# yuxiaoxiangyong/Multilateral-Temporal-view-Pyramid-Transformer-for-Video-Inpainting-Detection

Hardware: AMD Instinct MI355X
Metric: clips/sec fwd (B=8,T=5,224x224) (higher is better)
Workload: dtype f32; 1 GPU; full Mumpy forward (3 temporal views, pyramid decoder), B=8 clips/GPU, T=5, 224x224, fp32, tubelets (5,4,1); global_batch=8, launch=hipGraph replay, fork/join over HIP streams (independent branches co-scheduled), parallelism=batch-sharded x1, one metric all-reduce

## Files before the change

### multilateral-temporal-view-pyramid-transformer-for-video-inpainting-detection_amd/csrc/abi.cpp

```cpp
#include <stdarg.h>
#include <stdio.h>
#include <string.h>
#include "common.h"
#include "../../include/mumpy_hip_ext.h"
#include "../../include/mumpy_hip_ext2.h"
#include "../../include/mumpy_hip_ext3.h"
#include "../../include/mumpy_hip_ext4.h"
#include "../../include/mumpy_hip_ext5.h"
#include "../../include/mumpy_hip_ext6.h"
#include "../../include/mumpy_hip_ext7.h"
#include "../../include/mumpy_hip_ext8.h"
#include "../../include/mumpy_hip_ext9.h"
#include "../../include/mumpy_hip_ext10.h"
#include "../../include/mumpy_perturb.h"

namespace mumpy {
static thread_local char g_err[512] = "";
void set_error(const char* fmt, ...) {
    va_list ap;
    va_start(ap, fmt);
    vsnprintf(g_err, sizeof(g_err), fmt, ap);
    va_end(ap);
}
thread_local Route g_route;
static thread_local char g_route_text[160] = "";
static const char* format_route() {
    static const char* const addr[] = {"dense", "rows", "kseg", "conv"};
    static const char* const ln[] = {"none", "producer", "consumer"};
    static const char* const red[] = {"none", "one", "two-in-one", "taps"};
    const Route& r = g_route;
    char* t = g_route_text;
    const size_t n = sizeof(g_route_text);
    switch (r.family) {
    case Route::TILED: snprintf(t, n, "tiled tile=%d ks=%d np=%d addr=%s", r.tile, r.ks, r.np, addr[r.addr & 3]); break;
    case Route::TILED16: snprintf(t, n, "tiled16 tile=%d ks=%d np=%d addr=%s", r.tile, r.ks, r.np, addr[r.addr & 3]); break;
    case Route::WS:
        snprintf(t, n, "ws sched=%s P=%d ln=%s addr=%s", r.split ? "split" : "whole", r.passes, ln[r.ln < 3 ? r.ln : 0], addr[r.addr & 3]);
        break;
    case Route::WS64: snprintf(t, n, "ws64 P=%d addr=dense", r.passes); break;
    case Route::WS16: snprintf(t, n, "ws16 P=%d addr=dense", r.passes); break;
    case Route::XGEMM: {
        char dx[24] = "-", dw[24] = "-";
        if (r.prod[0].wt) snprintf(dx, sizeof(dx), "%dx%d", r.prod[0].wt, r.prod[0].ks);
        if (r.prod[1].wt) snprintf(dw, sizeof(dw), "%dx%d", r.prod[1].wt, r.prod[1].ks);
        snprintf(t, n, "xgemm np=%d addr=%s dx=%s dw=%s reduce=%s", r.np, addr[r.addr & 3], dx, dw, red[r.reduce & 3]);
        break;
    }
    default: snprintf(t, n, "none");
    }
    if (r.dual && r.family != Route::NONE) {
        const size_t len = strlen(t);
        snprintf(t + len, n - len, r.family == Route::XGEMM ? " gate=gelu" : " dual=z");
    }
    return t;
}
#ifdef MUMPY_TUNING
#include <stdlib.h>
int tune_int(const char* name, int dflt) {
    const char* v = getenv(name);
    return v ? atoi(v) : dflt;
}
const char* tune_str(const char* name) { return getenv(name); }
#endif
}

extern "C" int mumpy_tuning_build(void) {
#ifdef MUMPY_TUNING
    return 1;
#else
    return 0;
#endif
}

extern "C" int mumpy_abi_version(void) { return MUMPY_ABI_VERSION; }
extern "C" int mumpy_ext_version(void) { return MUMPY_EXT_VERSION; }
extern "C" int mumpy_ext2_version(void) { return MUMPY_EXT2_VERSION; }
extern "C" int mumpy_ext3_version(void) { return MUMPY_EXT3_VERSION; }
extern "C" int mumpy_ext4_version(void) { return MUMPY_EXT4_VERSION; }
extern "C" int mumpy_ext5_version(void) { return MUMPY_EXT5_VERSION; }
extern "C" int mumpy_ext6_version(void) { return MUMPY_EXT6_VERSION; }
extern "C" int mumpy_ext7_version(void) { return MUMPY_EXT7_VERSION; }
extern "C" int mumpy_ext8_version(void) { return MUMPY_EXT8_VERSION; }
extern "C" int mumpy_ext9_version(void) { return MUMPY_EXT9_VERSION; }
extern "C" int mumpy_ext10_version(void) { return MUMPY_EXT10_VERSION; }
extern "C" int mumpy_perturb_version(void) { return MUMPY_PERTURB_VERSION; }
extern "C" const char* mumpy_last_error(void) { return mumpy::g_err; }
extern "C" const char* mumpy_last_route(void) { return mumpy::format_route(); }
```

### multilateral-temporal-view-pyramid-transformer-for-video-inpainting-detection_amd/csrc/common.h

```cpp
#pragma once
#include <hip/hip_runtime.h>
#include <stdint.h>
#include <stdio.h>
#include "../../include/mumpy_hip.h"

namespace mumpy {

typedef float f32x4 __attribute__((ext_vector_type(4)));
typedef float f32x16 __attribute__((ext_vector_type(16)));

constexpr int WAVE = 64;
constexpr int WS = 7;
constexpr int WT = 49;
constexpr int HD = 32;

void set_error(const char* fmt, ...);

#ifdef MUMPY_TUNING
int tune_int(const char* name, int dflt);
const char* tune_str(const char* name);
#else
inline int tune_int(const char*, int dflt) { return dflt; }
inline const char* tune_str(const char*) { return nullptr; }
#endif

struct Route {
    enum Family : uint8_t { NONE, TILED, TILED16, WS, WS64, WS16, XGEMM };
    enum Addr : uint8_t { DENSE, ROWS, KSEG, CONV };
    enum Reduce : uint8_t { R_NONE, R_ONE, R_TWO_IN_ONE, R_TAPS };
    uint8_t family = NONE;
    uint8_t tile = 0;
    uint8_t np = 0;
    uint8_t addr = DENSE;
    uint8_t split = 0;
    uint8_t passes = 0;
    uint8_t ln = 0;
    uint8_t reduce = R_NONE;
    uint8_t dual = 0;
    int ks = 1;
    struct { int wt, ks; } prod[2] = {{0, 0}, {0, 0}};
};
extern thread_local Route g_route;

inline hipStream_t as_stream(void* s) { return reinterpret_cast<hipStream_t>(s); }
inline bool aligned16(const void* p) { return (reinterpret_cast<uintptr_t>(p) & 15u) == 0; }

#define MUMPY_CHECK_LAUNCH(name)                                                     \
    do {                                                                             \
        hipError_t e_ = hipGetLastError();                                           \
        if (e_ != hipSuccess) {                                                      \
            mumpy::set_error("%s: launch failed: %s", name, hipGetErrorString(e_));  \
            return (int)e_;                                                          \
        }                                                                            \
    } while (0)

#define MUMPY_REQUIRE(cond, code, ...)                                               \
    do {                                                                             \
        if (!(cond)) {                                                               \
            mumpy::set_error(__VA_ARGS__);                                           \
            return code;                                                             \
        }                                                                            \
    } while (0)

__device__ __forceinline__ unsigned xcd_major_id(unsigned orig, unsigned nwg) {
    const unsigned xcd = orig & 7, q8 = nwg >> 3, r8 = nwg & 7;
    return (xcd < r8 ? xcd * (q8 + 1) : r8 * (q8 + 1) + (xcd - r8) * q8) + (orig >> 3);
}

template <int CTRL>
__device__ __forceinline__ float dpp_f(float v) {
    return __builtin_bit_cast(float, __builtin_amdgcn_update_dpp(0, __builtin_bit_cast(int, v), CTRL, 0xF, 0xF, true));
}
__device__ __forceinline__ float swz_xor16(float v) {
    return __builtin_bit_cast(float, __builtin_amdgcn_ds_swizzle(__builtin_bit_cast(int, v), (16 << 10) | 0x1f));
}

__device__ __forceinline__ float wave_sum(float v, int width) {
    if (width > 1) v += dpp_f<0xB1>(v);
    if (width > 2) v += dpp_f<0x4E>(v);
    if (width > 4) v += dpp_f<0x141>(v);
    if (width > 8) v += dpp_f<0x140>(v);
    if (width > 16) v += swz_xor16(v);
    if (width > 32) v += __shfl_xor(v, 32);
    return v;
}

template <typename T>
__device__ __forceinline__ T ordered_sum(T first, const T* __restrict__ p, int64_t stride, int n_more) {
    T s = first;
    int z = 0;
    for (; z + 8 <= n_more; z += 8) {
        T v[8];
#pragma unroll
        for (int u = 0; u < 8; ++u) v[u] = p[(int64_t)(z + u) * stride];
#pragma unroll
        for (int u = 0; u < 8; ++u) s += v[u];
    }
    for (; z < n_more; ++z) s += p[(int64_t)z * stride];
    return s;
}

__device__ __forceinline__ void gn_block_stats(const float* __restrict__ stats, int nsplit, int G, int b, int64_t HW, int cg, float eps,
                                               float* gm, float* gr, double (*red)[2]) {
    const int tid = threadIdx.x, nslice = 256 / G, g = tid % G, k = tid / G;
    const int64_t per = (HW + nsplit - 1) / nsplit;
    const float* base = stats + (int64_t)b * nsplit * G * 2 + g * 2;
    const double piv = (double)base[0] / (double)((per < HW ? per : HW) * cg);
    double s = 0.0, q = 0.0;
    if (k < nslice)
        for (int sp = k; sp < nsplit; sp += nslice) {
            const int64_t p0 = sp * per, cnt = ((p0 + per < HW) ? p0 + per : HW) - p0;
            if (cnt <= 0) continue;
            const float* o = base + (int64_t)sp * G * 2;
            const double ni = (double)(cnt * cg), dm = (double)o[0] / ni - piv;
            s += ni * dm; q += (double)o[1] + ni * dm * dm;
        }
    red[tid][0] = s; red[tid][1] = q;
    __syncthreads();
    if (tid < G) {
        double ss = 0.0, qq = 0.0;
        for (int j = 0; j < nslice; ++j) { ss += red[j * G + tid][0]; qq += red[j * G + tid][1]; }
        const double n = (double)HW * (double)cg, dm = ss / n;
        double var = qq / n - dm * dm;
        if (var < 0.0) var = 0.0;
        gm[tid] = (float)(piv + dm);
        gr[tid] = (float)(1.0 / sqrt(var + (double)eps));
    }
    __syncthreads();
}

__device__ __forceinline__ float erf_fast(float x) {
    const float ax = fabsf(x);
    const float t = __builtin_amdgcn_rcpf(fmaf(0.3275911f, ax, 1.0f));
    float p = fmaf(1.061405429f, t, -1.453152027f);
    p = fmaf(p, t, 1.421413741f);
    p = fmaf(p, t, -0.284496736f);
    p = fmaf(p, t, 0.254829592f);
    const float y = 1.0f - p * t * __expf(-ax * ax);
    return copysignf(y, x);
}

__device__ __forceinline__ float gelu_erf(float x) { return 0.5f * x * (1.0f + erf_fast(x * 0.70710678118654752440f)); }

__device__ __forceinline__ float gelu_grad(float x) {
    const float cdf = 0.5f * (1.0f + erf_fast(x * 0.70710678118654752440f));
    const float pdf = 0.3989422804014327f * __expf(-0.5f * x * x);
    return cdf + x * pdf;
}

__device__ __forceinline__ int window_token(int wy, int wx, int p, int Hs, int W, int shift) {
    int py = p / WS, px = p - py * WS;
    int y = wy * WS + py + shift;
    int x = wx * WS + px + shift;
    if (y >= Hs) y -= Hs;
    if (x >= W) x -= W;
    return y * W + x;
}

}
```

### multilateral-temporal-view-pyramid-transformer-for-video-inpainting-detection_amd/csrc/gemm.hip

```cpp
#include <stdlib.h>
#include <type_traits>
#include "common.h"
#include "../../include/mumpy_hip_ext2.h"
#include "gemm_ws.h"
#include "gemm_ws64.h"
using namespace mumpy;

namespace {

constexpr int BK = 32;
constexpr int LDR = 36;

struct ConvGeom {
    int H, W, Cin, kh, kw, ph, pw;
    int kseg, kstride;
};

__device__ __attribute__((aligned(128))) float g_zero_page[32];

template <int BM, int BN>
__device__ __forceinline__ void tile_of_block(int64_t M, unsigned gn, int ksplit, unsigned& tm, unsigned& tn, int& ks) {
    constexpr unsigned NG = (BN >= 128) ? 4 : 8;
    unsigned wgid = xcd_major_id(blockIdx.x, gridDim.x);
    ks = (int)(wgid % (unsigned)ksplit);
    wgid /= (unsigned)ksplit;
    const unsigned gm = (unsigned)((M + BM - 1) / BM);
    const unsigned full = (gn / NG) * NG;
    if (wgid < gm * full) {
        const unsigned grp = wgid / (gm * NG), rem = wgid - grp * gm * NG;
        tm = rem / NG;
        tn = grp * NG + rem % NG;
    } else {
        const unsigned wdt = gn - full, rem = wgid - gm * full;
        tm = rem / wdt;
        tn = full + rem % wdt;
    }
}

struct ConvTap {
    int dy, dx, off;
    __device__ __forceinline__ bool inside(const ConvGeom& cg, int yx) const {
        const int yy = (yx >> 16) + dy, xx = (yx & 0xffff) + dx;
        return (unsigned)yy < (unsigned)cg.H && (unsigned)xx < (unsigned)cg.W;
    }
};
__device__ __forceinline__ ConvTap conv_tap(const ConvGeom& cg, int k0) {
    const int tap = k0 / cg.Cin, c0 = k0 - tap * cg.Cin;
    const int dy = tap / cg.kw - cg.ph, dx = tap % cg.kw - cg.pw;
    return {dy, dx, (dy * cg.W + dx) * cg.Cin + c0};
}

template <int TM, int TN, int WM, int WN, bool OUT16 = false, bool DUAL = false>
__device__ __forceinline__ void store_tile(const f32x16 (&acc)[TM][TN], int64_t m0, int n0, int wm, int wn, int c, int h,
                                           int64_t M, int N, const float* __restrict__ bias, const float* residual,
                                           float* Y, int act, int ksplit, int ks, float* slab) {
    const int wm_u = __builtin_amdgcn_readfirstlane(wm), wn_u = __builtin_amdgcn_readfirstlane(wn);
    const int64_t mw = m0 + wm_u * WM;
    const int64_t wbase = mw * N + n0 + wn_u * WN;
    const int rows_left = (int)((M - mw) < (int64_t)WM ? (M - mw) : (int64_t)WM);
    const uint32_t nb = 4u * (uint32_t)N;
    const uint32_t lane_off = 4u * h * nb + 4u * c;
    if (ksplit > 1) {
        char* S = reinterpret_cast<char*>(slab + (int64_t)ks * M * N + wbase);
#pragma unroll
        for (int j = 0; j < TN; ++j) {
            if (n0 + wn_u * WN + 32 * j + c >= N) continue;
#pragma unroll
            for (int i = 0; i < TM; ++i)
#pragma unroll
                for (int r = 0; r < 16; ++r) {
                    const int row = 32 * i + (r & 3) + 8 * (r >> 2);
                    if (row + 4 * h < rows_left) *reinterpret_cast<float*>(S + ((uint32_t)row * nb + lane_off + 128u * j)) = acc[i][j][r];
                }
        }
        return;
    }
    char* Yw = OUT16 ? reinterpret_cast<char*>(reinterpret_cast<__bf16*>(Y) + wbase) : reinterpret_cast<char*>(Y + wbase);
    const char* Rw = residual ? reinterpret_cast<const char*>(residual + wbase) : nullptr;
#pragma unroll
    for (int j = 0; j < TN; ++j) {
        const int n = n0 + wn_u * WN + 32 * j + c;
        if (n >= N) continue;
        const float bv = bias ? bias[n] : 0.f;
#pragma unroll
        for (int i = 0; i < TM; ++i)
#pragma unroll
            for (int r = 0; r < 16; ++r) {
                const int row = 32 * i + (r & 3) + 8 * (r >> 2);
                if (row + 4 * h >= rows_left) continue;
                const uint32_t off = (uint32_t)row * nb + lane_off + 128u * j;
                float v = acc[i][j][r] + bv;
                if (DUAL) *reinterpret_cast<float*>(const_cast<char*>(Rw) + off) = v;
                if (act == MUMPY_ACT_GELU) v = gelu_erf(v);
                if (!DUAL && Rw) v += *reinterpret_cast<const float*>(Rw + off);
                if (OUT16) *reinterpret_cast<__bf16*>(Yw + (off >> 1)) = (__bf16)v;
                else *reinterpret_cast<float*>(Yw + off) = v;
            }
    }
}

template <int BM, int BN, int WM, int WN, bool CONV, bool GLDS, bool PIPE = true, bool DUAL = false>
__global__ __launch_bounds__(64 * (BM / WM) * (BN / WN), (BM * BN > 64 * 64) ? 2 : (CONV ? 3 : 4)) void linear_kernel(const float* __restrict__ X, const float* __restrict__ Wt,
                                                     const float* __restrict__ bias, const float* residual,
                                                     float* Y, int64_t M, int N, int K, int act, unsigned gn,
                                                     int ksplit, float* slab, int64_t rpb, int64_t bstride, ConvGeom cg) {
    constexpr int TM = WM / 32, TN = WN / 32;
    constexpr int WAVES_N = BN / WN;
    constexpr int NT = 64 * (BM / WM) * (BN / WN);
    constexpr int RPI = NT / 8;
    constexpr int A_LD = BM / RPI;
    constexpr int B_LD = BN / RPI;
    static_assert(BM % RPI == 0 && BN % RPI == 0, "tile rows must divide over the staging passes");
    constexpr int LD = GLDS ? 32 : LDR;
    __shared__ __attribute__((aligned(1024))) float lds[2][(BM + BN) * LD];

    const int tid = threadIdx.x, lane = tid & 63, wave = tid >> 6;
    const int c = lane & 31, h = lane >> 5;
    const int wm = wave / WAVES_N, wn = wave % WAVES_N;
    unsigned tm, tn;
    int ks;
    tile_of_block<BM, BN>(M, gn, ksplit, tm, tn, ks);
    const int64_t m0 = (int64_t)tm * BM;
    const int n0 = (int)tn * BN;
    const int kbeg = ks * (K / ksplit);

    const int ld_row = tid >> 3, ld_c4 = tid & 7;
    f32x4 areg[A_LD], breg[B_LD];

    const float* arow[A_LD];
    const float* brow[B_LD];
    int ayx[A_LD];
#pragma unroll
    for (int i = 0; i < A_LD; ++i) {
        int64_t m = m0 + ld_row + RPI * i;
        if (m > M - 1) m = M - 1;
        if (CONV) {
            const unsigned mu = (unsigned)m, qx = mu / (unsigned)cg.W;
            const int x = (int)(mu - qx * (unsigned)cg.W);
            const int y = (int)(qx % (unsigned)cg.H);
            ayx[i] = (y << 16) | x;
            arow[i] = X + m * cg.Cin + 4 * ld_c4;
        } else {
            ayx[i] = 0;
            if (rpb >= M && !cg.kseg) arow[i] = X + m * K + 4 * ld_c4;
            else {
                const unsigned mu = (unsigned)m, blk = mu / (unsigned)rpb;
                arow[i] = X + (int64_t)blk * bstride + (int64_t)(mu - blk * (unsigned)rpb) * (cg.kseg ? cg.kseg : K) + 4 * ld_c4;
            }
        }
    }
#pragma unroll
    for (int i = 0; i < B_LD; ++i) {
        int n = n0 + ld_row + RPI * i;
        if (n > N - 1) n = N - 1;
        brow[i] = Wt + (int64_t)n * K + 4 * ld_c4;
    }
    int asw[A_LD], bsw[B_LD];
#pragma unroll
    for (int i = 0; i < A_LD; ++i) asw[i] = 4 * ((ld_c4 ^ (((ld_row + RPI * i) >> 1) & 7)) - ld_c4);
#pragma unroll
    for (int i = 0; i < B_LD; ++i) bsw[i] = 4 * ((ld_c4 ^ (((ld_row + RPI * i) >> 1) & 7)) - ld_c4);
    typedef __attribute__((address_space(1))) const void* gptr_t;
    typedef __attribute__((address_space(3))) void* lptr_t;
    auto gdma = [&](int k0, int buf) {
        const int wave_row = (tid >> 6) * 8;
        if (CONV) {
            const int tap = k0 / cg.Cin, c0 = k0 - tap * cg.Cin;
            const int dy = tap / cg.kw - cg.ph, dx = tap % cg.kw - cg.pw;
            const int off = (dy * cg.W + dx) * cg.Cin + c0;
#pragma unroll
            for (int i = 0; i < A_LD; ++i) {
                const int yy = (ayx[i] >> 16) + dy, xx = (ayx[i] & 0xffff) + dx;
                const bool ok = (unsigned)yy < (unsigned)cg.H && (unsigned)xx < (unsigned)cg.W;
                const float* src = ok ? arow[i] + off + asw[i] : g_zero_page + 4 * ld_c4;
                __builtin_amdgcn_global_load_lds((gptr_t)src, (lptr_t)&lds[buf][(wave_row + RPI * i) * LD], 16, 0, 0);
            }
        } else {
            const int ka = cg.kseg ? (k0 / cg.kseg) * cg.kstride + k0 % cg.kseg : k0;
#pragma unroll
            for (int i = 0; i < A_LD; ++i)
                __builtin_amdgcn_global_load_lds((gptr_t)(arow[i] + ka + asw[i]), (lptr_t)&lds[buf][(wave_row + RPI * i) * LD], 16, 0, 0);
        }
#pragma unroll
        for (int i = 0; i < B_LD; ++i)
            __builtin_amdgcn_global_load_lds((gptr_t)(brow[i] + k0 + bsw[i]), (lptr_t)&lds[buf][(BM + wave_row + RPI * i) * LD], 16, 0, 0);
    };
    auto gload = [&](int k0) {
        if (CONV) {
            const ConvTap t = conv_tap(cg, k0);
#pragma unroll
            for (int i = 0; i < A_LD; ++i) {
                const bool ok = t.inside(cg, ayx[i]);
                const f32x4 v = *reinterpret_cast<const f32x4*>(arow[i] + (ok ? t.off : 0));
                areg[i] = ok ? v : f32x4{0, 0, 0, 0};
            }
        } else {
            const int ka = cg.kseg ? (k0 / cg.kseg) * cg.kstride + k0 % cg.kseg : k0;
#pragma unroll
            for (int i = 0; i < A_LD; ++i) areg[i] = *reinterpret_cast<const f32x4*>(arow[i] + ka);
        }
#pragma unroll
        for (int i = 0; i < B_LD; ++i) breg[i] = *reinterpret_cast<const f32x4*>(brow[i] + k0);
    };
    auto lstore = [&](int buf) {
#pragma unroll
        for (int i = 0; i < A_LD; ++i)
            *reinterpret_cast<f32x4*>(&lds[buf][(ld_row + RPI * i) * LD + 4 * ld_c4]) = areg[i];
#pragma unroll
        for (int i = 0; i < B_LD; ++i)
            *reinterpret_cast<f32x4*>(&lds[buf][(BM + ld_row + RPI * i) * LD + 4 * ld_c4]) = breg[i];
    };
    auto fread = [&](int buf, f32x4 (&af)[TM][4], f32x4 (&bf)[TN][4]) {
#pragma unroll
        for (int i = 0; i < TM; ++i) {
            const int R = wm * WM + 32 * i + c;
#pragma unroll
            for (int q = 0; q < 4; ++q) {
                const int col = GLDS ? 4 * ((4 * h + q) ^ ((R >> 1) & 7)) : 16 * h + 4 * q;
                af[i][q] = *reinterpret_cast<const f32x4*>(&lds[buf][R * LD + col]);
            }
        }
#pragma unroll
        for (int j = 0; j < TN; ++j) {
            const int R = wn * WN + 32 * j + c;
#pragma unroll
            for (int q = 0; q < 4; ++q) {
                const int col = GLDS ? 4 * ((4 * h + q) ^ ((R >> 1) & 7)) : 16 * h + 4 * q;
                bf[j][q] = *reinterpret_cast<const f32x4*>(&lds[buf][(BM + R) * LD + col]);
            }
        }
    };

    f32x16 acc[TM][TN];
#pragma unroll
    for (int i = 0; i < TM; ++i)
#pragma unroll
        for (int j = 0; j < TN; ++j)
#pragma unroll
            for (int r = 0; r < 16; ++r) acc[i][j][r] = 0.f;
    auto mma = [&](const f32x4 (&af)[TM][4], const f32x4 (&bf)[TN][4]) {
#pragma unroll
        for (int s = 0; s < 16; ++s)
#pragma unroll
            for (int i = 0; i < TM; ++i)
#pragma unroll
                for (int j = 0; j < TN; ++j)
                    acc[i][j] = __builtin_amdgcn_mfma_f32_32x32x2f32(af[i][s >> 2][s & 3], bf[j][s >> 2][s & 3], acc[i][j], 0, 0, 0);
    };

    const int nk = K / ksplit / BK;
    f32x4 afA[TM][4], bfA[TN][4];
    if (GLDS && !PIPE) {
        gdma(kbeg, 0);
        if (nk > 1) gdma(kbeg + BK, 1);
        for (int kc = 0; kc < nk; ++kc) {
            __syncthreads();
            fread(kc & 1, afA, bfA);
            __syncthreads();
            if (kc + 2 < nk) gdma(kbeg + (kc + 2) * BK, kc & 1);
            mma(afA, bfA);
        }
    } else if (GLDS) {
        f32x4 afB[TM][4], bfB[TN][4];
        gdma(kbeg, 0);
        if (nk > 1) gdma(kbeg + BK, 1);
        __syncthreads();
        fread(0, afA, bfA);
        __syncthreads();
        if (nk > 2) gdma(kbeg + 2 * BK, 0);
        int kc = 0;
        for (; kc + 1 < nk; kc += 2) {
            fread(1, afB, bfB);
            mma(afA, bfA);
            __syncthreads();
            if (kc + 3 < nk) gdma(kbeg + (kc + 3) * BK, 1);
            if (kc + 2 < nk) fread(0, afA, bfA);
            mma(afB, bfB);
            __syncthreads();
            if (kc + 4 < nk) gdma(kbeg + (kc + 4) * BK, 0);
        }
        if (kc < nk) mma(afA, bfA);
    } else {
    f32x4 afB[TM][4], bfB[TN][4];
    gload(kbeg);
    lstore(0);
    if (nk > 1) gload(kbeg + BK);
    __syncthreads();
    fread(0, afA, bfA);
    if (nk > 1) lstore(1);
    if (nk > 2) gload(kbeg + 2 * BK);
    __syncthreads();
    int kc = 0;
    for (; kc + 1 < nk; kc += 2) {
        fread(1, afB, bfB);
        mma(afA, bfA);
        if (kc + 2 < nk) lstore(0);
        if (kc + 3 < nk) gload(kbeg + (kc + 3) * BK);
        __syncthreads();
        if (kc + 2 < nk) fread(0, afA, bfA);
        mma(afB, bfB);
        if (kc + 3 < nk) lstore(1);
        if (kc + 4 < nk) gload(kbeg + (kc + 4) * BK);
        __syncthreads();
    }
    if (kc < nk) mma(afA, bfA);
    }
    store_tile<TM, TN, WM, WN, false, DUAL>(acc, m0, n0, wm, wn, c, h, M, N, bias, residual, Y, act, ksplit, ks, slab);
}

typedef __bf16 bf16x8 __attribute__((ext_vector_type(8)));
typedef __bf16 bf16x2 __attribute__((ext_vector_type(2)));
typedef float f32x2 __attribute__((ext_vector_type(2)));
constexpr int LDH = 20;

template <int BM, int BN, int WM, int WN, bool CONV, int NP = 1, int NBUF = 2, bool IN16 = false, bool OUT16 = false, bool DUAL = false>
__global__ __launch_bounds__(256, 2) void linear_bf16_kernel(const float* __restrict__ X, const float* __restrict__ Wt,
                                                            const float* __restrict__ bias, const float* residual,
                                                            float* Y, int64_t M, int N, int K, int act, unsigned gn,
                                                            int ksplit, float* slab, int64_t rpb, int64_t bstride,
                                                            ConvGeom cg) {
    constexpr int TM = WM / 32, TN = WN / 32;
    constexpr int WAVES_N = BN / WN;
    static_assert((BM / WM) * (BN / WN) == 4, "4 waves per block");
    constexpr int RPI = 32, A_LD = BM / RPI, B_LD = BN / RPI;
    constexpr int PL = (BM + BN) * LDH;
    static_assert(NBUF * NP * PL * 4 <= 65536, "LDS tile exceeds the static limit");
    __shared__ __attribute__((aligned(16))) uint32_t lds[NBUF][NP * PL];
    const int tid = threadIdx.x, lane = tid & 63, wave = tid >> 6;
    const int c = lane & 31, h = lane >> 5;
    const int wm = wave / WAVES_N, wn = wave % WAVES_N;
    unsigned tm, tn;
    int ks;
    tile_of_block<BM, BN>(M, gn, ksplit, tm, tn, ks);
    const int64_t m0 = (int64_t)tm * BM;
    const int n0 = (int)tn * BN;
    const int kbeg = ks * (K / ksplit);
    const int ld_row = tid >> 3, ld_c4 = tid & 7;
    static_assert(!(IN16 || OUT16) || (NP == 1 && !CONV), "bf16 storage: plain bf16 products on dense operands only");
    f32x4 areg[A_LD], breg[B_LD];
    uint2 areg16[IN16 ? A_LD : 1], breg16[IN16 ? B_LD : 1];
    const float* arow[A_LD];
    const float* brow[B_LD];
    int ayx[A_LD];
#pragma unroll
    for (int i = 0; i < A_LD; ++i) {
        int64_t m = m0 + ld_row + RPI * i;
        if (m > M - 1) m = M - 1;
        if (IN16) {
            ayx[i] = 0;
            arow[i] = reinterpret_cast<const float*>(reinterpret_cast<const __bf16*>(X) + m * K + 4 * ld_c4);
            continue;
        }
        if (CONV) {
            const unsigned mu = (unsigned)m, qx = mu / (unsigned)cg.W;
            ayx[i] = ((int)(qx % (unsigned)cg.H) << 16) | (int)(mu - qx * (unsigned)cg.W);
            arow[i] = X + m * cg.Cin + 4 * ld_c4;
        } else {
            ayx[i] = 0;
            if (rpb >= M && !cg.kseg) arow[i] = X + m * K + 4 * ld_c4;
            else {
                const unsigned mu = (unsigned)m, blk = mu / (unsigned)rpb;
                arow[i] = X + (int64_t)blk * bstride + (int64_t)(mu - blk * (unsigned)rpb) * (cg.kseg ? cg.kseg : K) + 4 * ld_c4;
            }
        }
    }
#pragma unroll
    for (int i = 0; i < B_LD; ++i) {
        int n = n0 + ld_row + RPI * i;
        if (n > N - 1) n = N - 1;
        if (IN16) brow[i] = reinterpret_cast<const float*>(reinterpret_cast<const __bf16*>(Wt) + (int64_t)n * K + 4 * ld_c4);
        else brow[i] = Wt + (int64_t)n * K + 4 * ld_c4;
    }
    auto gload = [&](int k0) {
        if (IN16) {
#pragma unroll
            for (int i = 0; i < A_LD; ++i) areg16[i] = *reinterpret_cast<const uint2*>(reinterpret_cast<const __bf16*>(arow[i]) + k0);
#pragma unroll
            for (int i = 0; i < B_LD; ++i) breg16[i] = *reinterpret_cast<const uint2*>(reinterpret_cast<const __bf16*>(brow[i]) + k0);
            return;
        }
        if (CONV) {
            const ConvTap t = conv_tap(cg, k0);
#pragma unroll
            for (int i = 0; i < A_LD; ++i) {
                const bool ok = t.inside(cg, ayx[i]);
                const f32x4 v = *reinterpret_cast<const f32x4*>(arow[i] + (ok ? t.off : 0));
                areg[i] = ok ? v : f32x4{0, 0, 0, 0};
            }
        } else {
            const int ka = cg.kseg ? (k0 / cg.kseg) * cg.kstride + k0 % cg.kseg : k0;
#pragma unroll
            for (int i = 0; i < A_LD; ++i) areg[i] = *reinterpret_cast<const f32x4*>(arow[i] + ka);
        }
#pragma unroll
        for (int i = 0; i < B_LD; ++i) breg[i] = *reinterpret_cast<const f32x4*>(brow[i] + k0);
    };
    auto lstore_row = [&](uint32_t* dst, f32x4 r) {
#pragma unroll
        for (int p = 0; p < NP; ++p) {
            const bf16x2 lo = __builtin_convertvector(f32x2{r.x, r.y}, bf16x2), hi = __builtin_convertvector(f32x2{r.z, r.w}, bf16x2);
            const uint2 u = {*reinterpret_cast<const uint32_t*>(&lo), *reinterpret_cast<const uint32_t*>(&hi)};
            *reinterpret_cast<uint2*>(dst + p * PL) = u;
            if (p + 1 < NP)
                r -= f32x4{__uint_as_float(u.x << 16), __uint_as_float(u.x & 0xffff0000u), __uint_as_float(u.y << 16),
                           __uint_as_float(u.y & 0xffff0000u)};
        }
    };
    auto lstore = [&](int buf) {
        if (IN16) {
#pragma unroll
            for (int i = 0; i < A_LD; ++i) *reinterpret_cast<uint2*>(&lds[buf][(ld_row + RPI * i) * LDH + 2 * ld_c4]) = areg16[i];
#pragma unroll
            for (int i = 0; i < B_LD; ++i) *reinterpret_cast<uint2*>(&lds[buf][(BM + ld_row + RPI * i) * LDH + 2 * ld_c4]) = breg16[i];
            return;
        }
#pragma unroll
        for (int i = 0; i < A_LD; ++i) lstore_row(&lds[buf][(ld_row + RPI * i) * LDH + 2 * ld_c4], areg[i]);
#pragma unroll
        for (int i = 0; i < B_LD; ++i) lstore_row(&lds[buf][(BM + ld_row + RPI * i) * LDH + 2 * ld_c4], breg[i]);
    };
    f32x16 acc[TM][TN];
#pragma unroll
    for (int i = 0; i < TM; ++i)
#pragma unroll
        for (int j = 0; j < TN; ++j)
#pragma unroll
            for (int r = 0; r < 16; ++r) acc[i][j][r] = 0.f;
    constexpr int NPROD = (NP == 3) ? 6 : (NP == 2) ? 3 : 1;
    constexpr int PA[6] = {NP == 3 ? 2 : 1, 0, NP == 3 ? 1 : 0, 1, 0, 0}, PB[6] = {0, NP == 3 ? 2 : 1, NP == 3 ? 1 : 0, 0, 1, 0};
    const int nk = K / ksplit / BK;
    bf16x8 af[TM][2][NP], bf[TN][2][NP];
    auto fread = [&](int buf) {
#pragma unroll
        for (int i = 0; i < TM; ++i)
#pragma unroll
            for (int st = 0; st < 2; ++st)
#pragma unroll
                for (int p = 0; p < NP; ++p)
                    af[i][st][p] = *reinterpret_cast<const bf16x8*>(&lds[buf][p * PL + (wm * WM + 32 * i + c) * LDH + 8 * st + 4 * h]);
#pragma unroll
        for (int j = 0; j < TN; ++j)
#pragma unroll
            for (int st = 0; st < 2; ++st)
#pragma unroll
                for (int p = 0; p < NP; ++p)
                    bf[j][st][p] = *reinterpret_cast<const bf16x8*>(&lds[buf][p * PL + (BM + wn * WN + 32 * j + c) * LDH + 8 * st + 4 * h]);
    };
    auto mma = [&]() {
#pragma unroll
        for (int st = 0; st < 2; ++st)
#pragma unroll
            for (int q = 0; q < NPROD; ++q)
#pragma unroll
                for (int i = 0; i < TM; ++i)
#pragma unroll
                    for (int j = 0; j < TN; ++j)
                        acc[i][j] = __builtin_amdgcn_mfma_f32_32x32x16_bf16(af[i][st][NP > 1 ? PA[q] : 0],
                                                                            bf[j][st][NP > 1 ? PB[q] : 0], acc[i][j], 0, 0, 0);
    };
    const int klast = kbeg + (nk - 1) * BK;
    if (NBUF == 2) {
        gload(kbeg);
        lstore(0);
        __syncthreads();
        for (int kc = 0; kc + 1 < nk; ++kc) {
            gload(kbeg + (kc + 1) * BK);
            __builtin_amdgcn_sched_barrier(0);
            fread(kc & 1);
            mma();
            lstore((kc & 1) ^ 1);
            __syncthreads();
        }
        fread((nk - 1) & 1);
        mma();
    } else {
        gload(kbeg);
        lstore(0);
        gload(nk > 1 ? kbeg + BK : kbeg);
        __syncthreads();
        for (int kc = 0; kc + 1 < nk; ++kc) {
            fread(0);
            __syncthreads();
            lstore(0);
            const int knext = kbeg + (kc + 2) * BK;
            gload(knext < klast ? knext : klast);
            mma();
            __syncthreads();
        }
        fread(0);
        mma();
    }
    store_tile<TM, TN, WM, WN, OUT16, DUAL>(acc, m0, n0, wm, wn, c, h, M, N, bias, residual, Y, act, ksplit, ks, slab);
}

template <bool DUAL = false>
__global__ __launch_bounds__(256) void splitk_reduce_kernel(const float* __restrict__ slab, const float* __restrict__ bias,
                                                            const float* residual, float* Y, int64_t MN4, int N,
                                                            int ksplit, int act) {
    for (int64_t i = (int64_t)blockIdx.x * 256 + threadIdx.x; i < MN4; i += (int64_t)gridDim.x * 256) {
        f32x4 v = ordered_sum(reinterpret_cast<const f32x4*>(slab)[i], reinterpret_cast<const f32x4*>(slab) + MN4 + i, MN4, ksplit - 1);
        const int n = (int)((i * 4) % N);
        if (bias) v += *reinterpret_cast<const f32x4*>(bias + n);
        if (DUAL) reinterpret_cast<f32x4*>(const_cast<float*>(residual))[i] = v;
        if (act == MUMPY_ACT_GELU) {
#pragma unroll
            for (int e = 0; e < 4; ++e) v[e] = gelu_erf(v[e]);
        }
        if (!DUAL && residual) v += reinterpret_cast<const f32x4*>(residual)[i];
        reinterpret_cast<f32x4*>(Y)[i] = v;
    }
}

struct Plan {
    int tile;
    int ksplit;
    unsigned gn;
    int64_t gm;
};

constexpr int NUM_CU = 256;

int fit_ksplit(int K, int want, int min_slice, int max_ks) {
    int ks = want;
    if (ks > K / min_slice) ks = K / min_slice;
    if (ks > max_ks) ks = max_ks;
    while (ks > 1 && (K % (32 * ks)) != 0) --ks;
    return ks < 1 ? 1 : ks;
}

Plan make_plan_x3(int64_t M, int N, int K, bool allow_split) {
    Plan p;
    const int64_t gm128 = (M + 127) / 128, gm64 = (M + 63) / 64;
    const unsigned gn128 = (N + 127) / 128, gn64 = (N + 63) / 64;
    const int64_t b128 = gm128 * gn128, b64 = gm64 * gn64;
    auto fit = [&](int want) { return allow_split ? fit_ksplit(K, want, 384, 16) : 1; };
    const int ksw = fit((int)((448 + b128 / 2) / b128));
    if (b128 * ksw >= 240) {
        p.tile = 0; p.ksplit = ksw; p.gm = gm128; p.gn = gn128;
    } else {
        p.tile = 2; p.ksplit = (b64 < 2 * 256 && K >= 768) ? fit((int)((3 * 256 + b64 - 1) / b64)) : 1;
        p.gm = gm64; p.gn = gn64;
    }
    return p;
}

Plan make_plan(int64_t M, int N, int K, bool allow_split, bool x3 = false) {
    static const char* force = tune_str("MUMPY_GEMM_FORCE");
    if (x3 && !force) return make_plan_x3(M, N, K, allow_split);
    Plan p;
    const int64_t gm128 = (M + 127) / 128, gm64 = (M + 63) / 64;
    const unsigned gn128 = (N + 127) / 128, gn64 = (N + 63) / 64;
    const int64_t b128 = gm128 * gn128, b64 = gm64 * gn64;
    const double nk = (double)K / BK;
    const double t128 = (double)((b128 + NUM_CU - 1) / NUM_CU) * (nk + 2.0) / nk;
    double t64 = (double)((b64 + NUM_CU - 1) / NUM_CU) * 0.272;
    if (t64 < 0.357) t64 = 0.357;
    t64 *= (nk + 0.5) / nk;
    int tile = (t128 <= t64) ? 0 : 2;
    if (tile == 0 && b128 > NUM_CU && K >= 512) tile = 3;
    int ks = 1;
    static const int min_slice = tune_int("MUMPY_GEMM_MINSLICE", 384), max_ks = tune_int("MUMPY_GEMM_MAXKS", 16),
                     min_k = tune_int("MUMPY_GEMM_SPLIT_MINK", 768);
    if (tile == 2 && allow_split && b64 < 2 * NUM_CU && K >= min_k) ks = fit_ksplit(K, (int)((3 * NUM_CU + b64 - 1) / b64), min_slice, max_ks);
    if (force) {
        int ft = -1, fk = -1;
        if (sscanf(force, "%d,%d", &ft, &fk) >= 1 && ft >= 0 && ft <= 3) {
            tile = ft;
            if (fk >= 1 && allow_split && K % (32 * fk) == 0) ks = fk; else if (fk >= 1) ks = 1;
        }
    }
    p.tile = tile; p.ksplit = ks;
    p.gm = (tile == 0 || tile == 3) ? gm128 : gm64;
    p.gn = (tile == 2) ? gn64 : gn128;
    return p;
}

int device_cus() {
    static int num_cu = 0;
    if (!num_cu) {
        int dev = 0;
        hipDeviceProp_t prop;
        if (hipGetDevice(&dev) == hipSuccess && hipGetDeviceProperties(&prop, dev) == hipSuccess) num_cu = prop.multiProcessorCount;
        else num_cu = NUM_CU;
    }
    return num_cu;
}

int ws_plan(int64_t M, int N, int K, bool have_ws, bool conv) {
    static const int ws_mode = tune_int("MUMPY_GEMM_WS", 2);
    const int num_cu = device_cus();
    const int64_t tiles = ((M + 127) / 128) * ((N + 127) / 128);
    const int nk = K / 32;
    const double rounds = (double)tiles / num_cu, eff = rounds / (double)((tiles + num_cu - 1) / num_cu);
    const double per_cu = (double)tiles * nk / num_cu;
    int how = 0;
    if (ws_mode == 1) how = 1;
    else if (ws_mode == 3) how = have_ws ? 2 : 1;
    else if (ws_mode == 2 && conv) {
        if (have_ws && eff < 0.86 && per_cu >= 24.0 && (double)nk / per_cu <= 3.0) how = 2;
        else if (tiles >= (int64_t)(0.75 * num_cu) && eff >= 0.75 && K >= 128) how = 1;
    } else if (ws_mode == 2) {
        if (tiles >= (int64_t)(0.75 * num_cu) && eff >= 0.86 && K >= 128 && !(K >= 1024 && rounds >= 1.8)) how = 1;
        else if (have_ws && eff < 0.86 && per_cu >= 24.0 && (double)nk / per_cu <= 3.0 && !(K >= 1024 && rounds >= 1.8)) how = 2;
    }
    return how;
}

struct LinearArgs {
    const float *x, *W, *bias, *residual;
    float* y;
    int64_t M;
    int N, K, act;
    hipStream_t s;
    float* ws = nullptr;
    int64_t ws_bytes = 0;
    bool ws_clean = false;
    int64_t rpb = 0, bstride = 0;
    int kseg = 0, kstride = 0;
    const ConvGeom* conv = nullptr;
    const gemm_ws::LnArgs* ln = nullptr;
    float* z = nullptr;
};

struct TiledArgs {
    const float *x, *W, *bias, *residual;
    float* y;
    int64_t M;
    int N, K, act;
    unsigned gn;
    int ksplit;
    float* slab;
    int64_t rpb, bstride;
    ConvGeom cg;
    int64_t grid;
    hipStream_t s;
};

template <class Kern>
void launch_tiled(Kern kern, unsigned threads, const TiledArgs& t) {
    hipLaunchKernelGGL(kern, dim3((unsigned)t.grid), dim3(threads), 0, t.s, t.x, t.W, t.bias, t.residual, t.y, t.M, t.N, t.K, t.act,
                       t.gn, t.ksplit, t.slab, t.rpb, t.bstride, t.cg);
}

template <class F>
void with_bool(bool b, F&& f) {
    if (b) f(std::true_type{});
    else f(std::false_type{});
}

void launch_tiled_fp32(int tile, bool conv, bool glds, const TiledArgs& t) {
    with_bool(conv, [&](auto cv) {
        constexpr bool CV = decltype(cv)::value;
        if (tile == 3) return launch_tiled(linear_kernel<128, 128, 64, 64, CV, true, false>, 256, t);
        with_bool(glds, [&](auto gl) {
            constexpr bool GL = decltype(gl)::value;
            if (tile == 0) launch_tiled(linear_kernel<128, 128, 64, 32, CV, GL>, 512, t);
            else if (tile == 1) launch_tiled(linear_kernel<64, 128, 32, 64, CV, GL>, 256, t);
            else launch_tiled(linear_kernel<64, 64, 32, 32, CV, GL>, 256, t);
        });
    });
}

void launch_tiled_dual(int tile, bool bf16, const TiledArgs& t) {
    if (bf16) {
        if (tile == 0) launch_tiled(linear_bf16_kernel<128, 128, 64, 64, false, 1, 2, false, false, true>, 256, t);
        else launch_tiled(linear_bf16_kernel<64, 64, 32, 32, false, 1, 2, false, false, true>, 256, t);
    } else if (tile == 3) launch_tiled(linear_kernel<128, 128, 64, 64, false, true, false, true>, 256, t);
    else if (tile == 0) launch_tiled(linear_kernel<128, 128, 64, 32, false, false, true, true>, 512, t);
    else launch_tiled(linear_kernel<64, 64, 32, 32, false, false, true, true>, 256, t);
}

template <int NP, bool IN16 = false>
void launch_tiled_bf16(bool wide, bool flag, const TiledArgs& t) {
    with_bool(wide, [&](auto wd) {
        with_bool(flag, [&](auto fl) {
            constexpr int T = decltype(wd)::value ? 128 : 64, NBUF = (T == 128 && NP > 1) ? 1 : 2;
            constexpr bool FL = decltype(fl)::value;
            launch_tiled(linear_bf16_kernel<T, T, T / 2, T / 2, !IN16 && FL, NP, NBUF, IN16, IN16 && FL>, 256, t);
        });
    });
}

int launch_linear(const LinearArgs& a) {
    const int64_t M = a.M, rpb = a.rpb > 0 ? a.rpb : M, bstride = a.rpb > 0 ? a.bstride : 0;
    const int N = a.N, K = a.K, act = a.act & 0xff;
    const ConvGeom* conv = a.conv;
    ConvGeom cg = conv ? *conv : ConvGeom{0, 0, 0, 0, 0, 0, 0, 0, 0};
    cg.kseg = a.kseg; cg.kstride = a.kstride;
    const bool math_bf16 = (a.act & MUMPY_MATH_BF16) != 0;
    const bool math_x2 = (a.act & MUMPY_MATH_BF16X2) != 0;
    const bool math_x3 = (a.act & MUMPY_MATH_BF16X3) != 0 || math_x2;
    float* ws = a.ws;
    int64_t ws_bytes = a.ws_bytes;
    const gemm_ws::Conv cvd{cg.H, cg.W, cg.Cin, cg.kh, cg.kw};
    if (a.ln && (rpb < M || math_bf16 || math_x3 || conv || !gemm_ws::eligible(M, N, K) ||
                 !ws_plan(M, N, K, ws && ws_bytes >= gemm_ws::workspace_bytes(device_cus()), false))) {
        set_error("linear: LayerNorm folding needs a shape the persistent 128x128 kernel takes (mumpy_linear_ln_tiles) in fp32 mode");
        return MUMPY_EINVAL;
    }
    if (rpb >= M && !a.kseg && !math_bf16 && !math_x3 && (conv ? gemm_ws::conv_eligible(M, N, cvd) : gemm_ws::eligible(M, N, K))) {
        const int num_cu = device_cus();
        const bool have_ws = ws && ws_bytes >= gemm_ws::workspace_bytes(num_cu);
        const int how = ws_plan(M, N, K, have_ws, conv != nullptr);
        const int nk = K / 32;
        static const int ws64_mode = tune_int("MUMPY_GEMM_WS64", 1);
        if (!how && !conv && ws64_mode && !a.z) {
            const int64_t t64 = ((M + 63) / 64) * ((N + 63) / 64);
            const double r64 = (double)t64 / (2.0 * num_cu);
            const bool fits = ws64_mode == 2 || (act != MUMPY_ACT_GELU && nk <= 32 && t64 >= 64 && (r64 <= 1.0 || r64 >= 2.5 || nk <= 12));
            if (fits) {
                if (int rc = gemm_ws64::launch(a.x, a.W, a.bias, a.residual, a.y, M, N, K, act, num_cu, a.s)) return rc;
                MUMPY_CHECK_LAUNCH("linear(ws64)");
                return 0;
            }
        }
        if (how) {
            if (int rc = gemm_ws::launch(a.x, a.W, a.bias, a.residual, a.y, M, N, K, act, num_cu, a.s, ws, ws_bytes, how == 2 ? 1 : 0, nullptr,
                                         a.ws_clean, conv ? &cvd : nullptr, a.ln, a.z)) return rc;
            MUMPY_CHECK_LAUNCH("linear(ws)");
            return 0;
        }
    }
    Plan p = make_plan(M, N, K, ws != nullptr, math_x3);
    if (ws) { ws += 1024; ws_bytes -= 4096; }
    if (p.ksplit > 1 && (int64_t)p.ksplit * M * N * (int64_t)sizeof(float) > ws_bytes) p.ksplit = 1;
    if (math_bf16 || math_x3) {
        if (p.tile == 3) p.tile = 0;
        if (p.tile == 1) { p.tile = 2; p.gn = (unsigned)((N + 63) / 64); }
    }
    if (a.z && p.tile == 1) { p.tile = 2; p.gn = (unsigned)((N + 63) / 64); }
    const int64_t grid = p.gm * p.gn * p.ksplit;
    MUMPY_REQUIRE(grid < (1ll << 31), MUMPY_ERANGE, "linear: too many tiles");
    static const bool use_glds = tune_int("MUMPY_GEMM_GLDS", 0) != 0;
    const bool wide = (p.tile == 0 || p.tile == 3);
    const TiledArgs t{a.x, a.W, a.bias, a.z ? a.z : a.residual, a.y, M, N, K, act, p.gn, p.ksplit, ws, rpb, bstride, cg, grid, a.s};
    g_route = Route{};
    g_route.family = Route::TILED; g_route.tile = (uint8_t)p.tile; g_route.ks = p.ksplit;
    g_route.np = math_x2 ? 2 : math_x3 ? 3 : math_bf16 ? 1 : 0;
    g_route.addr = conv ? Route::CONV : a.kseg ? Route::KSEG : rpb < M ? Route::ROWS : Route::DENSE;
    g_route.dual = a.z ? 1 : 0;
    if (a.z) launch_tiled_dual(p.tile, math_bf16, t);
    else if (math_x2) launch_tiled_bf16<2>(wide, conv != nullptr, t);
    else if (math_x3) launch_tiled_bf16<3>(wide, conv != nullptr, t);
    else if (math_bf16) launch_tiled_bf16<1>(wide, conv != nullptr, t);
    else launch_tiled_fp32(p.tile, conv != nullptr, use_glds, t);
    MUMPY_CHECK_LAUNCH("linear");
    if (p.ksplit > 1) {
        const int64_t mn4 = M * N / 4;
        int64_t g = (mn4 + 255) / 256;
        if (g > 2048) g = 2048;
        if (a.z) hipLaunchKernelGGL(splitk_reduce_kernel<true>, dim3((unsigned)g), dim3(256), 0, a.s, ws, a.bias, a.z, a.y, mn4, N, p.ksplit, act);
        else hipLaunchKernelGGL(splitk_reduce_kernel<false>, dim3((unsigned)g), dim3(256), 0, a.s, ws, a.bias, a.residual, a.y, mn4, N,
                                p.ksplit, act);
        MUMPY_CHECK_LAUNCH("linear(split-K reduce)");
    }
    return 0;
}

}

static int check_linear_args(const char* who, const void* x, const void* W, const float* residual, const void* y, int64_t M, int N,
                             int K, int act) {
    MUMPY_REQUIRE(x && W && y, MUMPY_ENULL, "%s: null pointer", who);
    MUMPY_REQUIRE(aligned16(x) && aligned16(W) && aligned16(y) && aligned16(residual), MUMPY_EALIGN,
                  "%s: pointers must be 16-byte aligned", who);
    MUMPY_REQUIRE(M < (1ll << 31) - 256 && (int64_t)N * 4 * 128 < (1ll << 32), MUMPY_ERANGE,
                  "%s: M=%lld rows / N=%d columns beyond the 32-bit row index / tile byte offsets", who, (long long)M, N);
    MUMPY_REQUIRE(M >= 0 && N > 0 && K > 0 && K % BK == 0 && N % 32 == 0, MUMPY_EINVAL,
                  "%s: need K %% 32 == 0 and N %% 32 == 0 (got M=%lld N=%d K=%d)", who, (long long)M, N, K);
    MUMPY_REQUIRE((act & 0xff) == MUMPY_ACT_NONE || (act & 0xff) == MUMPY_ACT_GELU, MUMPY_EINVAL, "%s: unknown act %d", who, act);
    constexpr int math_bits = MUMPY_MATH_BF16 | MUMPY_MATH_BF16X3 | MUMPY_MATH_BF16X2;
    MUMPY_REQUIRE((act & ~(0xff | math_bits)) == 0, MUMPY_EINVAL, "%s: unknown flag bits in act 0x%x", who, act);
    MUMPY_REQUIRE(((act & math_bits) & ((act & math_bits) - 1)) == 0, MUMPY_EINVAL, "%s: the MUMPY_MATH_* modes are exclusive", who);
    return 0;
}

static LinearArgs linear_args(const float* x, const float* W, const float* bias, const float* residual, float* y, int64_t M, int N,
                              int K, int act, void* workspace, int64_t workspace_bytes, void* stream) {
    LinearArgs a{x, W, bias, residual, y, M, N, K, act, as_stream(stream)};
    a.ws = static_cast<float*>(workspace);
    a.ws_bytes = workspace ? workspace_bytes : 0;
    return a;
}

extern "C" int mumpy_linear_fwd(const float* x, const float* W, const float* bias, const float* residual, float* y,
                                int64_t M, int N, int K, int act, void* stream) {
    if (M == 0) return 0;
    if (int rc = check_linear_args("linear", x, W, residual, y, M, N, K, act)) return rc;
    return launch_linear(linear_args(x, W, bias, residual, y, M, N, K, act, nullptr, 0, stream));
}

extern "C" int64_t mumpy_linear_workspace_bytes(int64_t M, int N, int K) {
    if (M <= 0 || N <= 0 || K <= 0 || K % BK) return 0;
    const Plan p = make_plan(M, N, K, true), q = make_plan(M, N, K, true, true);
    const int ks = p.ksplit > q.ksplit ? p.ksplit : q.ksplit;
    int64_t bytes = ks > 1 ? (int64_t)ks * M * N * (int64_t)sizeof(float) + 4096 : 0;
    if (gemm_ws::eligible(M, N, K)) {
        const int64_t tiles = ((M + 127) / 128) * ((N + 127) / 128);
        const double per_cu = (double)tiles * (K / 32) / NUM_CU;
        const int64_t need = gemm_ws::workspace_bytes(2 * NUM_CU);
        if (per_cu >= 16.0 && bytes < need) bytes = need;
    }
    return bytes;
}

extern "C" int mumpy_linear_ws_fwd(const float* x, const float* W, const float* bias, const float* residual, float* y,
                                   int64_t M, int N, int K, int act, void* workspace, int64_t workspace_bytes,
                                   void* stream) {
    if (M == 0) return 0;
    if (int rc = check_linear_args("linear", x, W, residual, y, M, N, K, act)) return rc;
    MUMPY_REQUIRE(workspace_bytes >= 0, MUMPY_EINVAL, "linear_ws: workspace_bytes must not be negative");
    MUMPY_REQUIRE(aligned16(workspace), MUMPY_EALIGN, "linear: workspace must be 16-byte aligned");
    return launch_linear(linear_args(x, W, bias, residual, y, M, N, K, act, workspace, workspace_bytes, stream));
}

extern "C" int mumpy_linear_bf16s_fwd(const void* x, const void* W, const float* bias, const float* residual, void* y,
                                      int64_t M, int N, int K, int act, int out_bf16, void* stream) {
    if (M == 0) return 0;
    if (int rc = check_linear_args("linear_bf16s", x, W, residual, y, M, N, K, act)) return rc;
    MUMPY_REQUIRE((act & ~0xff) == 0, MUMPY_EINVAL, "linear_bf16s: unknown act %d", act);
    MUMPY_REQUIRE(!(out_bf16 && residual), MUMPY_EINVAL, "linear_bf16s: a bf16 output takes no residual");
    hipStream_t s = as_stream(stream);
    static const int ws16 = tune_int("MUMPY_GEMM_WS16", 2);
    const int64_t gm128 = (M + 127) / 128, gm64 = (M + 63) / 64;
    const unsigned gn128 = (N + 127) / 128, gn64 = (N + 63) / 64;
    if (ws16 && gemm_ws::eligible16(M, N, K)) {
        const int num_cu = device_cus();
        const int64_t tiles = gm128 * gn128;
        const double rounds = (double)tiles / num_cu, eff = rounds / (double)((tiles + num_cu - 1) / num_cu);
        if (ws16 == 2 || (tiles >= (int64_t)(0.75 * num_cu) && eff >= 0.75)) {
            if (int rc = gemm_ws::launch16(x, W, bias, residual, y, M, N, K, act, out_bf16 != 0, num_cu, s)) return rc;
            MUMPY_CHECK_LAUNCH("linear_bf16s(ws)");
            return 0;
        }
    }
    const bool wide = gm128 * gn128 >= 200;
    const unsigned gn = wide ? gn128 : gn64;
    const int64_t grid = (wide ? gm128 : gm64) * gn;
    MUMPY_REQUIRE(grid < (1ll << 31), MUMPY_ERANGE, "linear_bf16s: too many tiles");
    const TiledArgs t{static_cast<const float*>(x), static_cast<const float*>(W), bias, residual, static_cast<float*>(y), M, N, K, act,
                      gn, 1, nullptr, M, 0, ConvGeom{0, 0, 0, 0, 0, 0, 0, 0, 0}, grid, s};
    g_route = Route{};
    g_route.family = Route::TILED16; g_route.tile = wide ? 0 : 2; g_route.np = 1;
    launch_tiled_bf16<1, true>(wide, out_bf16 != 0, t);
    MUMPY_CHECK_LAUNCH("linear_bf16s");
    return 0;
}

extern "C" int mumpy_linear_wsz_fwd(const float* x, const float* W, const float* bias, const float* residual, float* y,
                                    int64_t M, int N, int K, int act, void* workspace, int64_t workspace_bytes,
                                    void* stream) {
    if (M == 0) return 0;
    if (int rc = check_linear_args("linear", x, W, residual, y, M, N, K, act)) return rc;
    MUMPY_REQUIRE(workspace_bytes >= 0, MUMPY_EINVAL, "linear_wsz: workspace_bytes must not be negative");
    MUMPY_REQUIRE(aligned16(workspace), MUMPY_EALIGN, "linear: workspace must be 16-byte aligned");
    LinearArgs a = linear_args(x, W, bias, residual, y, M, N, K, act, workspace, workspace_bytes, stream);
    a.ws_clean = true;
    return launch_linear(a);
}

extern "C" int mumpy_linear_gelu_dual_fwd(const float* x, const float* W, const float* bias, float* z, float* a, int64_t M, int N,
                                          int K, int math, void* workspace, int64_t workspace_bytes, void* stream) {
    if (M == 0) return 0;
    MUMPY_REQUIRE(math == 0 || math == MUMPY_MATH_BF16, MUMPY_EINVAL,
                  "linear_gelu_dual: math is 0 or MUMPY_MATH_BF16 (the split-precision modes have no dual-output form; got 0x%x)", math);
    MUMPY_REQUIRE(z, MUMPY_ENULL, "linear_gelu_dual: null pointer");
    if (int rc = check_linear_args("linear_gelu_dual", x, W, z, a, M, N, K, MUMPY_ACT_GELU | math)) return rc;
    MUMPY_REQUIRE(z != a, MUMPY_EINVAL, "linear_gelu_dual: z and a must be two buffers");
    MUMPY_REQUIRE(workspace_bytes >= 0, MUMPY_EINVAL, "linear_gelu_dual: workspace_bytes must not be negative");
    MUMPY_REQUIRE(aligned16(workspace) && aligned16(bias), MUMPY_EALIGN, "linear_gelu_dual: bias and workspace must be 16-byte aligned");
    MUMPY_REQUIRE(!workspace || workspace_bytes >= mumpy_linear_workspace_bytes(M, N, K), MUMPY_EINVAL,
                  "linear_gelu_dual: workspace too small (mumpy_linear_workspace_bytes)");
    LinearArgs la = linear_args(x, W, bias, nullptr, a, M, N, K, MUMPY_ACT_GELU | math, workspace, workspace_bytes, stream);
    la.ws_clean = true;
    la.z = z;
    return launch_linear(la);
}

extern "C" int mumpy_workspace_status(const void* workspace, int* status) {
    MUMPY_REQUIRE(workspace && status, MUMPY_ENULL, "workspace_status: null pointer");
    unsigned w[2] = {0, 0};
    static_assert(gemm_ws::LN_GUARD_WORD + 1 == gemm_ws::STATUS_WORD, "status words must be adjacent");
    hipError_t e = hipMemcpy(w, static_cast<const unsigned*>(workspace) + gemm_ws::LN_GUARD_WORD, sizeof(w), hipMemcpyDeviceToHost);
    if (e != hipSuccess) { set_error("workspace_status: %s", hipGetErrorString(e)); return (int)e; }
    *status = w[1] ? (int)w[1] : (w[0] ? -1 : 0);
    return 0;
}

extern "C" int mumpy_linear_ln_tiles(int64_t M, int N, int K) {
    if (M <= 0 || N <= 0 || K <= 0 || K % BK || N % 32 || !gemm_ws::eligible(M, N, K)) return 0;
    return ws_plan(M, N, K, true, false) ? (N + 127) / 128 : 0;
}

extern "C" int mumpy_linear_lnx_fwd(const float* x, const float* W, const float* bias, const float* residual, float* y, int64_t M,
                                    int N, int K, int act, void* workspace, int64_t workspace_bytes, float* stats_out,
                                    const float* ln_stats, int ln_gn, const float* ln_colsum, float ln_eps, void* stream) {
    if (M == 0) return 0;
    if (int rc = check_linear_args("linear", x, W, residual, y, M, N, K, act)) return rc;
    MUMPY_REQUIRE((act & ~0xff) == 0, MUMPY_EINVAL, "linear_lnx: fp32 matrix math only");
    MUMPY_REQUIRE(aligned16(workspace) && workspace, MUMPY_EALIGN, "linear_lnx: needs the kept (zeroed) workspace of mumpy_linear_wsz_fwd");
    MUMPY_REQUIRE(ln_gn >= 0, MUMPY_EINVAL, "linear_lnx: ln_gn must not be negative");
    MUMPY_REQUIRE(workspace_bytes >= 4096, MUMPY_EINVAL, "linear_lnx: the kept workspace holds at least its 4096-byte flag page (got %lld B)",
                  (long long)workspace_bytes);
    MUMPY_REQUIRE((stats_out != nullptr) != (ln_stats != nullptr), MUMPY_EINVAL, "linear_lnx: exactly one of stats_out (producer) / ln_stats (consumer)");
    MUMPY_REQUIRE(!ln_stats || (ln_colsum && bias && !residual && ln_gn == (K + 127) / 128 && ln_gn <= 16 && ln_eps > 0.f), MUMPY_EINVAL,
                  "linear_lnx: the consumer takes W gamma, colsum, bias = W beta + b, no residual, and ln_gn = ceil(K / 128) tiles (got %d)", ln_gn);
    MUMPY_REQUIRE(aligned16(stats_out) && aligned16(ln_stats) && aligned16(ln_colsum), MUMPY_EALIGN, "linear_lnx: pointers must be 16-byte aligned");
    MUMPY_REQUIRE(M * (int64_t)((N + 127) / 128) * 8 < (1ll << 31) && M * (int64_t)(ln_gn > 0 ? ln_gn : 1) * 8 < (1ll << 31), MUMPY_ERANGE,
                  "linear_lnx: statistics buffer beyond 2 GiB");
    const gemm_ws::LnArgs ln{stats_out, ln_stats, ln_colsum, ln_gn, K, ln_eps};
    LinearArgs a = linear_args(x, W, bias, residual, y, M, N, K, act, workspace, workspace_bytes, stream);
    a.ws_clean = true;
    a.ln = &ln;
    return launch_linear(a);
}

extern "C" int mumpy_linear_rows_fwd(const float* x, int64_t rows_per_block, int64_t block_stride, const float* W,
                                     const float* bias, const float* residual, float* y, int64_t M, int N, int K, int act,
                                     void* workspace, int64_t workspace_bytes, void* stream) {
    if (M == 0) return 0;
    if (int rc = check_linear_args("linear", x, W, residual, y, M, N, K, act)) return rc;
    MUMPY_REQUIRE(workspace_bytes >= 0, MUMPY_EINVAL, "linear_rows: workspace_bytes must not be negative");
    MUMPY_REQUIRE(rows_per_block > 0 && M % rows_per_block == 0 && block_stride >= 0 && block_stride % 4 == 0, MUMPY_EINVAL,
                  "linear_rows: M=%lld must be a multiple of rows_per_block=%lld and block_stride >= 0, %% 4 == 0",
                  (long long)M, (long long)rows_per_block);
    LinearArgs a = linear_args(x, W, bias, residual, y, M, N, K, act, workspace, workspace_bytes, stream);
    a.rpb = rows_per_block; a.bstride = block_stride;
    return launch_linear(a);
}

extern "C" int mumpy_linear_rows_kseg_fwd(const float* x, int64_t rows_per_block, int64_t block_stride, int kseg, int kstride,
                                          const float* W, const float* bias, const float* residual, float* y, int64_t M, int N, int K,
                                          int act, void* workspace, int64_t workspace_bytes, void* stream) {
    if (M == 0) return 0;
    if (int rc = check_linear_args("linear", x, W, residual, y, M, N, K, act)) return rc;
    MUMPY_REQUIRE(workspace_bytes >= 0, MUMPY_EINVAL, "linear_rows_kseg: workspace_bytes must not be negative");
    MUMPY_REQUIRE(rows_per_block > 0 && M % rows_per_block == 0 && block_stride >= 0 && block_stride % 4 == 0, MUMPY_EINVAL,
                  "linear_rows_kseg: M=%lld must be a multiple of rows_per_block=%lld and block_stride >= 0, %% 4 == 0",
                  (long long)M, (long long)rows_per_block);
    MUMPY_REQUIRE(kseg > 0 && kseg % 32 == 0 && K % kseg == 0 && kstride % 4 == 0 && kstride >= 0, MUMPY_EINVAL,
                  "linear_rows_kseg: need kseg %% 32 == 0, K %% kseg == 0, kstride %% 4 == 0 (got kseg=%d K=%d kstride=%d)", kseg, K, kstride);
    LinearArgs a = linear_args(x, W, bias, residual, y, M, N, K, act, workspace, workspace_bytes, stream);
    a.rpb = rows_per_block; a.bstride = block_stride;
    a.kseg = kseg; a.kstride = kstride;
    return launch_linear(a);
}

extern "C" int64_t mumpy_conv2d_workspace_bytes(int B, int H, int W, int Cin, int Cout, int kh, int kw) {
    return mumpy_linear_workspace_bytes((int64_t)B * H * W, Cout, kh * kw * Cin);
}

extern "C" int mumpy_conv2d_nhwc_fwd(const float* x, const float* w_krsc, const float* bias, const float* residual,
                                     float* y, int B, int H, int W, int Cin, int Cout, int kh, int kw, int act,
                                     void* workspace, int64_t workspace_bytes, void* stream) {
    MUMPY_REQUIRE(B > 0 && H > 0 && W > 0 && H < 32768 && W < 32768, MUMPY_EINVAL, "conv2d: bad image size %dx%d", H, W);
    MUMPY_REQUIRE(kh > 0 && kw > 0 && (kh & 1) && (kw & 1), MUMPY_EINVAL, "conv2d: kernel %dx%d must be odd (same padding)", kh, kw);
    MUMPY_REQUIRE(Cin % 32 == 0 && Cout % 32 == 0, MUMPY_EINVAL, "conv2d: Cin=%d and Cout=%d must be multiples of 32", Cin, Cout);
    const int64_t M = (int64_t)B * H * W;
    const int K = kh * kw * Cin;
    if (int rc = check_linear_args("linear", x, w_krsc, residual, y, M, Cout, K, act)) return rc;
    MUMPY_REQUIRE(workspace_bytes >= 0, MUMPY_EINVAL, "conv2d: workspace_bytes must not be negative");
    MUMPY_REQUIRE(aligned16(workspace), MUMPY_EALIGN, "conv2d: workspace must be 16-byte aligned");
    const ConvGeom cg{H, W, Cin, kh, kw, kh / 2, kw / 2, 0, 0};
    LinearArgs a = linear_args(x, w_krsc, bias, residual, y, M, Cout, K, act, workspace, workspace_bytes, stream);
    a.conv = &cg;
    return launch_linear(a);
}
```

### multilateral-temporal-view-pyramid-transformer-for-video-inpainting-detection_amd/csrc/gemm_ws.h

```cpp
#pragma once
#include <type_traits>
#include "common.h"

namespace mumpy {
namespace gemm_ws {

constexpr int BM = 128, BN = 128, BK = 32;
constexpr int STAGE_DW = (BM + BN) * BK;
constexpr int NSTAGE = 3;
constexpr int E_DW = BM * BN;
constexpr int E_OFF_DW = NSTAGE * STAGE_DW;
constexpr int LDS_BYTES = (E_OFF_DW + E_DW) * 4;
constexpr int PASSES = BM / 8;
#ifndef MUMPY_WS_DBG
#define MUMPY_WS_DBG 0
#endif
constexpr int DBG = MUMPY_WS_DBG;
#ifndef MUMPY_WS_STORE_AUX
#define MUMPY_WS_STORE_AUX 0
#endif
constexpr uint32_t OOB = 0x80000000u;
constexpr int LN_GUARD_WORD = 1022;
constexpr float LN_GUARD_RATIO = 256.f;
constexpr int STATUS_WORD = 1023;

typedef uint32_t u32x4 __attribute__((ext_vector_type(4)));

struct Params {
    const float* X;
    const float* W;
    const float* bias;
    const float* residual;
    float* Y;
    int M, N, K, act;
    int nk;
    unsigned gm, gn;
    unsigned tiles;
    unsigned rr_cnt, rr_G;
    unsigned st_w;
    unsigned walk = 0;
    unsigned units;
    int lmin = 0;
    int cv_H = 0, cv_W = 0, cv_C = 0, cv_kh = 0, cv_kw = 0, cv_cpc = 0;
    unsigned cv_mhw = 0, cv_shw = 0, cv_mw = 0, cv_sw = 0;
    unsigned* flags = nullptr;
    float* slabs = nullptr;
    float* stats_out = nullptr;
    const float* ln_stats = nullptr;
    const float* ln_colsum = nullptr;
    int ln_gn = 0, ln_C = 0;
    float ln_eps = 0.f;
    unsigned* ln_guard = nullptr;
#ifdef MUMPY_WS_STAMP
    unsigned long long* stamps = nullptr;
#endif
};

__device__ __forceinline__ void ws_barrier() { asm volatile("s_waitcnt lgkmcnt(0)\n\ts_barrier" ::: "memory"); }

__device__ __forceinline__ void tile_coords(const Params& p, unsigned v, unsigned& tm, unsigned& tn) {
    unsigned q = v;
    if (p.rr_cnt) {
        const unsigned bq = v / p.rr_cnt, rnd = v - bq * p.rr_cnt;
        q = bq + rnd * p.rr_G;
    }
    const unsigned SW = p.st_w, SH = 32u / SW, SN = p.gn / SW, row_tiles = SN * 32u;
    const unsigned full_rows = p.gm / SH, full = full_rows * row_tiles;
    if (p.walk && q < (full_rows >> 3) * 8u * row_tiles) {
        const unsigned grp = 8u * row_tiles, g = q / grp, l = q - g * grp, s = l >> 5, j = l & 31u;
        tm = (g * 8u + (s & 7u)) * SH + j / SW;
        tn = (s >> 3) * SW + j % SW;
    } else if (q < full) {
        const unsigned sm = q / row_tiles, r = q - sm * row_tiles, sn = r >> 5, j = r & 31u;
        tm = sm * SH + j / SW;
        tn = sn * SW + j % SW;
    } else {
        const unsigned per = (p.gm - full_rows * SH) * SW, r = q - full, sn = r / per, j = r - sn * per;
        tm = full_rows * SH + j / SW;
        tn = sn * SW + j % SW;
    }
}

__device__ __host__ __forceinline__ unsigned first_chunk(unsigned b, unsigned G, unsigned units, int nk, int lmin) {
    unsigned u = (unsigned)(((uint64_t)b * units) / G);
    const unsigned r = u % (unsigned)nk;
    if (r != 0 && r < (unsigned)lmin) u -= r;
    else if (r != 0 && (unsigned)nk - r < 3u) u += (unsigned)nk - r;
    return u;
}

__device__ __forceinline__ void matrix_role(const Params& p, float* lds, int kc0, int n_chunks, int wave, int lane) {
    const int c = lane & 31, h = lane >> 5, wm = wave >> 1, wn = wave & 1;
    const int sw = (c >> 1) & 7;
    int a_off[4], b_off[4];
#pragma unroll
    for (int q = 0; q < 4; ++q) {
        a_off[q] = (64 * wm + c) * BK + 4 * ((4 * h + q) ^ sw);
        b_off[q] = (BM + 64 * wn + c) * BK + 4 * ((4 * h + q) ^ sw);
    }
    float* const E = lds + E_OFF_DW + (64 * wm + 4 * h) * BN + 64 * wn + c;
    f32x16 acc[2][2];
    f32x4 fa0[2], fb0[2], fa1[2], fb1[2];
    auto rd = [&](const float* st, int q, f32x4 (&fa)[2], f32x4 (&fb)[2]) {
#pragma unroll
        for (int i = 0; i < 2; ++i) fa[i] = *reinterpret_cast<const f32x4*>(st + a_off[q] + 32 * i * BK);
#pragma unroll
        for (int j = 0; j < 2; ++j) fb[j] = *reinterpret_cast<const f32x4*>(st + b_off[q] + 32 * j * BK);
    };
    auto mm = [&](const f32x4 (&fa)[2], const f32x4 (&fb)[2], int e) {
#pragma unroll
        for (int i = 0; i < 2; ++i)
#pragma unroll
            for (int j = 0; j < 2; ++j)
                acc[i][j] = __builtin_amdgcn_mfma_f32_32x32x2f32(fa[i][e], fb[j][e], acc[i][j], 0, 0, 0);
    };
    auto mm4 = [&](const f32x4 (&fa)[2], const f32x4 (&fb)[2]) {
#pragma unroll
        for (int e = 0; e < 4; ++e) mm(fa, fb, e);
    };
    auto dump = [&]() {
#pragma unroll
        for (int i = 0; i < 2; ++i)
#pragma unroll
            for (int j = 0; j < 2; ++j)
#pragma unroll
                for (int r = 0; r < 16; ++r) E[(32 * i + (r & 3) + 8 * (r >> 2)) * BN + 32 * j] = acc[i][j][r];
    };
    auto zero = [&]() {
#pragma unroll
        for (int i = 0; i < 2; ++i)
#pragma unroll
            for (int j = 0; j < 2; ++j)
#pragma unroll
                for (int r = 0; r < 16; ++r) acc[i][j][r] = 0.f;
    };
    zero();
#ifdef MUMPY_WS_STAMP
    unsigned long long t_bar = 0;
    const unsigned long long t_begin = __builtin_amdgcn_s_memtime();
#endif
    ws_barrier();
#ifdef MUMPY_WS_STAMP
    const unsigned long long t_loop = __builtin_amdgcn_s_memtime();
#endif
    rd(lds, 0, fa0, fb0);
    int kc = kc0, stage = 0;
#define WS_INTERLEAVE()                                            \
    do {                                                           \
        _Pragma("unroll") for (int g_ = 0; g_ < 4; ++g_) {         \
            __builtin_amdgcn_sched_group_barrier(0x008, 1, 0);     \
            __builtin_amdgcn_sched_group_barrier(0x100, 1, 0);     \
        }                                                          \
        __builtin_amdgcn_sched_group_barrier(0x008, 12, 0);        \
    } while (0)
    for (int i = 0; i < n_chunks; ++i) {
        const float* st = lds + stage * STAGE_DW;
        stage = stage == NSTAGE - 1 ? 0 : stage + 1;
        if (kc == 0 && i > 0) { dump(); zero(); }
        __builtin_amdgcn_sched_barrier(0);
        rd(st, 1, fa1, fb1);
        mm4(fa0, fb0);
        WS_INTERLEAVE();
        rd(st, 2, fa0, fb0);
        mm4(fa1, fb1);
        WS_INTERLEAVE();
        rd(st, 3, fa1, fb1);
        mm4(fa0, fb0);
        WS_INTERLEAVE();
        mm(fa1, fb1, 0);
        mm(fa1, fb1, 1);
        __builtin_amdgcn_sched_barrier(0);
#ifdef MUMPY_WS_STAMP
        const unsigned long long tb0 = __builtin_amdgcn_s_memtime();
#endif
        ws_barrier();
#ifdef MUMPY_WS_STAMP
        t_bar += __builtin_amdgcn_s_memtime() - tb0;
#endif
        __builtin_amdgcn_sched_barrier(0);
        rd(lds + stage * STAGE_DW, 0, fa0, fb0);
        mm(fa1, fb1, 2);
        mm(fa1, fb1, 3);
        __builtin_amdgcn_sched_group_barrier(0x100, 4, 0);
        __builtin_amdgcn_sched_group_barrier(0x008, 8, 0);
        __builtin_amdgcn_sched_barrier(0);
        if (++kc == p.nk) kc = 0;
    }
#undef WS_INTERLEAVE
#ifdef MUMPY_WS_STAMP
    const unsigned long long t_end = __builtin_amdgcn_s_memtime();
    if (wave == 0 && lane == 0) {
        unsigned long long* o = p.stamps + 8 * blockIdx.x;
        o[0] = t_loop - t_begin; o[1] = t_end - t_loop; o[2] = t_bar; o[3] = (unsigned long long)n_chunks;
    }
#endif
    dump();
    ws_barrier();
}

typedef __bf16 bf16x8 __attribute__((ext_vector_type(8)));
__device__ __forceinline__ void matrix_role16(const Params& p, float* lds, int kc0, int n_chunks, int wave, int lane) {
    const int c = lane & 31, h = lane >> 5, wm = wave >> 1, wn = wave & 1;
    const int sw = (c >> 1) & 7;
    int a_off[4], b_off[4];
#pragma unroll
// ... 18 lines not shown
#pragma unroll
        for (int i = 0; i < 2; ++i)
#pragma unroll
            for (int j = 0; j < 2; ++j)
#pragma unroll
                for (int r = 0; r < 16; ++r) E[(32 * i + (r & 3) + 8 * (r >> 2)) * BN + 32 * j] = acc[i][j][r];
    };
    auto zero = [&]() {
#pragma unroll
        for (int i = 0; i < 2; ++i)
#pragma unroll
            for (int j = 0; j < 2; ++j)
#pragma unroll
                for (int r = 0; r < 16; ++r) acc[i][j][r] = 0.f;
    };
    zero();
    ws_barrier();
    rd(lds, 0, fa0, fb0);
    int kc = kc0, stage = 0;
    for (int i = 0; i < n_chunks; ++i) {
        const float* st = lds + stage * STAGE_DW;
        stage = stage == NSTAGE - 1 ? 0 : stage + 1;
        if (kc == 0 && i > 0) { dump(); zero(); }
        rd(st, 1, fa1, fb1);
        mm_row(fa0, fb0, 0); mm_row(fa0, fb0, 1);
        rd(st, 2, fa0, fb0);
        mm_row(fa1, fb1, 0); mm_row(fa1, fb1, 1);
        rd(st, 3, fa1, fb1);
        mm_row(fa0, fb0, 0); mm_row(fa0, fb0, 1);
        mm_row(fa1, fb1, 0);
        ws_barrier();
        rd(lds + stage * STAGE_DW, 0, fa0, fb0);
        mm_row(fa1, fb1, 1);
        if (++kc == p.nk) kc = 0;
    }
    dump();
    ws_barrier();
}

template <bool CONV, bool IN16 = false>
__device__ __forceinline__ void loader_role(const Params& p, float* lds, unsigned tile0, int kc0, int n_chunks, int hl) {
    constexpr uint32_t ESZ = IN16 ? 2u : 4u;
    const int lane = hl & 63, lw = __builtin_amdgcn_readfirstlane(hl >> 6);
    const int prow = lane >> 3;
    uint32_t aoff[4], boff[4];
    uint32_t amask[4];
    auto set_tile = [&](unsigned t) {
        unsigned tm, tn;
        tile_coords(p, t, tm, tn);
#pragma unroll
        for (int q = 0; q < 4; ++q) {
            const int r = 32 * q + 8 * lw + prow;
            const uint32_t ch = (uint32_t)((lane & 7) ^ ((r >> 1) & 7));
            int m = (int)tm * BM + r;
            if (m > p.M - 1) m = p.M - 1;
            if (CONV) {
                const uint32_t img = __umulhi((uint32_t)m, p.cv_mhw) >> p.cv_shw;
                const uint32_t rem = (uint32_t)m - img * (uint32_t)(p.cv_H * p.cv_W);
                const uint32_t yy = __umulhi(rem, p.cv_mw) >> p.cv_sw, xx = rem - yy * (uint32_t)p.cv_W;
                uint32_t colbits = 0, mask = 0;
                for (int sx = 0; sx < p.cv_kw; ++sx)
                    colbits |= (uint32_t)((uint32_t)((int)xx + sx - (p.cv_kw >> 1)) < (uint32_t)p.cv_W) << sx;
                for (int ry = 0; ry < p.cv_kh; ++ry)
                    if ((uint32_t)((int)yy + ry - (p.cv_kh >> 1)) < (uint32_t)p.cv_H) mask |= colbits << (ry * p.cv_kw);
                amask[q] = mask;
                aoff[q] = ((uint32_t)m * (uint32_t)p.cv_C + 4u * ch) * 4u;
            } else {
                aoff[q] = (uint32_t)m * (uint32_t)p.K * ESZ + 16u * ch;
            }
            int n = (int)tn * BN + r;
            if (n > p.N - 1) n = p.N - 1;
            boff[q] = (uint32_t)n * (uint32_t)p.K * ESZ + 16u * ch;
        }
    };
    const auto rs_x = __builtin_amdgcn_make_buffer_rsrc(const_cast<float*>(p.X), 0, (int)0x7fffffff, 0x00020000);
    const auto rs_w = __builtin_amdgcn_make_buffer_rsrc(const_cast<float*>(p.W), 0, (int)0x7fffffff, 0x00020000);
    typedef __attribute__((address_space(3))) void* lptr_t;
    int cv_r = 0, cv_s = 0, cv_c = 0;
    if (CONV) {
        const int tap0 = kc0 / p.cv_cpc;
        cv_c = kc0 - tap0 * p.cv_cpc;
        cv_r = tap0 / p.cv_kw;
        cv_s = tap0 - cv_r * p.cv_kw;
    }
    auto dma = [&](int kc, int stage) {
        if (DBG & 1) return;
        const int so = kc * 128;
        float* st = lds + stage * STAGE_DW + 8 * lw * BK;
        if (CONV) {
            const int tap = cv_r * p.cv_kw + cv_s;
            const int delta = (((cv_r - (p.cv_kh >> 1)) * p.cv_W + (cv_s - (p.cv_kw >> 1))) * p.cv_C + 32 * cv_c) * 4;
#pragma unroll
            for (int q = 0; q < 4; ++q) {
                const uint32_t off = ((amask[q] >> tap) & 1u) ? aoff[q] + (uint32_t)delta : OOB;
                __builtin_amdgcn_raw_ptr_buffer_load_lds(rs_x, (lptr_t)(st + 32 * q * BK), 16, off, 0, 0, 0);
            }
        } else {
#pragma unroll
            for (int q = 0; q < 4; ++q)
                __builtin_amdgcn_raw_ptr_buffer_load_lds(rs_x, (lptr_t)(st + 32 * q * BK), 16, aoff[q], so, 0, 0);
        }
#pragma unroll
        for (int q = 0; q < 4; ++q)
            __builtin_amdgcn_raw_ptr_buffer_load_lds(rs_w, (lptr_t)(st + (BM + 32 * q) * BK), 16, boff[q], so, 0, 0);
    };
    unsigned ld_tile = tile0;
    int ld_kc = kc0, ld_idx = 0;
    auto advance = [&]() {
        if (ld_idx + 1 < n_chunks) {
            ++ld_idx;
            if (++ld_kc == p.nk) {
                ld_kc = 0; ++ld_tile; set_tile(ld_tile);
                if (CONV) { cv_r = 0; cv_s = 0; cv_c = 0; }
            } else if (CONV && ++cv_c == p.cv_cpc) {
                cv_c = 0;
                if (++cv_s == p.cv_kw) { cv_s = 0; ++cv_r; }
            }
        }
    };
    set_tile(ld_tile);
    dma(ld_kc, 0);
    advance();
    dma(ld_kc, 1);
    advance();
    asm volatile("s_waitcnt vmcnt(8)" ::: "memory");
    ws_barrier();
    int stage = 2;
#ifdef MUMPY_WS_STAMP
    unsigned long long t_work = 0, t_wait = 0, t_prev = __builtin_amdgcn_s_memtime();
#endif
    for (int i = 0; i < n_chunks; ++i) {
        dma(ld_kc, stage);
        advance();
        stage = stage == NSTAGE - 1 ? 0 : stage + 1;
        asm volatile("s_waitcnt vmcnt(8)" ::: "memory");
#ifdef MUMPY_WS_STAMP
        const unsigned long long t1 = __builtin_amdgcn_s_memtime();
#endif
        ws_barrier();
#ifdef MUMPY_WS_STAMP
        const unsigned long long t2 = __builtin_amdgcn_s_memtime();
        t_work += t1 - t_prev; t_wait += t2 - t1; t_prev = t2;
#endif
    }
#ifdef MUMPY_WS_STAMP
    if (hl == 0) { p.stamps[8 * blockIdx.x + 4] = t_work; p.stamps[8 * blockIdx.x + 5] = t_wait; }
#endif
    asm volatile("s_waitcnt vmcnt(0)" ::: "memory");
    ws_barrier();
}

__device__ __forceinline__ float half_sum32(float x) { return wave_sum(x, 32); }

template <int P, bool OUT16 = false, int LN = 0, bool DUAL = false>
__device__ __forceinline__ void epilogue_role(const Params& p, float* lds, unsigned b, unsigned G, unsigned u0, unsigned u1, int hl) {
    constexpr uint32_t OSZ = OUT16 ? 2u : 4u;
    const float* const E = lds + E_OFF_DW;
    const int e_row = hl >> 5, e_c4 = hl & 31;
    const unsigned nk = (unsigned)p.nk;
    const bool split = p.flags != nullptr;
    const auto rs_y = __builtin_amdgcn_make_buffer_rsrc(p.Y, 0, (int)((int64_t)p.M * p.N * OSZ), 0x00020000);
    const auto rs_r = __builtin_amdgcn_make_buffer_rsrc(const_cast<float*>(p.residual ? p.residual : p.Y), 0,
                                                        p.residual ? (int)((int64_t)p.M * p.N * 4) : 0, 0x00020000);
    const auto rs_b = __builtin_amdgcn_make_buffer_rsrc(const_cast<float*>(p.bias ? p.bias : p.Y), 0, p.bias ? p.N * 4 : 0, 0x00020000);
    const auto rs_s = __builtin_amdgcn_make_buffer_rsrc(split ? p.slabs + (size_t)b * E_DW : p.Y, 0, split ? E_DW * 4 : 0, 0x00020000);
    constexpr int STEPS = PASSES / P;
    f32x4 rv[PASSES], bias4;
    uint32_t yo[PASSES];
    const uint32_t row8 = 8u * (uint32_t)p.N * OSZ;
    const auto rs_st = __builtin_amdgcn_make_buffer_rsrc(LN == 1 ? p.stats_out : p.Y, 0, LN == 1 ? (int)((int64_t)p.M * p.gn * 8) : 0, 0x00020000);
    const auto rs_ln = __builtin_amdgcn_make_buffer_rsrc(const_cast<float*>(LN == 2 ? p.ln_stats : p.Y), 0,
                                                         LN == 2 ? (int)((int64_t)p.M * p.ln_gn * 8) : 0, 0x00020000);
    const auto rs_cs = __builtin_amdgcn_make_buffer_rsrc(const_cast<float*>(LN == 2 ? p.ln_colsum : p.Y), 0, LN == 2 ? p.N * 4 : 0, 0x00020000);
    uint32_t st_off = 0;
    float st_inv = 0.f;
    bool st_valid = false;
    float ln_mean = 0.f, ln_rstd = 0.f;
    f32x4 cs4 = {0.f, 0.f, 0.f, 0.f};
    const int ln_lane4 = ((hl & 32)) * 4;
    auto begin_tile = [&](unsigned t) {
        unsigned tm, tn;
        tile_coords(p, t, tm, tn);
        const int n = (int)tn * BN + 4 * e_c4;
        const uint32_t ybase = n < p.N ? (((uint32_t)tm * BM + e_row) * (uint32_t)p.N + (uint32_t)n) * OSZ : OOB;
#pragma unroll
        for (int e = 0; e < PASSES; ++e) {
            yo[e] = ybase + (uint32_t)e * row8;
            if (!DUAL) rv[e] = __builtin_bit_cast(f32x4, __builtin_amdgcn_raw_buffer_load_b128(rs_r, yo[e], 0, 0));
        }
        bias4 = __builtin_bit_cast(f32x4, __builtin_amdgcn_raw_buffer_load_b128(rs_b, n < p.N ? (uint32_t)n * 4u : OOB, 0, 0));
        if (LN == 1) {
            const int nt = p.N - (int)tn * BN < BN ? p.N - (int)tn * BN : BN;
            st_inv = 1.0f / (float)nt;
            st_valid = n < p.N;
            st_off = ((((uint32_t)tm * BM + e_row) * p.gn) + tn) * 8u;
        }
        if (LN == 2) {
            cs4 = __builtin_bit_cast(f32x4, __builtin_amdgcn_raw_buffer_load_b128(rs_cs, n < p.N ? (uint32_t)n * 4u : OOB, 0, 0));
            const uint32_t row = (uint32_t)tm * BM + 8u * (uint32_t)(e_c4 & 15) + (uint32_t)e_row;
            const uint32_t base = row * (uint32_t)p.ln_gn * 8u;
            float msum = 0.f;
            for (int t = 0; t < p.ln_gn; ++t) {
                const float nt = (float)(p.ln_C - t * BN < BN ? p.ln_C - t * BN : BN);
                msum += nt * __builtin_bit_cast(float, __builtin_amdgcn_raw_buffer_load_b32(rs_ln, base + 8u * t, 0, 0));
            }
            const float mean = msum / (float)p.ln_C;
            float m2 = 0.f;
            for (int t = 0; t < p.ln_gn; ++t) {
                const float nt = (float)(p.ln_C - t * BN < BN ? p.ln_C - t * BN : BN);
                const float mt = __builtin_bit_cast(float, __builtin_amdgcn_raw_buffer_load_b32(rs_ln, base + 8u * t, 0, 0));
                const float qt = __builtin_bit_cast(float, __builtin_amdgcn_raw_buffer_load_b32(rs_ln, base + 8u * t + 4u, 0, 0));
                const float d = mt - mean;
                m2 += qt + nt * d * d;
            }
            ln_mean = mean;
            ln_rstd = rsqrtf(m2 / (float)p.ln_C + p.ln_eps);
            if (fabsf(mean) * ln_rstd > LN_GUARD_RATIO && row < (uint32_t)p.M && p.ln_guard)
                __hip_atomic_store(p.ln_guard, 1u, __ATOMIC_RELAXED, __HIP_MEMORY_SCOPE_AGENT);
        }
    };
    auto pass = [&](int e) {
        f32x4 v = *reinterpret_cast<const f32x4*>(E + (8 * e + e_row) * BN + 4 * e_c4);
        if (LN == 2) {
            const float mean = __builtin_bit_cast(float, __builtin_amdgcn_ds_bpermute(ln_lane4 + 4 * e, __builtin_bit_cast(int, ln_mean)));
            const float rstd = __builtin_bit_cast(float, __builtin_amdgcn_ds_bpermute(ln_lane4 + 4 * e, __builtin_bit_cast(int, ln_rstd)));
            v = rstd * (v - mean * cs4);
        }
        v += bias4;
        if (DUAL) __builtin_amdgcn_raw_buffer_store_b128(__builtin_bit_cast(u32x4, v), rs_r, yo[e], 0, MUMPY_WS_STORE_AUX);
        if (p.act == MUMPY_ACT_GELU) {
#pragma unroll
            for (int x = 0; x < 4; ++x) v[x] = gelu_erf(v[x]);
        }
        if (!DUAL) v += rv[e];
        if (LN == 1) {
            const float mean_t = half_sum32(st_valid ? (v[0] + v[1]) + (v[2] + v[3]) : 0.f) * st_inv;
            const f32x4 d = v - mean_t;
            const float m2 = half_sum32(st_valid ? (d[0] * d[0] + d[1] * d[1]) + (d[2] * d[2] + d[3] * d[3]) : 0.f);
            if (e_c4 == 0) {
                typedef uint32_t u32x2 __attribute__((ext_vector_type(2)));
                const u32x2 st = {__builtin_bit_cast(uint32_t, mean_t), __builtin_bit_cast(uint32_t, m2)};
                __builtin_amdgcn_raw_buffer_store_b64(st, rs_st, st_off + (uint32_t)e * (8u * p.gn * 8u), 0, 0);
            }
        }
        if (OUT16) {
            typedef __bf16 bf16x4 __attribute__((ext_vector_type(4)));
            typedef uint32_t u32x2 __attribute__((ext_vector_type(2)));
            const bf16x4 o = {(__bf16)v[0], (__bf16)v[1], (__bf16)v[2], (__bf16)v[3]};
            __builtin_amdgcn_raw_buffer_store_b64(__builtin_bit_cast(u32x2, o), rs_y, yo[e], 0, MUMPY_WS_STORE_AUX);
        } else {
            __builtin_amdgcn_raw_buffer_store_b128(__builtin_bit_cast(u32x4, v), rs_y, yo[e], 0, MUMPY_WS_STORE_AUX);
        }
    };
    const uint32_t soff = ((uint32_t)e_row * BN + 4u * e_c4) * 4u;
    auto pass_part = [&](int e) {
        const f32x4 v = *reinterpret_cast<const f32x4*>(E + (8 * e + e_row) * BN + 4 * e_c4);
        __builtin_amdgcn_raw_buffer_store_b128(__builtin_bit_cast(u32x4, v), rs_s, soff, e * (8 * BN * 4), 0);
    };
    auto publish = [&]() {
        if (hl == 0) {
            __builtin_amdgcn_fence(__ATOMIC_RELEASE, "agent");
            asm volatile("s_waitcnt vmcnt(0)" ::: "memory");
            __hip_atomic_store(p.flags + b, 1u, __ATOMIC_RELAXED, __HIP_MEMORY_SCOPE_AGENT);
        }
    };

    ws_barrier();
    unsigned prev_t = u0 / nk;
    bool prev_part = (u0 % nk) != 0;
    unsigned u = (prev_t + 1) * nk < u1 ? (prev_t + 1) * nk : u1;
    for (unsigned c = u0; c < u; ++c) ws_barrier();
    if (DBG & 2) {
        for (; u < u1; ++u) ws_barrier();
        ws_barrier();
        return;
    }
    if (u < u1 && prev_part) {
        const unsigned end = u + nk < u1 ? u + nk : u1;
        ws_barrier();
#pragma unroll
        for (int st = 0; st < STEPS; ++st) {
#pragma unroll
            for (int k = 0; k < P; ++k) pass_part(st * P + k);
            if (st == STEPS - 1) asm volatile("s_waitcnt vmcnt(0)" ::: "memory");
            ws_barrier();
        }
        publish();
        for (unsigned c = u + 1 + STEPS; c < end; ++c) ws_barrier();
        prev_t = u / nk;
        prev_part = false;
        u = end;
    }
    while (u < u1) {
        const unsigned end = u + nk < u1 ? u + nk : u1;
        begin_tile(prev_t);
        ws_barrier();
#pragma unroll
        for (int st = 0; st < STEPS; ++st) {
#pragma unroll
            for (int k = 0; k < P; ++k) pass(st * P + k);
            ws_barrier();
        }
        for (unsigned c = u + 1 + STEPS; c < end; ++c) ws_barrier();
        prev_t = u / nk;
        u = end;
    }
    const bool head = split && !prev_part && (u1 % nk) != 0;
    if (!prev_part) begin_tile(prev_t);
    ws_barrier();
    if (prev_part) {
#pragma unroll
        for (int e = 0; e < PASSES; ++e) {
            pass_part(e);
            if (e % 4 == 3) __builtin_amdgcn_sched_barrier(0);
        }
        asm volatile("s_waitcnt vmcnt(0)\n\ts_barrier" ::: "memory");
        publish();
        return;
    }
    if (head) {
        const unsigned tile_end = (prev_t + 1) * nk;
        if (hl == 0) {
            for (unsigned b2 = b + 1; b2 < G; ++b2) {
                const unsigned f0 = first_chunk(b2, G, p.units, p.nk, p.lmin);
                if (f0 >= tile_end) break;
                if (first_chunk(b2 + 1, G, p.units, p.nk, p.lmin) == f0) continue;
                unsigned spins = 0;
                while (__hip_atomic_load(p.flags + b2, __ATOMIC_RELAXED, __HIP_MEMORY_SCOPE_AGENT) == 0u && ++spins < (1u << 24))
                    __builtin_amdgcn_s_sleep(8);
                if (spins >= (1u << 24)) {
                    __hip_atomic_store(p.flags + STATUS_WORD, 1u + b2, __ATOMIC_RELAXED, __HIP_MEMORY_SCOPE_AGENT);
                    continue;
                }
                __hip_atomic_store(p.flags + b2, 0u, __ATOMIC_RELAXED, __HIP_MEMORY_SCOPE_AGENT);
            }
            __builtin_amdgcn_fence(__ATOMIC_ACQUIRE, "agent");
            asm volatile("s_waitcnt vmcnt(0)" ::: "memory");
        }
        asm volatile("s_waitcnt vmcnt(0) lgkmcnt(0)\n\ts_barrier" ::: "memory");
        float* const Ew = lds + E_OFF_DW;
        for (unsigned b2 = b + 1; b2 < G; ++b2) {
            const unsigned f0 = first_chunk(b2, G, p.units, p.nk, p.lmin);
            if (f0 >= tile_end) break;
            if (first_chunk(b2 + 1, G, p.units, p.nk, p.lmin) == f0) continue;
            const float* sl = p.slabs + (size_t)b2 * E_DW + e_row * BN + 4 * e_c4;
#pragma unroll 4
            for (int e = 0; e < PASSES; ++e) {
                f32x4* d = reinterpret_cast<f32x4*>(Ew + (8 * e + e_row) * BN + 4 * e_c4);
                *d += *reinterpret_cast<const f32x4*>(sl + 8 * e * BN);
            }
        }
        asm volatile("s_waitcnt lgkmcnt(0)" ::: "memory");
    }
#pragma unroll
    for (int e = 0; e < PASSES; ++e) {
        pass(e);
        if (e % 4 == 3) __builtin_amdgcn_sched_barrier(0);
    }
}

template <int P, bool CONV = false, int IO = 0, int LN = 0, bool DUAL = false>
__global__ __launch_bounds__(768, 3) void gemm_ws_kernel(Params p) {
    extern __shared__ __attribute__((aligned(1024))) float lds[];
    const int tid = threadIdx.x, lane = tid & 63;
    const int wave = __builtin_amdgcn_readfirstlane(tid >> 6);
    const unsigned G = gridDim.x, b = xcd_major_id(blockIdx.x, G);
    const bool split = p.flags != nullptr;
    unsigned u0, u1;
    if (split) {
        u0 = first_chunk(b, G, p.units, p.nk, p.lmin);
        u1 = first_chunk(b + 1, G, p.units, p.nk, p.lmin);
    } else {
        const unsigned cnt = b < p.tiles ? (p.tiles - b + G - 1) / G : 0;
        u0 = b * p.rr_cnt * (unsigned)p.nk;
        u1 = u0 + cnt * (unsigned)p.nk;
    }
    const int n_chunks = (int)(u1 - u0);
    if (n_chunks == 0) return;
    const unsigned t0 = u0 / (unsigned)p.nk;
    const int kc0 = (int)(u0 - t0 * (unsigned)p.nk);
    if (wave < 4) {
        if (IO == 0) matrix_role(p, lds, kc0, n_chunks, wave, lane);
        else matrix_role16(p, lds, kc0, n_chunks, wave, lane);
    } else {
        if (!(DBG & 8)) __builtin_amdgcn_s_setprio(3);
        if (wave < 8) loader_role<CONV, IO != 0>(p, lds, t0, kc0, n_chunks, tid - 256);
        else epilogue_role<P, IO == 1, LN, DUAL>(p, lds, b, G, u0, u1, tid - 512);
    }
}

inline bool eligible(int64_t M, int N, int K) {
    return K % BK == 0 && K >= 3 * BK && N % 4 == 0 && M >= 1 && M * (int64_t)K * 4 < (1ll << 31) &&
           (int64_t)N * K * 4 < (1ll << 31) && M * (int64_t)N * 4 < (1ll << 31);
}

struct Conv { int H, W, C, kh, kw; };
inline bool conv_eligible(int64_t M, int N, const Conv& c) {
    const int64_t K = (int64_t)c.kh * c.kw * c.C;
    return c.C % BK == 0 && c.kh * c.kw <= 32 && K >= 3 * BK && K < (1 << 24) && N % 4 == 0 && M >= 1 && c.W >= 2 && c.H * (int64_t)c.W < (1 << 30) &&
           M * (int64_t)c.C * 4 < (1ll << 31) && (int64_t)N * K * 4 < (1ll << 31) && M * (int64_t)N * 4 < (1ll << 31);
}
inline void magic_div(unsigned d, unsigned& magic, unsigned& shift) {
    unsigned s = 0;
    while ((1ull << s) < d) ++s;
    magic = (unsigned)(((1ull << (31 + s)) + d - 1) / d);
    shift = s - 1;
}

inline int64_t workspace_bytes(int num_cu) { return 4096 + (int64_t)num_cu * E_DW * 4; }

struct LnArgs {
    float* stats_out;
    const float* ln_stats;
    const float* ln_colsum;
    int ln_gn, ln_C;
    float ln_eps;
};

inline unsigned base_params(Params& p, const void* x, const void* W, const float* bias, const float* residual, void* y, int64_t M,
                            int N, int K, int act, int tile, int chunk, unsigned slots) {
    p.X = static_cast<const float*>(x); p.W = static_cast<const float*>(W); p.bias = bias; p.residual = residual;
    p.Y = static_cast<float*>(y);
    p.M = (int)M; p.N = N; p.K = K; p.act = act; p.nk = K / chunk;
    p.gm = (unsigned)((M + tile - 1) / tile); p.gn = (unsigned)((N + tile - 1) / tile);
    p.tiles = p.gm * p.gn;
    p.units = p.tiles * (unsigned)p.nk;
    p.st_w = (p.gn % 4 == 0) ? 4u : (p.gn % 2 == 0) ? 2u : 1u;
    const unsigned grid = p.tiles < slots ? p.tiles : slots;
    p.rr_G = grid;
    p.rr_cnt = (p.tiles + grid - 1) / grid;
    return grid;
}

inline int passes_per_chunk(int passes, int nk) {
    const int need = (passes + nk - 2) / (nk - 1);
    return need <= 1 ? 1 : need <= 2 ? 2 : need <= 4 ? 4 : 8;
}

template <int PMAX = 8, class F>
inline int with_passes(int P, F&& f) {
    if (P == 1) return f(std::integral_constant<int, 1>{});
    if (P == 2) return f(std::integral_constant<int, 2>{});
    if (PMAX == 4 || P == 4) return f(std::integral_constant<int, 4>{});
    return f(std::integral_constant<int, PMAX>{});
}

template <auto Kernel>
inline int launch_ws(unsigned grid, int lds_bytes, int max_lds, hipStream_t s, const Params& p, const char* who = "gemm_ws") {
    static bool attr_set = false;
    if (!attr_set) {
        hipError_t e = hipFuncSetAttribute(reinterpret_cast<const void*>(Kernel), hipFuncAttributeMaxDynamicSharedMemorySize, max_lds);
        if (e != hipSuccess) { set_error("%s: cannot reserve %d B of LDS: %s", who, max_lds, hipGetErrorString(e)); return (int)e; }
        attr_set = true;
    }
    hipLaunchKernelGGL(Kernel, dim3(grid), dim3(768), lds_bytes, s, p);
    return 0;
}

inline int launch(const float* x, const float* W, const float* bias, const float* residual, float* y, int64_t M, int N,
                  int K, int act, int num_cu, hipStream_t s, void* ws = nullptr, int64_t ws_bytes = 0, int force_split = -1,
                  void* stamps = nullptr, bool ws_clean = false, const Conv* cv = nullptr, const LnArgs* ln = nullptr,
                  float* dual_z = nullptr) {
    Params p;
    unsigned grid = base_params(p, x, W, bias, dual_z ? dual_z : residual, y, M, N, K, act, BM, BK, (unsigned)num_cu);
    if (ln) {
        p.stats_out = ln->stats_out; p.ln_stats = ln->ln_stats; p.ln_colsum = ln->ln_colsum;
        p.ln_gn = ln->ln_gn; p.ln_C = ln->ln_C; p.ln_eps = ln->ln_eps;
        if (ln->ln_stats && ws && ws_bytes >= 4096) p.ln_guard = static_cast<unsigned*>(ws) + LN_GUARD_WORD;
    }
    const int ln_mode = !ln ? 0 : (ln->stats_out ? 1 : 2);
    if (cv) {
        p.cv_H = cv->H; p.cv_W = cv->W; p.cv_C = cv->C; p.cv_kh = cv->kh; p.cv_kw = cv->kw; p.cv_cpc = cv->C / BK;
        magic_div((unsigned)(cv->H * cv->W), p.cv_mhw, p.cv_shw);
        magic_div((unsigned)cv->W, p.cv_mw, p.cv_sw);
    }
#ifdef MUMPY_WS_STAMP
    p.stamps = static_cast<unsigned long long*>(stamps);
#endif
    int P = passes_per_chunk(PASSES, p.nk);
    const double rounds = (double)p.tiles / num_cu;
    const double eff = rounds / (double)((p.tiles + num_cu - 1) / num_cu);
    bool split = ws && ws_bytes >= workspace_bytes(num_cu) && eff < 0.93 && p.units >= 16u * (unsigned)num_cu;
    if (force_split >= 0) split = force_split && ws && ws_bytes >= workspace_bytes(num_cu);
    if (split && P < 4) P = 4;
    p.lmin = 1 + PASSES / P;
    p.walk = (grid == 256u && !split && tune_int("MUMPY_WS_WALK", 0)) ? 1u : 0u;
    if (split) {
        p.rr_cnt = 0;
        grid = (unsigned)num_cu;
        p.flags = static_cast<unsigned*>(ws);
        p.slabs = reinterpret_cast<float*>(static_cast<char*>(ws) + 4096);
        if (!ws_clean) {
            hipError_t e = hipMemsetAsync(p.flags, 0, 4096, s);
            if (e != hipSuccess) { set_error("gemm_ws: flag reset failed: %s", hipGetErrorString(e)); return (int)e; }
        }
    }
    g_route = Route{};
    g_route.family = Route::WS; g_route.addr = cv ? Route::CONV : Route::DENSE;
    g_route.split = split; g_route.passes = (uint8_t)P; g_route.ln = (uint8_t)ln_mode; g_route.dual = dual_z ? 1 : 0;
    return with_passes(P, [&](auto pc) {
        constexpr int PC = decltype(pc)::value;
        if (dual_z) return launch_ws<gemm_ws_kernel<PC, false, 0, 0, true>>(grid, LDS_BYTES, LDS_BYTES, s, p);
        if (cv) return launch_ws<gemm_ws_kernel<PC, true>>(grid, LDS_BYTES, LDS_BYTES, s, p);
        if (ln_mode == 1) return launch_ws<gemm_ws_kernel<PC, false, 0, 1>>(grid, LDS_BYTES, LDS_BYTES, s, p);
        if (ln_mode == 2) return launch_ws<gemm_ws_kernel<PC, false, 0, 2>>(grid, LDS_BYTES, LDS_BYTES, s, p);
        return launch_ws<gemm_ws_kernel<PC>>(grid, LDS_BYTES, LDS_BYTES, s, p);
    });
}

inline bool eligible16(int64_t M, int N, int K) {
    return K % 64 == 0 && K >= 192 && N % 4 == 0 && M >= 1 && M * (int64_t)K * 2 < (1ll << 31) && (int64_t)N * K * 2 < (1ll << 31) &&
           M * (int64_t)N * 4 < (1ll << 31);
}

inline int launch16(const void* x16, const void* W16, const float* bias, const float* residual, void* y, int64_t M, int N, int K,
                    int act, bool out_bf16, int num_cu, hipStream_t s) {
    Params p;
    const unsigned grid = base_params(p, x16, W16, bias, residual, y, M, N, K, act, BM, 64, (unsigned)num_cu);
    const int P = passes_per_chunk(PASSES, p.nk);
    p.lmin = 1 + PASSES / P;
    g_route = Route{};
    g_route.family = Route::WS16; g_route.passes = (uint8_t)P;
    return with_passes(P, [&](auto pc) {
        constexpr int PC = decltype(pc)::value;
        if (out_bf16) return launch_ws<gemm_ws_kernel<PC, false, 1>>(grid, LDS_BYTES, LDS_BYTES, s, p);
        return launch_ws<gemm_ws_kernel<PC, false, 2>>(grid, LDS_BYTES, LDS_BYTES, s, p);
    });
}

}
}
```

### multilateral-temporal-view-pyramid-transformer-for-video-inpainting-detection_amd/csrc/gemm_ws64.h

```cpp
#pragma once
#include "gemm_ws.h"

namespace mumpy {
namespace gemm_ws64 {

using gemm_ws::BK;
using gemm_ws::OOB;
using gemm_ws::Params;
using gemm_ws::tile_coords;
using gemm_ws::u32x4;
using gemm_ws::ws_barrier;

constexpr int T = 64;
constexpr int STAGE_DW = 2 * T * BK;
constexpr int NSTAGE = 3;
constexpr int E_DW = T * T;
constexpr int E_OFF_DW = NSTAGE * STAGE_DW;
constexpr int LDS_BYTES = (E_OFF_DW + E_DW) * 4;
constexpr int PASSES = 4;

__device__ __forceinline__ void matrix_role(const Params& p, float* lds, int n_chunks, int wave, int lane) {
    const int c = lane & 31, h = lane >> 5, wm = wave >> 1, wn = wave & 1;
    const int sw = (c >> 1) & 7;
    int a_off[4], b_off[4];
#pragma unroll
    for (int q = 0; q < 4; ++q) {
        a_off[q] = (32 * wm + c) * BK + 4 * ((4 * h + q) ^ sw);
        b_off[q] = (T + 32 * wn + c) * BK + 4 * ((4 * h + q) ^ sw);
    }
    float* const E = lds + E_OFF_DW + (32 * wm + 4 * h) * T + 32 * wn + c;
    f32x16 acc;
    f32x4 fa0, fb0, fa1, fb1;
    auto rd = [&](const float* st, int q, f32x4& fa, f32x4& fb) {
        fa = *reinterpret_cast<const f32x4*>(st + a_off[q]);
        fb = *reinterpret_cast<const f32x4*>(st + b_off[q]);
    };
    auto mm = [&](const f32x4& fa, const f32x4& fb, int e) { acc = __builtin_amdgcn_mfma_f32_32x32x2f32(fa[e], fb[e], acc, 0, 0, 0); };
    auto mm4 = [&](const f32x4& fa, const f32x4& fb) {
#pragma unroll
        for (int e = 0; e < 4; ++e) mm(fa, fb, e);
    };
    auto dump = [&]() {
#pragma unroll
        for (int r = 0; r < 16; ++r) E[((r & 3) + 8 * (r >> 2)) * T] = acc[r];
    };
    auto zero = [&]() {
#pragma unroll
        for (int r = 0; r < 16; ++r) acc[r] = 0.f;
    };
    zero();
    ws_barrier();
    rd(lds, 0, fa0, fb0);
    int kc = 0, stage = 0;
    for (int i = 0; i < n_chunks; ++i) {
        const float* st = lds + stage * STAGE_DW;
        stage = stage == NSTAGE - 1 ? 0 : stage + 1;
        if (kc == 0 && i > 0) { dump(); zero(); }
        __builtin_amdgcn_sched_barrier(0);
        rd(st, 1, fa1, fb1);
        mm4(fa0, fb0);
        __builtin_amdgcn_sched_group_barrier(0x008, 1, 0);
        __builtin_amdgcn_sched_group_barrier(0x100, 2, 0);
        __builtin_amdgcn_sched_group_barrier(0x008, 3, 0);
        rd(st, 2, fa0, fb0);
        mm4(fa1, fb1);
        __builtin_amdgcn_sched_group_barrier(0x008, 1, 0);
        __builtin_amdgcn_sched_group_barrier(0x100, 2, 0);
        __builtin_amdgcn_sched_group_barrier(0x008, 3, 0);
        rd(st, 3, fa1, fb1);
        mm4(fa0, fb0);
        __builtin_amdgcn_sched_group_barrier(0x008, 1, 0);
        __builtin_amdgcn_sched_group_barrier(0x100, 2, 0);
        __builtin_amdgcn_sched_group_barrier(0x008, 3, 0);
        mm(fa1, fb1, 0);
        mm(fa1, fb1, 1);
        __builtin_amdgcn_sched_barrier(0);
        ws_barrier();
        __builtin_amdgcn_sched_barrier(0);
        rd(lds + stage * STAGE_DW, 0, fa0, fb0);
        mm(fa1, fb1, 2);
        mm(fa1, fb1, 3);
        __builtin_amdgcn_sched_barrier(0);
        if (++kc == p.nk) kc = 0;
    }
    dump();
    ws_barrier();
}

__device__ __forceinline__ void loader_role(const Params& p, float* lds, unsigned tile0, int n_chunks, int hl) {
    const int lane = hl & 63, lw = __builtin_amdgcn_readfirstlane(hl >> 6);
    const int prow = lane >> 3;
    uint32_t aoff[2], boff[2];
    auto set_tile = [&](unsigned t) {
        unsigned tm, tn;
        tile_coords(p, t, tm, tn);
#pragma unroll
        for (int q = 0; q < 2; ++q) {
            const int r = 32 * q + 8 * lw + prow;
            const uint32_t ch = (uint32_t)((lane & 7) ^ ((r >> 1) & 7));
            int m = (int)tm * T + r;
            if (m > p.M - 1) m = p.M - 1;
            aoff[q] = (uint32_t)m * (uint32_t)p.K * 4u + 16u * ch;
            int n = (int)tn * T + r;
            if (n > p.N - 1) n = p.N - 1;
            boff[q] = (uint32_t)n * (uint32_t)p.K * 4u + 16u * ch;
        }
    };
    const auto rs_x = __builtin_amdgcn_make_buffer_rsrc(const_cast<float*>(p.X), 0, (int)0x7fffffff, 0x00020000);
    const auto rs_w = __builtin_amdgcn_make_buffer_rsrc(const_cast<float*>(p.W), 0, (int)0x7fffffff, 0x00020000);
    typedef __attribute__((address_space(3))) void* lptr_t;
    auto dma = [&](int kc, int stage) {
        const int so = kc * 128;
        float* st = lds + stage * STAGE_DW + 8 * lw * BK;
#pragma unroll
        for (int q = 0; q < 2; ++q)
            __builtin_amdgcn_raw_ptr_buffer_load_lds(rs_x, (lptr_t)(st + 32 * q * BK), 16, aoff[q], so, 0, 0);
#pragma unroll
        for (int q = 0; q < 2; ++q)
            __builtin_amdgcn_raw_ptr_buffer_load_lds(rs_w, (lptr_t)(st + (T + 32 * q) * BK), 16, boff[q], so, 0, 0);
    };
    unsigned ld_tile = tile0;
    int ld_kc = 0, ld_idx = 0;
    auto advance = [&]() {
        if (ld_idx + 1 < n_chunks) {
            ++ld_idx;
            if (++ld_kc == p.nk) { ld_kc = 0; ++ld_tile; set_tile(ld_tile); }
        }
    };
    set_tile(ld_tile);
    dma(ld_kc, 0);
    advance();
    dma(ld_kc, 1);
    advance();
    asm volatile("s_waitcnt vmcnt(4)" ::: "memory");
    ws_barrier();
    int stage = 2;
    for (int i = 0; i < n_chunks; ++i) {
        dma(ld_kc, stage);
        advance();
        stage = stage == NSTAGE - 1 ? 0 : stage + 1;
        asm volatile("s_waitcnt vmcnt(4)" ::: "memory");
        ws_barrier();
    }
    asm volatile("s_waitcnt vmcnt(0)" ::: "memory");
    ws_barrier();
}

template <int P>
__device__ __forceinline__ void epilogue_role(const Params& p, float* lds, unsigned v0, unsigned n_tiles, int hl) {
    const float* const E = lds + E_OFF_DW;
    const int e_row = hl >> 4, e_c4 = hl & 15;
    const int nk = p.nk;
    const auto rs_y = __builtin_amdgcn_make_buffer_rsrc(p.Y, 0, (int)((int64_t)p.M * p.N * 4), 0x00020000);
    const auto rs_r = __builtin_amdgcn_make_buffer_rsrc(const_cast<float*>(p.residual ? p.residual : p.Y), 0,
                                                        p.residual ? (int)((int64_t)p.M * p.N * 4) : 0, 0x00020000);
    const auto rs_b = __builtin_amdgcn_make_buffer_rsrc(const_cast<float*>(p.bias ? p.bias : p.Y), 0, p.bias ? p.N * 4 : 0, 0x00020000);
    constexpr int STEPS = PASSES / P;
    f32x4 rv[PASSES], bias4;
    uint32_t yo[PASSES];
    const uint32_t row16 = 16u * (uint32_t)p.N * 4u;
    auto begin_tile = [&](unsigned t) {
        unsigned tm, tn;
        tile_coords(p, t, tm, tn);
        const int n = (int)tn * T + 4 * e_c4;
        const uint32_t ybase = n < p.N ? (((uint32_t)tm * T + e_row) * (uint32_t)p.N + (uint32_t)n) * 4u : OOB;
#pragma unroll
        for (int e = 0; e < PASSES; ++e) {
            yo[e] = ybase + (uint32_t)e * row16;
            rv[e] = __builtin_bit_cast(f32x4, __builtin_amdgcn_raw_buffer_load_b128(rs_r, yo[e], 0, 0));
        }
        bias4 = __builtin_bit_cast(f32x4, __builtin_amdgcn_raw_buffer_load_b128(rs_b, n < p.N ? (uint32_t)n * 4u : OOB, 0, 0));
    };
    auto pass = [&](int e) {
        f32x4 v = *reinterpret_cast<const f32x4*>(E + (16 * e + e_row) * T + 4 * e_c4) + bias4;
        if (p.act == MUMPY_ACT_GELU) {
#pragma unroll
            for (int x = 0; x < 4; ++x) v[x] = gelu_erf(v[x]);
        }
        v += rv[e];
        __builtin_amdgcn_raw_buffer_store_b128(__builtin_bit_cast(u32x4, v), rs_y, yo[e], 0, 0);
    };
    ws_barrier();
    for (int c = 0; c < nk; ++c) ws_barrier();
    for (unsigned t = 1; t < n_tiles; ++t) {
        begin_tile(v0 + t - 1);
        ws_barrier();
#pragma unroll
        for (int st = 0; st < STEPS; ++st) {
#pragma unroll
            for (int k = 0; k < P; ++k) pass(st * P + k);
            ws_barrier();
        }
        for (int c = 1 + STEPS; c < nk; ++c) ws_barrier();
    }
    begin_tile(v0 + n_tiles - 1);
    ws_barrier();
#pragma unroll
    for (int e = 0; e < PASSES; ++e) pass(e);
}

template <int P>
__global__ __launch_bounds__(768, 6) void gemm_ws64_kernel(Params p) {
    extern __shared__ __attribute__((aligned(1024))) float lds[];
    const int tid = threadIdx.x, lane = tid & 63;
    const int wave = __builtin_amdgcn_readfirstlane(tid >> 6);
    const unsigned G = gridDim.x, b = xcd_major_id(blockIdx.x, G);
    const unsigned cnt = b < p.tiles ? (p.tiles - b + G - 1) / G : 0;
    if (cnt == 0) return;
    const unsigned v0 = b * p.rr_cnt;
    const int n_chunks = (int)cnt * p.nk;
    if (wave < 4) matrix_role(p, lds, n_chunks, wave, lane);
    else {
        __builtin_amdgcn_s_setprio(3);
        if (wave < 8) loader_role(p, lds, v0, n_chunks, tid - 256);
        else epilogue_role<P>(p, lds, v0, cnt, tid - 512);
    }
}

inline bool eligible(int64_t M, int N, int K) { return gemm_ws::eligible(M, N, K); }

inline int launch(const float* x, const float* W, const float* bias, const float* residual, float* y, int64_t M, int N, int K,
                  int act, int num_cu, hipStream_t s, int per_cu = 2) {
    Params p;
    const unsigned grid = gemm_ws::base_params(p, x, W, bias, residual, y, M, N, K, act, T, BK, (unsigned)per_cu * (unsigned)num_cu);
    const int P = gemm_ws::passes_per_chunk(PASSES, p.nk);
    const int lds_bytes = per_cu == 1 ? 2 * LDS_BYTES + 1024 : LDS_BYTES;
    g_route = Route{};
    g_route.family = Route::WS64; g_route.passes = (uint8_t)(P > 4 ? 4 : P);
    return gemm_ws::with_passes<4>(P, [&](auto pc) {
        return gemm_ws::launch_ws<gemm_ws64_kernel<decltype(pc)::value>>(grid, lds_bytes, 2 * LDS_BYTES + 1024, s, p, "gemm_ws64");
    });
}

}
}
```

### multilateral-temporal-view-pyramid-transformer-for-video-inpainting-detection_amd/models/encoder/multiTemporalViewEncoder.py

```python
import torch
import torch.nn as nn

from models.modules.blocks import Block
from models.modules.dct import FAF
from models.modules.deformableAttention import SwinDAttention
from models.modules.layers import Derived, DropPath, refuse_stochastic_depth, to_2tuple, trunc_normal_
from models.modules.swinTransformer import Mlp, SwinTransformerBlock, ThreeViewPatchMerging, WindowAttention
from mumpy_hip import ops
from mumpy_hip.streams import run_parallel


class CVAModule(nn.Module):
    def __init__(self, dim1, num_heads, window_size=7, temporal_dims=[], qkv_bias=True, qk_scale=None, drop=0.0,
                 attn_drop=0.0, drop_path=0.0, cur_stage=0):
        super().__init__()
        self.crossattn = SwinDAttention(dim1, num_heads, attn_drop, n_groups=3)
        self.drop_path = DropPath(drop_path) if drop_path > 0.0 else nn.Identity()

    def forward(self, x1, x2, mask=None, return_attention=False):
        if return_attention:
            return self.crossattn(x1, x2, return_attention=True)[1]
        y, _ = self.crossattn(x1, x2)
        return ops.add(x1, y), None


class CrossSwinBlock(nn.Module):
    def __init__(self, dim1, dim2, input_resolution, num_heads, window_size=7, shift_size=0, mlp_ratio=4.0, qkv_bias=True,
                 qk_scale=None, drop=0.0, attn_drop=0.0, drop_path=0.0, act_layer=nn.GELU, norm_layer=nn.LayerNorm,
                 fused_window_process=False, last_view=False, temporal_dims=1, cur_stage=0):
        super().__init__()
        if shift_size != 0:
            raise NotImplementedError("cross blocks are always un-shifted (mTVE:310,323,336)")
        self.dim, self.input_resolution, self.num_heads = dim1, tuple(input_resolution), num_heads
        self.window_size = min(window_size, min(self.input_resolution))
        self.shift_size, self.mlp_ratio = 0, mlp_ratio
        self.last_view, self.temporal_dims, self.cur_stage = last_view, temporal_dims, cur_stage
        self.norm1 = norm_layer(dim1)
        self.attn = WindowAttention(dim1, to_2tuple(self.window_size), num_heads, qkv_bias, qk_scale, attn_drop, drop)
        self.drop_path = DropPath(drop_path) if drop_path > 0.0 else nn.Identity()
        self.norm2 = norm_layer(dim1)
        self.mlp = Mlp(dim1, int(dim1 * mlp_ratio), act_layer=act_layer, drop=drop)
        if last_view:
            self.pre, self.cva = nn.Identity(), nn.Identity()
        else:
            self.pre = nn.Linear(dim2, dim1)
            trunc_normal_(self.pre.weight, std=0.02)
            nn.init.zeros_(self.pre.bias)
            self.cva = CVAModule(dim1, num_heads, to_2tuple(self.window_size), temporal_dims, qkv_bias, qk_scale, drop,
                                 attn_drop, drop_path, cur_stage)
        self.register_buffer("attn_mask", None)

    def msa(self, x1, need_out=True):
        h, w = self.input_resolution
        b, l1, c1 = x1.shape
        if self.training:
            refuse_stochastic_depth(self)
        if ops.storage() == "bf16":
            from models.modules.swinTransformer import _w16
            a = self.attn.attend(ops.layernorm_bf16(x1, self.norm1.weight, self.norm1.bias, self.norm1.eps), b, l1 // w, w, 0, None)
            out = ops.linear_bf16s(a, _w16(self.attn, "proj"), self.attn.proj.bias, out_bf16=False)
            return ops.add(x1, out), out
        a = self.attn.attend(ops.layernorm(x1, self.norm1.weight, self.norm1.bias, self.norm1.eps), b, l1 // w, w, 0, None)
        if not need_out:
            return ops.linear(a, self.attn.proj.weight, self.attn.proj.bias, residual=x1), None
        out = ops.linear(a, self.attn.proj.weight, self.attn.proj.bias)
        return ops.add(x1, out), out

    def prep(self, x1):
        if self.last_view:
            return None
        h, w = self.input_resolution
        b, l1, _ = x1.shape
        return self.cva.crossattn._prep(x1, (b, l1 // w, w))

    def tail(self, x1, x2, prep=None):
        h, w = self.input_resolution
        b, l1, c1 = x1.shape
        hs1 = l1 // w
        if not self.last_view:
            hs2 = x2.shape[1] // w
            x2p = ops.linear(x2, self.pre.weight, self.pre.bias)
            x1 = self.cva.crossattn.attend_combine(x1, x2p, b, hs1, w, hs2, prep)
        if ops.storage() == "bf16":
            return self.mlp.forward_bf16(ops.layernorm_bf16(x1, self.norm2.weight, self.norm2.bias, self.norm2.eps), x1)
        m = b * l1
        emit = ops.linear_ln_tiles(m, c1, self.mlp.fc2.in_features) > 0 and ops.linear_ln_tiles(m, 3 * c1, c1) > 0
        return self.mlp(ops.layernorm(x1, self.norm2.weight, self.norm2.bias, self.norm2.eps), residual=x1, emit_stats=emit)

    def forward(self, x1, x2):
        x1, out = self.msa(x1)
        return self.tail(x1, x2), out


class CrossThreeViewSwinBlock(nn.Module):
    def __init__(self, view_configs, input_resolution, cur_stage, mlp_ratio=4.0, qkv_bias=True, qk_scale=None, drop=0.0,
                 attn_drop=0.0, drop_path=0.0, norm_layer=nn.LayerNorm, fused_window_process=False):
        super().__init__()
        kw = dict(shift_size=0, mlp_ratio=mlp_ratio, qkv_bias=qkv_bias, qk_scale=qk_scale, drop=drop, attn_drop=attn_drop,
                  drop_path=drop_path, cur_stage=cur_stage)
        hid = [view_configs[v]["hidden_size"][cur_stage] for v in range(3)]
        heads = [view_configs[v]["num_heads"][cur_stage] for v in range(3)]
        ws = [view_configs[v]["window_size"] for v in range(3)]
        self.block1 = CrossSwinBlock(hid[0], hid[1], input_resolution[0], heads[0], window_size=ws[0],
                                     temporal_dims=view_configs[0]["temporal_ratio"], **kw)
        self.block2 = CrossSwinBlock(hid[1], hid[2], input_resolution[1], heads[1], window_size=ws[1],
                                     temporal_dims=view_configs[0]["temporal_ratio"], **kw)
        self.block3 = CrossSwinBlock(hid[2], hid[2], input_resolution[2], heads[2], window_size=ws[2], last_view=True,
                                     temporal_dims=3, **kw)

    def forward(self, x):
        from mumpy_hip import streams
        if streams.SERIAL:
            x3, out3 = self.block3(x[2], x[2])
            x2, out2 = self.block2(x[1], out3)
            x1, _ = self.block1(x[0], out2)
            return [x1, x2, x3]
        main = torch.cuda.current_stream()
        sa, sb = streams._side_stream(main.device, 0), streams._side_stream(main.device, 1)
        fork, e3, e2 = torch.cuda.Event(), torch.cuda.Event(), torch.cuda.Event()
        fork.record(main)
        streams._DEPTH[0] += 1
        try:
            x3a, out3 = self.block3.msa(x[2])
            e3.record(main)
            sa.wait_event(fork)
            x[1].record_stream(sa)
            with torch.cuda.stream(sa):
                x2a, out2 = self.block2.msa(x[1])
                e2.record(sa)
                prep2 = self.block2.prep(x2a)
                sa.wait_event(e3)
                out3.record_stream(sa)
                x2 = self.block2.tail(x2a, out3, prep2)
            sb.wait_event(fork)
            x[0].record_stream(sb)
            with torch.cuda.stream(sb):
                x1a, _ = self.block1.msa(x[0], need_out=False)
                prep1 = self.block1.prep(x1a)
                sb.wait_event(e2)
                out2.record_stream(sb)
                x1 = self.block1.tail(x1a, out2, prep1)
            x3 = self.block3.tail(x3a, None)
        finally:
            streams._DEPTH[0] -= 1
        main.wait_stream(sa)
        main.wait_stream(sb)
        x2.record_stream(main)
        x1.record_stream(main)
        return [x1, x2, x3]


class OriginalThreeViewSwinBlock(nn.Module):
    def __init__(self, view_configs, input_resolution, cur_stage, cur_lyr, mlp_ratio=4.0, qkv_bias=True, qk_scale=None,
                 drop=0.0, attn_drop=0.0, drop_path=0.0, norm_layer=nn.LayerNorm, fused_window_process=False):
        super().__init__()
        shift = 0 if cur_lyr % 2 == 0 else view_configs[0]["window_size"] // 2
        for v in range(3):
            if cur_lyr < view_configs[v]["depths"][cur_stage]:
                blk = SwinTransformerBlock(view_configs[v]["hidden_size"][cur_stage], input_resolution[v],
                                           view_configs[v]["num_heads"][cur_stage], view_configs[v]["window_size"], shift,
                                           mlp_ratio, qkv_bias, qk_scale, drop, attn_drop, drop_path,
                                           norm_layer=norm_layer, temporal_dim=view_configs[v]["temporal_dim"])
            else:
                blk = nn.Identity()
            setattr(self, f"block{v + 1}", blk)

    def forward(self, x):
        return [self.block1(x[0]), self.block2(x[1]), self.block3(x[2])]


class MultiViewBasicLayer(nn.Module):
    def __init__(self, view_configs, cur_stage, depth, mlp_ratio=4.0, qkv_bias=True, qk_scale=None, drop=0.0,
                 attn_drop=0.0, drop_path=0.0, norm_layer=nn.LayerNorm, downsample=None, fused_window_process=False):
        super().__init__()
        res = [view_configs[k]["input_resolution"][cur_stage] for k in range(3)]
        blocks = []
        for i in range(depth):
            dp = drop_path[i] if isinstance(drop_path, list) else drop_path
            kw = dict(mlp_ratio=mlp_ratio, qkv_bias=qkv_bias, qk_scale=qk_scale, drop=drop, attn_drop=attn_drop,
                      drop_path=dp, norm_layer=norm_layer)
            blocks.append(CrossThreeViewSwinBlock(view_configs, res, cur_stage, **kw) if i == 0 else
                          OriginalThreeViewSwinBlock(view_configs, res, cur_stage, i, **kw))
        self.blocks = nn.ModuleList(blocks)
        self.downsample = downsample(view_configs, cur_stage) if downsample is not None else None

    def _view_chain(self, v, x):
        for blk in self.blocks[1:]:
            x = getattr(blk, f"block{v + 1}")(x)
        out = x
        if self.downsample is not None:
            x = getattr(self.downsample, f"downsample{v + 1}")(x)
        return x, out

    def forward(self, x):
        x = self.blocks[0](x)
        def bg(v):
            from mumpy_hip import streams
            if streams.SERIAL:
                return self._view_chain(v, x[v])
            with ops.background():
                return self._view_chain(v, x[v])
        res = run_parallel([lambda: bg(0), lambda: bg(1), lambda: self._view_chain(2, x[2])], [(x[0],), (x[1],), (x[2],)])
        return [r[0] for r in res], [r[1] for r in res]


class CreateStages(nn.Module):
    def __init__(self, view_configs, depths=[2, 2, 18, 2], mlp_ratio=4.0, qkv_bias=True, qk_scale=None, stages=4,
                 drop_rate=0.0, attn_drop_rate=0.0, drop_path_rate=0.0, norm_layer=nn.LayerNorm, ape=False,
                 patch_norm=True, use_checkpoint=False, fused_window_process=False):
        super().__init__()
        dpr = torch.linspace(0, drop_path_rate, sum(depths)).tolist()
        self.layers = nn.ModuleList([
            MultiViewBasicLayer(view_configs, i, depths[i], mlp_ratio, qkv_bias, qk_scale, drop_rate, attn_drop_rate,
                                dpr[sum(depths[:i]):sum(depths[:i + 1])], norm_layer,
                                ThreeViewPatchMerging if i < stages - 1 else None)
            for i in range(stages)])

    def forward(self, x):
        outs = []
        for layer in self.layers:
            x, o = layer(x)
            outs.append(o)
        return x, outs


class CrossThreeViewTokenize(nn.Module):

    def __init__(self, view_configs):
        super().__init__()
        for v in range(3):
            size = view_configs[v]["patches"].size
            k = (size[-1], size[0], size[1])
            c = view_configs[v]["hidden_size"][0]
            setattr(self, f"project{v + 1}", nn.Conv3d(3, c, kernel_size=k, stride=k, padding=0))
        for v in range(3):
            setattr(self, f"norm{v + 1}", nn.LayerNorm(view_configs[v]["hidden_size"][0]))
        self._wt = [Derived(), Derived(), Derived()]

    def _view(self, v, x):
        proj, norm = getattr(self, f"project{v + 1}"), getattr(self, f"norm{v + 1}")
        w = proj.weight
        if tuple(w.shape[3:]) != (4, 4):
            raise NotImplementedError("tokenizer kernel is built for 4x4 spatial patches")
        wt = self._wt[v].get((w,), lambda: w.reshape(w.shape[0], -1).t().contiguous())
        return ops.patch_embed(x, wt, proj.bias, norm.weight, norm.bias, w.shape[2], norm.eps)

    def forward(self, x):
        return run_parallel([lambda: self._view(0, x), lambda: self._view(1, x), lambda: self._view(2, x)], [(x,), (x,), (x,)])


class CreateGlobalBlocks(nn.Module):
    def __init__(self, global_encoder_config, dpr, dropout_rate):
        super().__init__()
        g = global_encoder_config
        self.blocks = nn.ModuleList([Block(g["hidden_size"], g["num_heads"], g["mlp_dim"], dropout_rate, dpr[i])
                                     for i in range(g["num_layers"])])

    def forward(self, x, keep_t=None):
        last = len(self.blocks) - 1
        for i, blk in enumerate(self.blocks):
            x = blk(x, keep_t=keep_t) if (i == last and keep_t is not None) else blk(x)
        return x


class ThreeViewSwinTransformer(nn.Module):
    def __init__(self, view_configs, input_token_temporal_dims, global_encoder_config, depths=[2, 2, 18, 2], mlp_ratio=4.0,
                 qkv_bias=True, qk_scale=None, stages=4, drop_rate=0.0, attn_drop_rate=0.0, drop_path_rate=0.2,
                 norm_layer=nn.LayerNorm, ape=False, patch_norm=True, use_checkpoint=False, fused_window_process=False):
        super().__init__()
        self.faf = FAF()
        self.tokenize = CrossThreeViewTokenize(view_configs)
        self.input_token_temporal_dims = list(input_token_temporal_dims)
        self.layers = CreateStages(view_configs, depths, mlp_ratio, qkv_bias, qk_scale, stages, drop_rate, attn_drop_rate,
                                   drop_path_rate, norm_layer)
        self.pos_drop = nn.Dropout(p=drop_rate)
        self.globalembedding = nn.Linear(2560, 768)
        self.global_dpr = torch.linspace(0, drop_path_rate, global_encoder_config["num_layers"]).tolist()
        self.globalblocks = CreateGlobalBlocks(global_encoder_config, self.global_dpr, drop_rate)

    def merge_views_along_channel_axis(self, tokens):
        tmax = max(self.input_token_temporal_dims)
        parts = []
        for v, x in enumerate(tokens):
            b, l, c = x.shape
            t = self.input_token_temporal_dims[v]
            x = x.reshape(b, t, l // t, c)
            parts.append(x.expand(b, tmax, l // t, c) if t == 1 else x.repeat(1, tmax // t, 1, 1))
        return torch.cat(parts, dim=-1)

    def forward_stages(self, x):
        (ffinfo,), (views, stage_out) = run_parallel(
            [lambda: (self.faf.forward_frame(x, 1),), lambda: self.layers(self.tokenize(x))], [(x,), (x,)])
        return views, [[v.unsqueeze(1) for v in stage] for stage in stage_out], ffinfo

# ... 22 lines not shown
```

### multilateral-temporal-view-pyramid-transformer-for-video-inpainting-detection_amd/mumpy_hip/lib.py

```python
import ctypes
import os
import subprocess
from typing import NamedTuple

_HERE = os.path.dirname(os.path.abspath(__file__))
_PKG = os.path.dirname(_HERE)
_LIB = None

c_f = ctypes.c_void_p
c_i = ctypes.c_int
c_l = ctypes.c_int64
c_fl = ctypes.c_float
c_d = ctypes.c_double


class Surface(NamedTuple):
    header: str
    version_fn: str
    version: int
    signatures: dict


SURFACES = [
    Surface("mumpy_hip.h", "mumpy_abi_version", 2, {
# ... 11 lines not shown
        "mumpy_tuning_build": [],
        "mumpy_workspace_status": [c_f, ctypes.POINTER(ctypes.c_int)],
        "mumpy_linear_ln_tiles": [c_l, c_i, c_i],
        "mumpy_linear_lnx_fwd": [c_f, c_f, c_f, c_f, c_f, c_l, c_i, c_i, c_i, c_f, c_l, c_f, c_f, c_i, c_f, c_fl, c_f],
        "mumpy_linear_rows_fwd": [c_f, c_l, c_l, c_f, c_f, c_f, c_f, c_l, c_i, c_i, c_i, c_f, c_l, c_f],
        "mumpy_linear_rows_kseg_fwd": [c_f, c_l, c_l, c_i, c_i, c_f, c_f, c_f, c_f, c_l, c_i, c_i, c_i, c_f, c_l, c_f],
        "mumpy_gn_stats_nhwc_fwd": [c_f, c_f, c_i, c_l, c_i, c_i, c_i, c_f],
        "mumpy_gn_apply_resample_nhwc_fwd": [c_f, c_f, c_i, c_f, c_f, c_i, c_fl, c_i, c_i, c_i, c_i, c_i, c_f, c_f, c_f, c_i, c_i,
                                             c_i, c_i, c_i, c_i, c_f],
        "mumpy_conv2d_nhwc_fwd": [c_f, c_f, c_f, c_f, c_f, c_i, c_i, c_i, c_i, c_i, c_i, c_i, c_i, c_f, c_l, c_f],
        "mumpy_conv2d_workspace_bytes": [c_i, c_i, c_i, c_i, c_i, c_i, c_i],
        "mumpy_avgpool2_pad_nhwc_fwd": [c_f, c_f, c_i, c_i, c_i, c_i, c_i, c_i, c_f],
        "mumpy_copy_rows_fwd": [c_f, c_l, c_f, c_l, c_l, c_i, c_f],
        "mumpy_merge_views_fwd": [c_f, c_f, c_f, c_f, c_i, c_i, c_i, c_i, c_i, c_i, c_i, c_i, c_i, c_f],
        "mumpy_trunk_head_fwd": [c_f, c_f, c_f, c_f, c_f, c_i, c_i, c_i, c_i, c_f],
        "mumpy_final_conv_fwd": [c_f, c_f, c_f, c_f, c_f, c_i, c_i, c_i, c_i, c_fl, c_f],
        "mumpy_window_attention_fwd": [c_f, c_f, c_f, c_f, c_f, c_i, c_i, c_i, c_i, c_i, c_i, c_fl, c_f],
        "mumpy_deform_offsets_fwd": [c_f, c_f, c_f, c_f, c_f, c_f, c_f, c_i, c_i, c_i, c_i, c_f],
        "mumpy_deform_sample_fwd": [c_f, c_f, c_f, c_i, c_i, c_i, c_i, c_i, c_f],
        "mumpy_deform_attention_fwd": [c_f, c_f, c_f, c_f, c_i, c_i, c_i, c_i, c_i, c_fl, c_f],
        "mumpy_deform_sample_kv_fwd": [c_f, c_f, c_f, c_f, c_f, c_i, c_i, c_i, c_i, c_i, c_f],
        "mumpy_deform_out_combine_fwd": [c_f, c_f, c_f, c_f, c_f, c_i, c_i, c_i, c_i, c_f],
        "mumpy_deform_attention_mm16_fwd": [c_f, c_f, c_f, c_f, c_i, c_i, c_i, c_i, c_i, c_fl, c_f],
        "mumpy_window_attention_plan": [c_i, c_i, c_i, c_i],
        "mumpy_window_attention_bf16_plan": [c_i, c_i, c_i, c_i],
        "mumpy_deform_attention_plan": [c_i, c_i, c_i, c_i, c_i],
        "mumpy_deform_sample_kv_mm16_fwd": [c_f, c_f, c_f, c_f, c_f, c_i, c_i, c_i, c_i, c_i, c_f],
        "mumpy_deform_out_combine_mm16_fwd": [c_f, c_f, c_f, c_f, c_f, c_i, c_i, c_i, c_i, c_f],
        "mumpy_deform_combine_fwd": [c_f, c_f, c_f, c_i, c_i, c_i, c_i, c_f],
        "mumpy_faf_fwd": [c_f, c_f, c_f, c_f, c_f, c_i, c_i, c_i, c_i, c_i, c_i, c_f],
        "mumpy_patch_embed_fwd": [c_f, c_f, c_f, c_f, c_f, c_f, c_i, c_i, c_i, c_i, c_i, c_i, c_fl, c_f],
        "mumpy_patch_merge_ln_fwd": [c_f, c_f, c_f, c_f, c_i, c_i, c_i, c_i, c_fl, c_f],
        "mumpy_temporal_attention_fwd": [c_f, c_f, c_l, c_i, c_i, c_i, c_fl, c_f],
        "mumpy_attention_probs_fwd": [c_f, c_f, c_f, c_l, c_i, c_i, c_i, c_i, c_l, c_l, c_l, c_l, c_l, c_fl, c_f],
        "mumpy_temporal_attention_q_fwd": [c_f, c_f, c_l, c_i, c_i, c_i, c_i, c_fl, c_f],
        "mumpy_sigmoid_threshold_fwd": [c_f, c_f, c_l, c_fl, c_f],
        "mumpy_add_fwd": [c_f, c_f, c_f, c_l, c_f],
        "mumpy_normalize_u8_fwd": [c_f, c_f, c_l, c_i, c_i, ctypes.POINTER(ctypes.c_float), ctypes.POINTER(ctypes.c_float), c_f],
        "mumpy_resize_nearest_table": [c_i, c_i, ctypes.POINTER(ctypes.c_int32)],
        "mumpy_resize_normalize_u8_fwd": [c_f, c_f, c_f, c_f, c_l, c_i, c_i, c_i, c_i, ctypes.POINTER(ctypes.c_float), ctypes.POINTER(ctypes.c_float), c_f],
        "mumpy_mask_loss_workspace_bytes": [c_i, c_l],
        "mumpy_mask_loss_fwd_bwd": [c_f, c_f, c_f, c_f, c_f, c_l, c_i, c_l, c_fl, c_fl, c_f],
        "mumpy_layernorm_bwd_workspace_bytes": [c_l, c_i],
        "mumpy_layernorm_bwd": [c_f, c_f, c_f, c_f, c_f, c_f, c_f, c_f, c_l, c_l, c_i, c_fl, c_i, c_f],
        "mumpy_gelu_fwd": [c_f, c_f, c_l, c_f],
        "mumpy_gelu_bwd": [c_f, c_f, c_f, c_l, c_f],
        "mumpy_transpose_fwd": [c_f, c_f, c_l, c_l, c_f],
        "mumpy_col_sum_workspace_bytes": [c_l, c_i],
        "mumpy_col_sum_fwd": [c_f, c_f, c_f, c_l, c_l, c_i, c_f],
        "mumpy_final_conv_bwd_workspace_bytes": [c_i, c_i, c_i],
        "mumpy_final_conv_bwd": [c_f, c_f, c_f, c_f, c_f, c_f, c_f, c_l, c_i, c_i, c_i, c_i, c_f],
        "mumpy_patch_gather_fwd": [c_f, c_f, c_l, c_i, c_i, c_i, c_i, c_f],
        "mumpy_conv_weight_dgrad_fwd": [c_f, c_f, c_i, c_i, c_i, c_i, c_f],
        "mumpy_conv2d_wgrad_workspace_bytes": [c_i, c_i, c_i, c_i, c_i, c_i, c_i],
        "mumpy_conv2d_wgrad_nhwc": [c_f, c_f, c_f, c_i, c_i, c_i, c_i, c_i, c_i, c_i, c_i, c_f, c_l, c_f],
        "mumpy_linear_bwd_workspace_bytes": [c_l, c_i, c_i],
        "mumpy_linear_bwd": [c_f, c_f, c_f, c_f, c_f, c_f, c_l, c_i, c_i, c_i, c_f, c_l, c_f],
        "mumpy_window_attention_bwd_workspace_bytes": [c_i, c_i, c_i, c_i],
        "mumpy_window_attention_bwd": [c_f, c_f, c_f, c_f, c_f, c_i, c_f, c_f, c_f, c_f, c_l, c_i, c_i, c_i, c_i, c_i, c_fl, c_i, c_f],
        "mumpy_window_attention_bwd_csr": [c_f, c_f, c_f, c_f, c_f, c_i, c_f, c_f, c_f, c_f, c_f, c_l, c_i, c_i, c_i, c_i, c_i, c_fl, c_i, c_f],
        "mumpy_window_attention_mm16_fwd": [c_f, c_f, c_f, c_f, c_f, c_i, c_i, c_i, c_i, c_i, c_i, c_fl, c_f],
        "mumpy_window_attention_mm16_bwd_workspace_bytes": [c_i, c_i, c_i, c_i],
        "mumpy_window_attention_mm16_bwd": [c_f, c_f, c_f, c_f, c_f, c_i, c_f, c_f, c_f, c_f, c_f, c_l, c_i, c_i, c_i, c_i, c_i, c_fl, c_i, c_f],
        "mumpy_relpos_bias_expand_fwd": [c_f, c_f, c_f, c_i, c_f],
        "mumpy_gn_bwd_workspace_bytes": [c_i, c_l, c_i],
        "mumpy_gn_bwd_nhwc": [c_f, c_f, c_i, c_f, c_f, c_f, c_f, c_f, c_f, c_f, c_l, c_i, c_l, c_i, c_i, c_fl, c_i, c_f],
        "mumpy_upsample_bwd_nhwc": [c_f, c_f, c_i, c_i, c_i, c_i, c_i, c_i, c_f],
        "mumpy_temporal_attention_bwd": [c_f, c_f, c_f, c_l, c_i, c_i, c_i, c_fl, c_f],
        "mumpy_scale_samples_fwd": [c_f, c_f, c_f, c_i, c_l, c_f],
        "mumpy_dwconv5_window_fwd": [c_f, c_f, c_f, c_f, c_l, c_i, c_f],
        "mumpy_dwconv5_window_bwd_workspace_bytes": [c_l, c_i],
        "mumpy_dwconv5_window_bwd": [c_f, c_f, c_f, c_f, c_f, c_f, c_f, c_l, c_l, c_i, c_f],
        "mumpy_deform_attention_bwd_workspace_bytes": [c_l, c_i],
        "mumpy_deform_attention_bwd": [c_f, c_f, c_f, c_f, c_f, c_f, c_l, c_l, c_i, c_i, c_fl, c_f],
        "mumpy_deform_sample_bwd": [c_f, c_f, c_f, c_f, c_f, c_l, c_i, c_i, c_f],
        "mumpy_adamw_hyper": [ctypes.POINTER(ctypes.c_float), c_d, c_d, c_d, c_d, c_d, c_i, c_d],
        "mumpy_adamw_step_dev": [c_f, c_f, c_f, c_f, c_l, c_f, c_f],
        "mumpy_adamw_step": [c_f, c_f, c_f, c_f, c_l, c_d, c_d, c_d, c_d, c_d, c_i, c_d, c_f],
        "mumpy_sgd_step": [c_f, c_f, c_f, c_l, c_d, c_d, c_d, c_d, c_i, c_d, c_f],
        "mumpy_sgd_hyper": [ctypes.POINTER(ctypes.c_float), c_d, c_d, c_d, c_d, c_i, c_d],
        "mumpy_sgd_step_dev": [c_f, c_f, c_f, c_l, c_f, c_i, c_f],
        "mumpy_rmsprop_step": [c_f, c_f, c_f, c_f, c_l, c_d, c_d, c_d, c_d, c_d, c_d, c_f],
        "mumpy_rmsprop_hyper": [ctypes.POINTER(ctypes.c_float), c_d, c_d, c_d, c_d, c_d, c_d],
        "mumpy_rmsprop_step_dev": [c_f, c_f, c_f, c_f, c_l, c_f, c_f],
        "mumpy_grad_norm_partials": [c_l],
        "mumpy_grad_norm_partial": [c_f, c_l, c_f, c_f],
        "mumpy_grad_norm_finish": [c_f, c_f, c_f, c_f, c_i, c_i, c_d, c_f, c_f],
    }),
    Surface("mumpy_hip_ext.h", "mumpy_ext_version", 1, {
        "mumpy_adamw_gate_hyper": [ctypes.POINTER(ctypes.c_double), c_d, c_d, c_d, c_i],
        "mumpy_update_gate": [c_f, c_i, c_f, c_f, c_f, c_i, c_f, c_f, c_f],
        "mumpy_adamw_step_gated_dev": [c_f, c_f, c_f, c_f, c_l, c_f, c_f, c_f],
        "mumpy_sgd_step_gated_dev": [c_f, c_f, c_f, c_l, c_f, c_i, c_f, c_f],
        "mumpy_rmsprop_step_gated_dev": [c_f, c_f, c_f, c_f, c_l, c_f, c_f, c_f],
    }),
    Surface("mumpy_hip_ext2.h", "mumpy_ext2_version", 2, {
        "mumpy_deform_attention_mm16_bwd_workspace_bytes": [c_l, c_i, c_i],
        "mumpy_deform_attention_mm16_bwd": [c_f, c_f, c_f, c_f, c_f, c_f, c_l, c_l, c_i, c_i, c_fl, c_f],
        "mumpy_linear_gelu_dual_fwd": [c_f, c_f, c_f, c_f, c_f, c_l, c_i, c_i, c_i, c_f, c_l, c_f],
        "mumpy_linear_gelu_bwd_workspace_bytes": [c_l, c_i, c_i],
        "mumpy_linear_gelu_bwd": [c_f, c_f, c_f, c_f, c_f, c_f, c_f, c_l, c_i, c_i, c_i, c_f, c_l, c_f],
    }),
    Surface("mumpy_hip_ext3.h", "mumpy_ext3_version", 1, {
        "mumpy_augment_stage_u8_fwd": [c_f, c_f, c_f, c_f, c_f, c_f, c_f, c_l, c_i, c_l, c_i, c_i, c_i, ctypes.POINTER(ctypes.c_float),
                                       ctypes.POINTER(ctypes.c_float), c_f],
    }),
    Surface("mumpy_hip_ext4.h", "mumpy_ext4_version", 1, {
        "mumpy_augment_warp_u8_fwd": [c_f, c_f, c_f, c_f, c_f, c_f, c_f, c_f, c_f, c_f, c_f, c_f, c_f, c_l, c_i, c_l, c_i, c_i, c_i,
                                      ctypes.POINTER(ctypes.c_float), ctypes.POINTER(ctypes.c_float), c_f],
    }),
    Surface("mumpy_hip_ext5.h", "mumpy_ext5_version", 1, {
        "mumpy_clip_window_u8_fwd": [c_f, c_f, c_f, c_f, c_f, c_l, c_i, c_l, c_i, c_i, c_i, c_i, ctypes.POINTER(ctypes.c_float),
                                     ctypes.POINTER(ctypes.c_float), c_f],
        "mumpy_mask_score_u8_fwd": [c_f, c_f, c_f, c_f, c_f, c_l, c_l, c_l, c_f],
        "mumpy_frame_metrics_fwd": [c_f, c_l, c_l, c_f, c_i, c_f],
    }),
    Surface("mumpy_hip_ext6.h", "mumpy_ext6_version", 1, {
        "mumpy_resize_bilinear_u8_fwd": [c_f, c_f, c_f, c_f, c_f, c_f, c_f, c_f, c_l, c_i, c_i, c_i, c_i, c_i, c_i, c_f],
    }),
    Surface("mumpy_hip_ext7.h", "mumpy_ext7_version", 1, {
        "mumpy_score_exceed_fwd": [c_f, c_f, c_f, c_f, c_f, c_l, c_l, c_l, c_i, c_f],
        "mumpy_sweep_metrics_fwd": [c_f, c_l, c_l, c_i, c_f, c_f, c_i, c_f],
    }),
    Surface("mumpy_hip_ext8.h", "mumpy_ext8_version", 1, {
        "mumpy_deform_sample_grouped_fwd": [c_f, c_f, c_f, c_i, c_i, c_i, c_i, c_i, c_i, c_f],
        "mumpy_deform_sample_kv_grouped_fwd": [c_f, c_f, c_f, c_f, c_f, c_i, c_i, c_i, c_i, c_i, c_i, c_f],
        "mumpy_deform_sample_kv_mm16_grouped_fwd": [c_f, c_f, c_f, c_f, c_f, c_i, c_i, c_i, c_i, c_i, c_i, c_f],
        "mumpy_deform_attention_grouped_fwd": [c_f, c_f, c_f, c_f, c_i, c_i, c_i, c_i, c_i, c_fl, c_i, c_f],
        "mumpy_deform_attention_mm16_grouped_fwd": [c_f, c_f, c_f, c_f, c_i, c_i, c_i, c_i, c_i, c_fl, c_i, c_f],
    }),
    Surface("mumpy_hip_ext9.h", "mumpy_ext9_version", 1, {
        "mumpy_deform_sample_grouped_bwd": [c_f, c_f, c_f, c_f, c_f, c_l, c_i, c_i, c_i, c_f],
        "mumpy_deform_attention_grouped_bwd": [c_f, c_f, c_f, c_f, c_f, c_f, c_l, c_l, c_i, c_i, c_fl, c_i, c_f],
        "mumpy_deform_attention_mm16_grouped_bwd": [c_f, c_f, c_f, c_f, c_f, c_f, c_l, c_l, c_i, c_i, c_fl, c_i, c_f],
    }),
    Surface("mumpy_hip_ext10.h", "mumpy_ext10_version", 1, {
        "mumpy_faf_bwd": [c_f, c_f, c_f, c_f, c_f, c_i, c_i, c_i, c_i, c_f],
        "mumpy_tokenize_dx": [c_f, c_f, c_f, c_f, c_f, c_i, c_i, c_i, c_i, c_i, c_i, c_i, c_i, c_i, c_i, c_i, c_f],
        "mumpy_pgd_step": [c_f, c_f, c_f, c_l, c_l, c_fl, ctypes.POINTER(ctypes.c_float), ctypes.POINTER(ctypes.c_float),
                           ctypes.POINTER(ctypes.c_float), c_f],
    }),
]
ABI_VERSION = SURFACES[0].version
SIGNATURES = {name: args for s in SURFACES for name, args in s.signatures.items()}

PERTURB = Surface("mumpy_perturb.h", "mumpy_perturb_version", 1, {
    "mumpy_jpeg_roundtrip_workspace_bytes": [c_l, c_i, c_i],
    "mumpy_jpeg_roundtrip_u8_fwd": [c_f, c_f, c_f, c_f, c_f, c_l, c_l, c_i, c_i, c_i, c_f],
    "mumpy_gaussian_blur_workspace_bytes": [c_l, c_i, c_i],
    "mumpy_gaussian_blur_u8_fwd": [c_f, c_f, c_f, c_f, c_l, c_l, c_i, c_i, c_f],
    "mumpy_resize_nearest_u8_fwd": [c_f, c_f, c_f, c_f, c_l, c_i, c_i, c_i, c_i, c_i, c_f],
})


def library_path() -> str:
    if "MUMPY_HIP_LIB" in os.environ:
        return os.environ["MUMPY_HIP_LIB"]
    name = "libmumpy_hip_tuning.so" if os.environ.get("MUMPY_TUNING", "0") == "1" else "libmumpy_hip.so"
    return os.path.join(_PKG, "lib", name)


def tuning_library_path() -> str:
    return os.path.join(_PKG, "lib", "libmumpy_hip_tuning.so")


def build_library(verbose: bool = False) -> str:
    r = subprocess.run(["make", "-C", os.path.join(_PKG, "csrc"), "-j8", "all", "tuning"], capture_output=True, text=True)
    if verbose or r.returncode:
        print(r.stdout[-4000:], r.stderr[-4000:])
    if r.returncode:
        raise RuntimeError("building libmumpy_hip.so failed (see output above)")
    return library_path()


def load_library():
    global _LIB
    if _LIB is not None:
        return _LIB
    path = library_path()
    if not os.path.exists(path):
        raise RuntimeError(
            f"libmumpy_hip.so not found at {path}: the HIP kernels are the only implementation of this package "
            "(no CPU/torch fallback). Build it with `python __graft_entry__.py` or `make -C <pkg>/csrc`.")
    lib = ctypes.CDLL(path)
    lib.mumpy_last_error.restype = ctypes.c_char_p
    lib.mumpy_last_route.restype = ctypes.c_char_p
    lib.mumpy_last_route.argtypes = []
    for s in SURFACES + [PERTURB]:
        version = getattr(lib, s.version_fn)
        version.restype, version.argtypes = c_i, []
        if version() != s.version:
            raise RuntimeError(f"{path}: {s.version_fn}() is {version()}, the binding of include/{s.header} expects {s.version}; rebuild")
        for name, args in s.signatures.items():
            fn = getattr(lib, name)
            fn.argtypes = args
            fn.restype = c_l if name.endswith("_bytes") else c_i
    _LIB = lib
    return lib
```

### multilateral-temporal-view-pyramid-transformer-for-video-inpainting-detection_amd/mumpy_hip/ops.py

```python
import math
import os
from typing import Optional

import torch

from .lib import load_library

ACT_NONE, ACT_GELU = 0, 1
MATH_FP32, MATH_BF16, MATH_BF16X3, MATH_BF16X2 = 0, 0x100, 0x200, 0x400
_MATH = MATH_FP32
_WS_BYTES = {}


def set_matrix_math(mode: str) -> None:
    global _MATH
    if mode not in _MODES:
        raise ValueError(f"unknown matrix math mode {mode!r}")
    _MATH = _MODES[mode]


_MODES = {"fp32": MATH_FP32, "bf16": MATH_BF16, "bf16x3": MATH_BF16X3, "bf16x2": MATH_BF16X2}


def matrix_math() -> str:
# ... 149 lines not shown
    return _ATTN_MATH


def set_cva_math(mode: str) -> None:
    global _CVA_MATH
    _CVA_MATH = _choice(mode, _CVA_MATHS, _CVA_WHAT)


def cva_math() -> str:
    return _CVA_MATH


def set_clip_coupling(mode: str) -> None:
    global _CLIP_COUPLING
    _CLIP_COUPLING = _choice(mode, _COUPLINGS, _COUPLING_WHAT)


def clip_coupling() -> str:
    return _CLIP_COUPLING


class clip_coupling_as:

    def __init__(self, mode: Optional[str]):
        self.mode = _choice(mode, (None,) + _COUPLINGS, _COUPLING_WHAT)

    def __enter__(self):
        self.prev = _CLIP_COUPLING
        if self.mode is not None:
            set_clip_coupling(self.mode)
        return self

    def __exit__(self, *exc):
        set_clip_coupling(self.prev)
        return False


def cva_pairing(nkv: int, nq: int, groups: int = 1):
    import numpy as np
    nkv, nq, groups = int(nkv), int(nq), int(groups)
    if nq < 1 or nkv < 1 or nkv % nq:
        raise ValueError(f"cva_pairing: {nkv} kv windows are not a positive multiple of {nq} q windows")
    if groups < 1 or nq % groups:
        raise ValueError(f"cva_pairing: groups={groups} must be at least 1 and divide the {nq} q windows")
    r, nqg = nkv // nq, nq // groups
    i = np.arange(nkv, dtype=np.int64)
    g = i // (r * nqg)
    return g * nqg + (i - g * r * nqg) % nqg, i // r


def cva_pairing_members(nkv: int, nq: int, groups: int = 1):
    import numpy as np
    nkv, nq, groups = int(nkv), int(nq), int(groups)
    if nq < 1 or nkv < 1 or nkv % nq:
        raise ValueError(f"cva_pairing_members: {nkv} kv windows are not a positive multiple of {nq} q windows")
    if groups < 1 or nq % groups:
        raise ValueError(f"cva_pairing_members: groups={groups} must be at least 1 and divide the {nq} q windows")
    r, nqg = nkv // nq, nq // groups
    qw = np.arange(nq, dtype=np.int64)[:, None]
    g = qw // nqg
    return g * (r * nqg) + (qw - g * nqg) + np.arange(r, dtype=np.int64)[None, :] * nqg


def set_mlp_fusion(on: bool) -> None:
    global _MLP_FUSED
    if not isinstance(on, (bool, int)) or on not in (0, 1):
        raise ValueError(f"set_mlp_fusion: expected a bool, got {on!r}")
    _MLP_FUSED = bool(on)


def mlp_fusion() -> bool:
    return _MLP_FUSED


def _mm16(entry, math):
    return entry.replace("_fwd", "_mm16_fwd") if _choice(math, _CVA_MATHS, _CVA_WHAT) == "bf16" else entry


def _window_attention(entry, chk, dtype, who, qkv, bias_pad, b, hs, w, c, shift, scale, mask_tab, mask_id, out=None):
    qkv = chk(qkv, "qkv")
    if qkv.numel() != b * hs * w * 3 * c:
        raise RuntimeError(f"{who}: qkv shape mismatch")
    out = torch.empty(b, hs * w, c, device=qkv.device, dtype=dtype) if out is None else _chk_exact(out, "out", dtype, (b, hs * w, c), who)
    bias_pad = _rd(bias_pad, "bias", (c // 32) * 64 * 64, who)
    mask_tab, mask_id, n_mask = _chk_mask(mask_tab, mask_id, b * (hs // 7) * (w // 7), who)
    _call(entry, _p(qkv), _p(out), _p(bias_pad), _p(mask_tab), _p(mask_id), n_mask,
          b, hs, w, c, shift, scale, _stream(), work=307328.0 * b * (hs // 7) * (w // 7) * (c // 32))
    return out


def _chk_mask(mask_tab, mask_id, nwin, who):
    if mask_id is None:
        if mask_tab is not None:
            raise RuntimeError(f"mumpy_hip: {who}: mask_tab needs mask_id")
        return None, None, 0
    n_mask = mask_id.numel()
    if n_mask < 1 or nwin % n_mask:
        raise RuntimeError(f"mumpy_hip: {who}: {n_mask} mask ids do not divide the {nwin} windows of the launch")
    mask_id = _rd(mask_id, "mask_id", n_mask, who, torch.int32)
    if mask_tab is None or mask_tab.numel() < 4096 or mask_tab.numel() % 4096:
        raise RuntimeError(f"mumpy_hip: {who} needs mask_tab (nU, 64, 64) with mask_id")
    return _rd(mask_tab, "mask_tab", mask_tab.numel(), who), mask_id, n_mask


def window_attention_bf16(qkv16, bias_pad, b, hs, w, c, shift, scale, mask_tab=None, mask_id=None, math=None):
    math = _ATTN_MATH if math is None else _choice(math, _ATTN_MATHS, _ATTN_WHAT)
    return _window_attention("mumpy_window_attention_bf16mm_fwd" if math == "bf16" else "mumpy_window_attention_bf16_fwd", _chk16,
                             torch.bfloat16, "window_attention_bf16", qkv16, bias_pad, b, hs, w, c, shift, scale, mask_tab, mask_id)


def layernorm(x, gamma, beta, eps=1e-5, out=None):
    x = _chk(x, "x")
    c = x.shape[-1]
    gamma, beta = _rd(gamma, "gamma", c, "layernorm"), _rd(beta, "beta", c, "layernorm")
    if out is None:
        out = torch.empty_like(x)
    else:
        _drop_ln_stats(_wr(out, "out", x.numel(), "layernorm"))
    _call("mumpy_layernorm_fwd", _p(x), _p(gamma), _p(beta), _p(out), x.numel() // c, c,
          eps, _stream(), work=8.0 * x.numel())
    return out


def linear(x, weight, bias=None, act=ACT_NONE, residual=None, out=None, emit_stats=False):
    x = _chk(x, "x")
    weight = _chk(weight, "weight")
    n, k = weight.shape[0], weight.numel() // weight.shape[0]
    if x.shape[-1] != k:
        raise RuntimeError(f"linear: x has {x.shape[-1]} features, weight expects {k}")
    m = x.numel() // k
    if out is None:
        out = torch.empty(*x.shape[:-1], n, device=x.device, dtype=torch.float32)
    else:
        _drop_ln_stats(_wr(out, "out", m * n, "linear"))
    residual, bias = _rd_opt(residual, "residual", m * n, "linear"), _rd_opt(bias, "bias", n, "linear")
    if _in_background():
        _call("mumpy_linear_rd_fwd", _p(x), _p(weight), _p(bias), _p(residual), _p(out), m, n, k,
              act, _stream(), work=2.0 * m * n * k)
        return out
    wsb = _ws_bytes((m, n, k), "mumpy_linear_workspace_bytes", m, n, k)
    if emit_stats:
        gn = linear_ln_tiles(m, n, k) if k >= LN_FOLD_MIN_K else 0
        if gn:
            stats = torch.empty(m, gn, 2, device=x.device, dtype=torch.float32)
            ws = _kept_workspace(max(wsb, 4096), x.device)
            _call("mumpy_linear_lnx_fwd", _p(x), _p(weight), _p(bias), _p(residual), _p(out), m, n, k,
                  act, _p(ws), ws.numel() * 4, _p(stats), None, 0, None, 0.0, _stream(), work=2.0 * m * n * k)
            out._mumpy_ln_stats = stats
            return out
    ws = _kept_workspace(wsb, x.device) if wsb else None
    _call("mumpy_linear_wsz_fwd", _p(x), _p(weight), _p(bias), _p(residual),
          _p(out), m, n, k, act | _MATH, _p(ws), 0 if ws is None else ws.numel() * 4, _stream(), work=2.0 * m * n * k)
    return out


_BACKGROUND = [0]
BACKGROUND_ON = os.environ.get("MUMPY_BACKGROUND", "0") == "1"


class background:

    def __enter__(self):
        _BACKGROUND[0] += 1
        return self

    def __exit__(self, *exc):
        _BACKGROUND[0] -= 1
        return False


def _in_background():
    return _BACKGROUND[0] > 0 and BACKGROUND_ON and _MATH == MATH_FP32 and _STORAGE == "fp32"


LN_FOLD = os.environ.get("MUMPY_LN_FOLD", "1") != "0"
LN_FOLD_MIN_K = 512
_LN_TILES = {}


def linear_ln_tiles(m, n, k):
    if not LN_FOLD or _MATH != MATH_FP32 or _STORAGE != "fp32":
        return 0
    key = (m, n, k)
    t = _LN_TILES.get(key)
    if t is None:
        t = _LN_TILES[key] = int(_lib().mumpy_linear_ln_tiles(m, n, k))
    return t


def ln_stats_of(x):
    return getattr(x, "_mumpy_ln_stats", None)


def linear_ln(x, stats, wg, colsum, bprime, eps, act=ACT_NONE):
    x, wg = _chk(x, "x"), _chk(wg, "wg")
    n, k = wg.shape
    if x.shape[-1] != k:
        raise RuntimeError(f"linear_ln: x has {x.shape[-1]} features, wg expects {k}")
    m = x.numel() // k
    if stats.dim() != 3 or stats.shape[0] != m or stats.shape[2] != 2 or stats.shape[1] < 1:
        raise RuntimeError(f"linear_ln: stats must be ({m}, tiles, 2), got {tuple(stats.shape)}")
    stats, colsum, bprime = _rd(stats, "stats", stats.numel(), "linear_ln"), _rd(colsum, "colsum", n, "linear_ln"), _rd(bprime, "bprime", n, "linear_ln")
    out = torch.empty(*x.shape[:-1], n, device=x.device, dtype=torch.float32)
    wsb = _ws_bytes((m, n, k), "mumpy_linear_workspace_bytes", m, n, k)
    ws = _kept_workspace(max(wsb, 4096), x.device)
    _call("mumpy_linear_lnx_fwd", _p(x), _p(wg), _p(bprime), None, _p(out), m, n, k, act, _p(ws), ws.numel() * 4, None,
          _p(stats), stats.shape[-2], _p(colsum), eps, _stream(), work=2.0 * m * n * k)
    return out


def fold_ln_weights(weight, bias, gamma, beta):
    w64 = weight.detach().double()
    wg = w64 * gamma.detach().double()[None, :]
    bp = w64 @ beta.detach().double()
    if bias is not None:
        bp = bp + bias.detach().double()
    return wg.float().contiguous(), wg.sum(1).float().contiguous(), bp.float().contiguous()


_KEPT_WS = {}
_RETIRED_WS = []


def _kept_workspace(nbytes, device):
    s = torch.cuda.current_stream(device)
    key = (str(device), s.cuda_stream)
    ws = _KEPT_WS.get(key)
    if ws is None or ws.numel() * 4 < nbytes:
        if torch.cuda.is_current_stream_capturing():
            return torch.zeros(nbytes // 4, device=device, dtype=torch.float32)
        if ws is not None:
            _RETIRED_WS.append(ws)
        ws = _KEPT_WS[key] = torch.zeros(max(nbytes // 4, 1024), device=device, dtype=torch.float32)
    return ws


def check_workspaces():
    import ctypes
    bad = []
    for key, ws in list(_KEPT_WS.items()):
        st = ctypes.c_int(0)
        rc = _lib().mumpy_workspace_status(ws.data_ptr(), ctypes.byref(st))
        if rc:
            raise RuntimeError(f"mumpy_workspace_status failed (rc={rc}): {_lib().mumpy_last_error().decode()}")
        if st.value == -1:
            global LN_FOLD
            LN_FOLD = False
            ws.view(torch.int32)[1022] = 0
            import warnings
            warnings.warn("mumpy_hip: a folded LayerNorm met a row with |mean| > 256 sigma; LayerNorm folding is now off "
                          "(ops.LN_FOLD = False) -- re-capture any hipGraph to apply it")
        elif st.value:
            bad.append((key, st.value))
    if bad:
        reset_workspaces()
        raise RuntimeError(f"mumpy_hip: split GEMM launch(es) timed out waiting for a partial tile {bad}; results since the last "
                           "check are invalid (workspaces re-zeroed)")


def reset_workspaces():
    for ws in list(_KEPT_WS.values()) + _RETIRED_WS:
        ws.zero_()


def linear_rows(x_view, weight, bias=None, residual=None, out=None):
    if not x_view.is_cuda or x_view.dtype != torch.float32:
        raise RuntimeError("mumpy_hip: linear_rows needs a float32 GPU tensor (there is no CPU path)")
    nblk, rows, k = x_view.shape
    if x_view.stride(2) != 1 or x_view.stride(1) != k:
        raise RuntimeError("linear_rows: rows of a block must be contiguous")
    weight = _chk(weight, "weight")
    n = weight.shape[0]
    if weight.numel() != n * k:
        raise RuntimeError(f"linear_rows: x has {k} features, weight {tuple(weight.shape)}")
    m = nblk * rows
    bias, residual = _rd_opt(bias, "bias", n, "linear_rows"), _rd_opt(residual, "residual", m * n, "linear_rows")
    if out is None:
        out = torch.empty(m, n, device=x_view.device, dtype=torch.float32)
    else:
        _drop_ln_stats(_wr(out, "out", m * n, "linear_rows"))
    wsb = _ws_bytes((m, n, k), "mumpy_linear_workspace_bytes", m, n, k)
    ws = torch.empty(wsb // 4, device=x_view.device, dtype=torch.float32) if wsb else None
    _call("mumpy_linear_rows_fwd", _p(x_view), rows, x_view.stride(0), _p(weight),
          _p(bias), _p(residual), _p(out), m, n, k, ACT_NONE | _MATH, _p(ws), wsb, _stream(),
          work=2.0 * m * n * k)
    return out


def linear_time_slices(x4, weight, bias=None, residual=None):
    x4, weight = _chk(x4, "x"), _chk(weight, "weight")
    b, t, n, c = x4.shape
    nout, k = weight.shape
    if k != t * c or c % 32:
        raise RuntimeError(f"linear_time_slices: weight expects K = T*C = {t * c} (got {k}); C % 32 == 0")
    m = b * n
    out = torch.empty(m, nout, device=x4.device, dtype=torch.float32)
    residual, bias = _rd_opt(residual, "residual", m * nout, "linear_time_slices"), _rd_opt(bias, "bias", nout, "linear_time_slices")
    wsb = _ws_bytes((m, nout, k), "mumpy_linear_workspace_bytes", m, nout, k)
    ws = torch.empty(wsb // 4, device=x4.device, dtype=torch.float32) if wsb else None
    _call("mumpy_linear_rows_kseg_fwd", _p(x4), n, t * n * c, c, n * c, _p(weight), _p(bias),
          _p(residual), _p(out), m, nout, k, ACT_NONE | _MATH, _p(ws), wsb, _stream(), work=2.0 * m * nout * k)
    return out


def conv2d_nhwc(x, w_krsc, bias=None, act=ACT_NONE, residual=None):
    x = _nhwc(x, "x")
# ... 1409 lines not shown
```

Measured before the change: 384.6 clips/s.

## Fold cross-view pre projection into attention proj via split-output GEMM

Composes each block's `pre` linear with the preceding view's attention output projection into one weight (W_pre·W_proj), then concatenates it with the proj weight. A single GEMM writes two column-split outputs: the residual-added block output and the pre-projected handover tensor for the next view. This removes a separate `pre` linear launch and its re-read of the projection output on the cross-view critical path. The cost is a wider GEMM, a new COLS2 epilogue in the tiled, ws and ws64 kernels, and composed weights whose rounding differs slightly from running the two linears in sequence.

```diff
diff --git a/include/mumpy_linear_split.h b/include/mumpy_linear_split.h
--- /dev/null
+++ b/include/mumpy_linear_split.h
@@ -0,0 +1,19 @@
+#ifndef MUMPY_LINEAR_SPLIT_H
+#define MUMPY_LINEAR_SPLIT_H
+
+#include "mumpy_hip.h"
+
+#ifdef __cplusplus
+extern "C" {
+#endif
+
+#define MUMPY_LINEAR_SPLIT_VERSION 1
+int mumpy_linear_split_version(void);
+
+int mumpy_linear_split_fwd(const float* x, const float* W, const float* bias, const float* residual, float* y0, float* y1, int64_t M,
+                           int N0, int N1, int K, int act, void* workspace, int64_t workspace_bytes, void* stream);
+
+#ifdef __cplusplus
+}
+#endif
+#endif
diff --git a/multilateral-temporal-view-pyramid-transformer-for-video-inpainting-detection_amd/csrc/abi.cpp b/multilateral-temporal-view-pyramid-transformer-for-video-inpainting-detection_amd/csrc/abi.cpp
--- a/multilateral-temporal-view-pyramid-transformer-for-video-inpainting-detection_amd/csrc/abi.cpp
+++ b/multilateral-temporal-view-pyramid-transformer-for-video-inpainting-detection_amd/csrc/abi.cpp
@@ -13,6 +13,7 @@
 #include "../../include/mumpy_hip_ext9.h"
 #include "../../include/mumpy_hip_ext10.h"
 #include "../../include/mumpy_perturb.h"
+#include "../../include/mumpy_linear_split.h"
 
 namespace mumpy {
 static thread_local char g_err[512] = "";
@@ -52,6 +53,10 @@
         const size_t len = strlen(t);
         snprintf(t + len, n - len, r.family == Route::XGEMM ? " gate=gelu" : " dual=z");
     }
+    if (r.n1 && r.family != Route::NONE) {
+        const size_t len = strlen(t);
+        snprintf(t + len, n - len, " cols=%d+%d", r.n0, r.n1);
+    }
     return t;
 }
 #ifdef MUMPY_TUNING
@@ -84,5 +89,6 @@
 extern "C" int mumpy_ext9_version(void) { return MUMPY_EXT9_VERSION; }
 extern "C" int mumpy_ext10_version(void) { return MUMPY_EXT10_VERSION; }
 extern "C" int mumpy_perturb_version(void) { return MUMPY_PERTURB_VERSION; }
+extern "C" int mumpy_linear_split_version(void) { return MUMPY_LINEAR_SPLIT_VERSION; }
 extern "C" const char* mumpy_last_error(void) { return mumpy::g_err; }
 extern "C" const char* mumpy_last_route(void) { return mumpy::format_route(); }
diff --git a/multilateral-temporal-view-pyramid-transformer-for-video-inpainting-detection_amd/csrc/common.h b/multilateral-temporal-view-pyramid-transformer-for-video-inpainting-detection_amd/csrc/common.h
--- a/multilateral-temporal-view-pyramid-transformer-for-video-inpainting-detection_amd/csrc/common.h
+++ b/multilateral-temporal-view-pyramid-transformer-for-video-inpainting-detection_amd/csrc/common.h
@@ -38,6 +38,7 @@
     uint8_t reduce = R_NONE;
     uint8_t dual = 0;
     int ks = 1;
+    int n0 = 0, n1 = 0;
     struct { int wt, ks; } prod[2] = {{0, 0}, {0, 0}};
 };
 extern thread_local Route g_route;
diff --git a/multilateral-temporal-view-pyramid-transformer-for-video-inpainting-detection_amd/csrc/gemm.hip b/multilateral-temporal-view-pyramid-transformer-for-video-inpainting-detection_amd/csrc/gemm.hip
--- a/multilateral-temporal-view-pyramid-transformer-for-video-inpainting-detection_amd/csrc/gemm.hip
+++ b/multilateral-temporal-view-pyramid-transformer-for-video-inpainting-detection_amd/csrc/gemm.hip
@@ -2,6 +2,7 @@
 #include <type_traits>
 #include "common.h"
 #include "../../include/mumpy_hip_ext2.h"
+#include "../../include/mumpy_linear_split.h"
 #include "gemm_ws.h"
 #include "gemm_ws64.h"
 using namespace mumpy;
@@ -50,10 +51,10 @@
     return {dy, dx, (dy * cg.W + dx) * cg.Cin + c0};
 }
 
-template <int TM, int TN, int WM, int WN, bool OUT16 = false, bool DUAL = false>
+template <int TM, int TN, int WM, int WN, bool OUT16 = false, bool DUAL = false, bool COLS2 = false>
 __device__ __forceinline__ void store_tile(const f32x16 (&acc)[TM][TN], int64_t m0, int n0, int wm, int wn, int c, int h,
                                            int64_t M, int N, const float* __restrict__ bias, const float* residual,
-                                           float* Y, int act, int ksplit, int ks, float* slab) {
+                                           float* Y, int act, int ksplit, int ks, float* slab, float* Y1 = nullptr, int N0 = 0) {
     const int wm_u = __builtin_amdgcn_readfirstlane(wm), wn_u = __builtin_amdgcn_readfirstlane(wn);
     const int64_t mw = m0 + wm_u * WM;
     const int64_t wbase = mw * N + n0 + wn_u * WN;
@@ -71,6 +72,30 @@
                 for (int r = 0; r < 16; ++r) {
                     const int row = 32 * i + (r & 3) + 8 * (r >> 2);
                     if (row + 4 * h < rows_left) *reinterpret_cast<float*>(S + ((uint32_t)row * nb + lane_off + 128u * j)) = acc[i][j][r];
+                }
+        }
+        return;
+    }
+    if (COLS2) {
+        const int N1 = N - N0;
+#pragma unroll
+        for (int j = 0; j < TN; ++j) {
+            const int n = n0 + wn_u * WN + 32 * j + c;
+            if (n >= N) continue;
+            const float bv = bias ? bias[n] : 0.f;
+            const bool first = n < N0;
+            const int64_t pitch = first ? N0 : N1;
+            float* const yp = (first ? Y + n : Y1 + (n - N0)) + (mw + 4 * h) * pitch;
+            const float* const rp = (first && residual) ? residual + n + (mw + 4 * h) * pitch : nullptr;
+#pragma unroll
+            for (int i = 0; i < TM; ++i)
+#pragma unroll
+                for (int r = 0; r < 16; ++r) {
+                    const int row = 32 * i + (r & 3) + 8 * (r >> 2);
+                    if (row + 4 * h >= rows_left) continue;
+                    float v = acc[i][j][r] + bv;
+                    if (rp) v += rp[row * pitch];
+                    yp[row * pitch] = v;
                 }
         }
         return;
@@ -99,7 +124,7 @@
     }
 }
 
-template <int BM, int BN, int WM, int WN, bool CONV, bool GLDS, bool PIPE = true, bool DUAL = false>
+template <int BM, int BN, int WM, int WN, bool CONV, bool GLDS, bool PIPE = true, bool DUAL = false, bool COLS2 = false>
 __global__ __launch_bounds__(64 * (BM / WM) * (BN / WN), (BM * BN > 64 * 64) ? 2 : (CONV ? 3 : 4)) void linear_kernel(const float* __restrict__ X, const float* __restrict__ Wt,
                                                      const float* __restrict__ bias, const float* residual,
                                                      float* Y, int64_t M, int N, int K, int act, unsigned gn,
@@ -305,7 +330,9 @@
     }
     if (kc < nk) mma(afA, bfA);
     }
-    store_tile<TM, TN, WM, WN, false, DUAL>(acc, m0, n0, wm, wn, c, h, M, N, bias, residual, Y, act, ksplit, ks, slab);
+    static_assert(!COLS2 || (!CONV && !DUAL), "two outputs by column: a plain dense GEMM");
+    store_tile<TM, TN, WM, WN, false, DUAL, COLS2>(acc, m0, n0, wm, wn, c, h, M, N, bias, residual, Y, act, ksplit, ks, slab,
+                                                   COLS2 ? reinterpret_cast<float*>(bstride) : nullptr, COLS2 ? cg.H : 0);
 }
 
 typedef __bf16 bf16x8 __attribute__((ext_vector_type(8)));
@@ -511,6 +538,24 @@
     }
 }
 
+__global__ __launch_bounds__(256) void splitk_reduce_cols2_kernel(const float* __restrict__ slab, const float* __restrict__ bias,
+                                                                  const float* residual, float* Y, float* Y1, int64_t MN4, int N,
+                                                                  int N0, int ksplit) {
+    const int N1 = N - N0;
+    for (int64_t i = (int64_t)blockIdx.x * 256 + threadIdx.x; i < MN4; i += (int64_t)gridDim.x * 256) {
+        f32x4 v = ordered_sum(reinterpret_cast<const f32x4*>(slab)[i], reinterpret_cast<const f32x4*>(slab) + MN4 + i, MN4, ksplit - 1);
+        const int64_t m = (i * 4) / N;
+        const int n = (int)(i * 4 - m * N);
+        if (bias) v += *reinterpret_cast<const f32x4*>(bias + n);
+        if (n < N0) {
+            if (residual) v += *reinterpret_cast<const f32x4*>(residual + m * N0 + n);
+            *reinterpret_cast<f32x4*>(Y + m * N0 + n) = v;
+        } else {
+            *reinterpret_cast<f32x4*>(Y1 + m * N1 + (n - N0)) = v;
+        }
+    }
+}
+
 struct Plan {
     int tile;
     int ksplit;
@@ -620,6 +665,8 @@
     const ConvGeom* conv = nullptr;
     const gemm_ws::LnArgs* ln = nullptr;
     float* z = nullptr;
+    float* y1 = nullptr;
+    int n0 = 0;
 };
 
 struct TiledArgs {
@@ -668,6 +715,12 @@
     } else if (tile == 3) launch_tiled(linear_kernel<128, 128, 64, 64, false, true, false, true>, 256, t);
     else if (tile == 0) launch_tiled(linear_kernel<128, 128, 64, 32, false, false, true, true>, 512, t);
     else launch_tiled(linear_kernel<64, 64, 32, 32, false, false, true, true>, 256, t);
+}
+
+void launch_tiled_cols2(int tile, const TiledArgs& t) {
+    if (tile == 3) launch_tiled(linear_kernel<128, 128, 64, 64, false, true, false, false, true>, 256, t);
+    else if (tile == 0) launch_tiled(linear_kernel<128, 128, 64, 32, false, false, true, false, true>, 512, t);
+    else launch_tiled(linear_kernel<64, 64, 32, 32, false, false, true, false, true>, 256, t);
 }
 
 template <int NP, bool IN16 = false>
@@ -709,14 +762,14 @@
             const double r64 = (double)t64 / (2.0 * num_cu);
             const bool fits = ws64_mode == 2 || (act != MUMPY_ACT_GELU && nk <= 32 && t64 >= 64 && (r64 <= 1.0 || r64 >= 2.5 || nk <= 12));
             if (fits) {
-                if (int rc = gemm_ws64::launch(a.x, a.W, a.bias, a.residual, a.y, M, N, K, act, num_cu, a.s)) return rc;
+                if (int rc = gemm_ws64::launch(a.x, a.W, a.bias, a.residual, a.y, M, N, K, act, num_cu, a.s, 2, a.y1, a.n0)) return rc;
                 MUMPY_CHECK_LAUNCH("linear(ws64)");
                 return 0;
             }
         }
         if (how) {
             if (int rc = gemm_ws::launch(a.x, a.W, a.bias, a.residual, a.y, M, N, K, act, num_cu, a.s, ws, ws_bytes, how == 2 ? 1 : 0, nullptr,
-                                         a.ws_clean, conv ? &cvd : nullptr, a.ln, a.z)) return rc;
+                                         a.ws_clean, conv ? &cvd : nullptr, a.ln, a.z, a.y1, a.n0)) return rc;
             MUMPY_CHECK_LAUNCH("linear(ws)");
             return 0;
         }
@@ -728,18 +781,22 @@
         if (p.tile == 3) p.tile = 0;
         if (p.tile == 1) { p.tile = 2; p.gn = (unsigned)((N + 63) / 64); }
     }
-    if (a.z && p.tile == 1) { p.tile = 2; p.gn = (unsigned)((N + 63) / 64); }
+    if ((a.z || a.y1) && p.tile == 1) { p.tile = 2; p.gn = (unsigned)((N + 63) / 64); }
     const int64_t grid = p.gm * p.gn * p.ksplit;
     MUMPY_REQUIRE(grid < (1ll << 31), MUMPY_ERANGE, "linear: too many tiles");
     static const bool use_glds = tune_int("MUMPY_GEMM_GLDS", 0) != 0;
     const bool wide = (p.tile == 0 || p.tile == 3);
-    const TiledArgs t{a.x, a.W, a.bias, a.z ? a.z : a.residual, a.y, M, N, K, act, p.gn, p.ksplit, ws, rpb, bstride, cg, grid, a.s};
+    if (a.y1) cg.H = a.n0;
+    const TiledArgs t{a.x, a.W, a.bias, a.z ? a.z : a.residual, a.y, M, N, K, act, p.gn, p.ksplit, ws, rpb,
+                      a.y1 ? (int64_t)reinterpret_cast<intptr_t>(a.y1) : bstride, cg, grid, a.s};
     g_route = Route{};
     g_route.family = Route::TILED; g_route.tile = (uint8_t)p.tile; g_route.ks = p.ksplit;
     g_route.np = math_x2 ? 2 : math_x3 ? 3 : math_bf16 ? 1 : 0;
     g_route.addr = conv ? Route::CONV : a.kseg ? Route::KSEG : rpb < M ? Route::ROWS : Route::DENSE;
     g_route.dual = a.z ? 1 : 0;
-    if (a.z) launch_tiled_dual(p.tile, math_bf16, t);
+    if (a.y1) { g_route.n0 = a.n0; g_route.n1 = N - a.n0; }
+    if (a.y1) launch_tiled_cols2(p.tile, t);
+    else if (a.z) launch_tiled_dual(p.tile, math_bf16, t);
     else if (math_x2) launch_tiled_bf16<2>(wide, conv != nullptr, t);
     else if (math_x3) launch_tiled_bf16<3>(wide, conv != nullptr, t);
     else if (math_bf16) launch_tiled_bf16<1>(wide, conv != nullptr, t);
@@ -749,7 +806,9 @@
         const int64_t mn4 = M * N / 4;
         int64_t g = (mn4 + 255) / 256;
         if (g > 2048) g = 2048;
-        if (a.z) hipLaunchKernelGGL(splitk_reduce_kernel<true>, dim3((unsigned)g), dim3(256), 0, a.s, ws, a.bias, a.z, a.y, mn4, N, p.ksplit, act);
+        if (a.y1) hipLaunchKernelGGL(splitk_reduce_cols2_kernel, dim3((unsigned)g), dim3(256), 0, a.s, ws, a.bias, a.residual, a.y, a.y1, mn4, N,
+                                     a.n0, p.ksplit);
+        else if (a.z) hipLaunchKernelGGL(splitk_reduce_kernel<true>, dim3((unsigned)g), dim3(256), 0, a.s, ws, a.bias, a.z, a.y, mn4, N, p.ksplit, act);
         else hipLaunchKernelGGL(splitk_reduce_kernel<false>, dim3((unsigned)g), dim3(256), 0, a.s, ws, a.bias, a.residual, a.y, mn4, N,
                                 p.ksplit, act);
         MUMPY_CHECK_LAUNCH("linear(split-K reduce)");
@@ -875,6 +934,24 @@
     la.ws_clean = true;
     la.z = z;
     return launch_linear(la);
+}
+
+extern "C" int mumpy_linear_split_fwd(const float* x, const float* W, const float* bias, const float* residual, float* y0, float* y1,
+                                      int64_t M, int N0, int N1, int K, int act, void* workspace, int64_t workspace_bytes, void* stream) {
+    if (M == 0) return 0;
+    MUMPY_REQUIRE(y1, MUMPY_ENULL, "linear_split: null pointer");
+    MUMPY_REQUIRE(aligned16(y1) && aligned16(bias), MUMPY_EALIGN, "linear_split: pointers must be 16-byte aligned");
+    MUMPY_REQUIRE(act == 0, MUMPY_EINVAL, "linear_split: no activation and fp32 matrix math only (got act 0x%x)", act);
+    MUMPY_REQUIRE(N0 > 0 && N1 > 0 && N0 % 4 == 0 && N1 % 4 == 0 && N0 < (1 << 30) && N1 < (1 << 30), MUMPY_EINVAL,
+                  "linear_split: N0=%d and N1=%d must be positive multiples of 4", N0, N1);
+    if (int rc = check_linear_args("linear_split", x, W, residual, y0, M, N0 + N1, K, 0)) return rc;
+    MUMPY_REQUIRE(y0 != y1, MUMPY_EINVAL, "linear_split: y0 and y1 must be two buffers");
+    MUMPY_REQUIRE(workspace_bytes >= 0, MUMPY_EINVAL, "linear_split: workspace_bytes must not be negative");
+    MUMPY_REQUIRE(aligned16(workspace), MUMPY_EALIGN, "linear_split: workspace must be 16-byte aligned");
+    LinearArgs a = linear_args(x, W, bias, residual, y0, M, N0 + N1, K, 0, workspace, workspace_bytes, stream);
+    a.ws_clean = true;
+    a.y1 = y1; a.n0 = N0;
+    return launch_linear(a);
 }
 
 extern "C" int mumpy_workspace_status(const void* workspace, int* status) {
diff --git a/multilateral-temporal-view-pyramid-transformer-for-video-inpainting-detection_amd/csrc/gemm_ws.h b/multilateral-temporal-view-pyramid-transformer-for-video-inpainting-detection_amd/csrc/gemm_ws.h
--- a/multilateral-temporal-view-pyramid-transformer-for-video-inpainting-detection_amd/csrc/gemm_ws.h
+++ b/multilateral-temporal-view-pyramid-transformer-for-video-inpainting-detection_amd/csrc/gemm_ws.h
@@ -51,6 +51,8 @@
     int ln_gn = 0, ln_C = 0;
     float ln_eps = 0.f;
     unsigned* ln_guard = nullptr;
+    float* Y1 = nullptr;
+    int N0 = 0;
 #ifdef MUMPY_WS_STAMP
     unsigned long long* stamps = nullptr;
 #endif
@@ -375,22 +377,26 @@
 
 __device__ __forceinline__ float half_sum32(float x) { return wave_sum(x, 32); }
 
-template <int P, bool OUT16 = false, int LN = 0, bool DUAL = false>
+template <int P, bool OUT16 = false, int LN = 0, bool DUAL = false, bool COLS2 = false>
 __device__ __forceinline__ void epilogue_role(const Params& p, float* lds, unsigned b, unsigned G, unsigned u0, unsigned u1, int hl) {
     constexpr uint32_t OSZ = OUT16 ? 2u : 4u;
+    static_assert(!COLS2 || (!OUT16 && LN == 0 && !DUAL), "two outputs by column: plain fp32 epilogue only");
+    const int ny = COLS2 ? p.N0 : p.N;
     const float* const E = lds + E_OFF_DW;
     const int e_row = hl >> 5, e_c4 = hl & 31;
     const unsigned nk = (unsigned)p.nk;
     const bool split = p.flags != nullptr;
-    const auto rs_y = __builtin_amdgcn_make_buffer_rsrc(p.Y, 0, (int)((int64_t)p.M * p.N * OSZ), 0x00020000);
+    const auto rs_y = __builtin_amdgcn_make_buffer_rsrc(p.Y, 0, (int)((int64_t)p.M * ny * OSZ), 0x00020000);
+    const auto rs_y1 = __builtin_amdgcn_make_buffer_rsrc(COLS2 ? p.Y1 : p.Y, 0, COLS2 ? (int)((int64_t)p.M * (p.N - p.N0) * 4) : 0, 0x00020000);
     const auto rs_r = __builtin_amdgcn_make_buffer_rsrc(const_cast<float*>(p.residual ? p.residual : p.Y), 0,
-                                                        p.residual ? (int)((int64_t)p.M * p.N * 4) : 0, 0x00020000);
+                                                        p.residual ? (int)((int64_t)p.M * ny * 4) : 0, 0x00020000);
     const auto rs_b = __builtin_amdgcn_make_buffer_rsrc(const_cast<float*>(p.bias ? p.bias : p.Y), 0, p.bias ? p.N * 4 : 0, 0x00020000);
     const auto rs_s = __builtin_amdgcn_make_buffer_rsrc(split ? p.slabs + (size_t)b * E_DW : p.Y, 0, split ? E_DW * 4 : 0, 0x00020000);
     constexpr int STEPS = PASSES / P;
     f32x4 rv[PASSES], bias4;
     uint32_t yo[PASSES];
-    const uint32_t row8 = 8u * (uint32_t)p.N * OSZ;
+    uint32_t yo1[COLS2 ? PASSES : 1];
+    const uint32_t row8 = 8u * (uint32_t)ny * OSZ;
     const auto rs_st = __builtin_amdgcn_make_buffer_rsrc(LN == 1 ? p.stats_out : p.Y, 0, LN == 1 ? (int)((int64_t)p.M * p.gn * 8) : 0, 0x00020000);
     const auto rs_ln = __builtin_amdgcn_make_buffer_rsrc(const_cast<float*>(LN == 2 ? p.ln_stats : p.Y), 0,
                                                          LN == 2 ? (int)((int64_t)p.M * p.ln_gn * 8) : 0, 0x00020000);
@@ -405,7 +411,13 @@
         unsigned tm, tn;
         tile_coords(p, t, tm, tn);
         const int n = (int)tn * BN + 4 * e_c4;
-        const uint32_t ybase = n < p.N ? (((uint32_t)tm * BM + e_row) * (uint32_t)p.N + (uint32_t)n) * OSZ : OOB;
+        const uint32_t ybase = n < ny ? (((uint32_t)tm * BM + e_row) * (uint32_t)ny + (uint32_t)n) * OSZ : OOB;
+        if (COLS2) {
+            const uint32_t n1 = (uint32_t)(p.N - p.N0);
+            const uint32_t ybase1 = (n >= p.N0 && n < p.N) ? (((uint32_t)tm * BM + e_row) * n1 + (uint32_t)(n - p.N0)) * 4u : OOB;
+#pragma unroll
+            for (int e = 0; e < PASSES; ++e) yo1[e] = ybase1 + (uint32_t)e * (8u * n1 * 4u);
+        }
 #pragma unroll
         for (int e = 0; e < PASSES; ++e) {
             yo[e] = ybase + (uint32_t)e * row8;
@@ -473,6 +485,7 @@
             __builtin_amdgcn_raw_buffer_store_b64(__builtin_bit_cast(u32x2, o), rs_y, yo[e], 0, MUMPY_WS_STORE_AUX);
         } else {
             __builtin_amdgcn_raw_buffer_store_b128(__builtin_bit_cast(u32x4, v), rs_y, yo[e], 0, MUMPY_WS_STORE_AUX);
+            if (COLS2) __builtin_amdgcn_raw_buffer_store_b128(__builtin_bit_cast(u32x4, v), rs_y1, yo1[e], 0, MUMPY_WS_STORE_AUX);
         }
     };
     const uint32_t soff = ((uint32_t)e_row * BN + 4u * e_c4) * 4u;
@@ -582,7 +595,7 @@
     }
 }
 
-template <int P, bool CONV = false, int IO = 0, int LN = 0, bool DUAL = false>
+template <int P, bool CONV = false, int IO = 0, int LN = 0, bool DUAL = false, bool COLS2 = false>
 __global__ __launch_bounds__(768, 3) void gemm_ws_kernel(Params p) {
     extern __shared__ __attribute__((aligned(1024))) float lds[];
     const int tid = threadIdx.x, lane = tid & 63;
@@ -608,7 +621,7 @@
     } else {
         if (!(DBG & 8)) __builtin_amdgcn_s_setprio(3);
         if (wave < 8) loader_role<CONV, IO != 0>(p, lds, t0, kc0, n_chunks, tid - 256);
-        else epilogue_role<P, IO == 1, LN, DUAL>(p, lds, b, G, u0, u1, tid - 512);
+        else epilogue_role<P, IO == 1, LN, DUAL, COLS2>(p, lds, b, G, u0, u1, tid - 512);
     }
 }
 
@@ -683,9 +696,10 @@
 inline int launch(const float* x, const float* W, const float* bias, const float* residual, float* y, int64_t M, int N,
                   int K, int act, int num_cu, hipStream_t s, void* ws = nullptr, int64_t ws_bytes = 0, int force_split = -1,
                   void* stamps = nullptr, bool ws_clean = false, const Conv* cv = nullptr, const LnArgs* ln = nullptr,
-                  float* dual_z = nullptr) {
+                  float* dual_z = nullptr, float* y1 = nullptr, int n0 = 0) {
     Params p;
     unsigned grid = base_params(p, x, W, bias, dual_z ? dual_z : residual, y, M, N, K, act, BM, BK, (unsigned)num_cu);
+    p.Y1 = y1; p.N0 = n0;
     if (ln) {
         p.stats_out = ln->stats_out; p.ln_stats = ln->ln_stats; p.ln_colsum = ln->ln_colsum;
         p.ln_gn = ln->ln_gn; p.ln_C = ln->ln_C; p.ln_eps = ln->ln_eps;
@@ -721,9 +735,11 @@
     g_route = Route{};
     g_route.family = Route::WS; g_route.addr = cv ? Route::CONV : Route::DENSE;
     g_route.split = split; g_route.passes = (uint8_t)P; g_route.ln = (uint8_t)ln_mode; g_route.dual = dual_z ? 1 : 0;
+    if (y1) { g_route.n0 = n0; g_route.n1 = N - n0; }
     return with_passes(P, [&](auto pc) {
         constexpr int PC = decltype(pc)::value;
         if (dual_z) return launch_ws<gemm_ws_kernel<PC, false, 0, 0, true>>(grid, LDS_BYTES, LDS_BYTES, s, p);
+        if (y1) return launch_ws<gemm_ws_kernel<PC, false, 0, 0, false, true>>(grid, LDS_BYTES, LDS_BYTES, s, p);
         if (cv) return launch_ws<gemm_ws_kernel<PC, true>>(grid, LDS_BYTES, LDS_BYTES, s, p);
         if (ln_mode == 1) return launch_ws<gemm_ws_kernel<PC, false, 0, 1>>(grid, LDS_BYTES, LDS_BYTES, s, p);
         if (ln_mode == 2) return launch_ws<gemm_ws_kernel<PC, false, 0, 2>>(grid, LDS_BYTES, LDS_BYTES, s, p);
diff --git a/multilateral-temporal-view-pyramid-transformer-for-video-inpainting-detection_amd/csrc/gemm_ws64.h b/multilateral-temporal-view-pyramid-transformer-for-video-inpainting-detection_amd/csrc/gemm_ws64.h
--- a/multilateral-temporal-view-pyramid-transformer-for-video-inpainting-detection_amd/csrc/gemm_ws64.h
+++ b/multilateral-temporal-view-pyramid-transformer-for-video-inpainting-detection_amd/csrc/gemm_ws64.h
@@ -146,24 +146,32 @@
     ws_barrier();
 }
 
-template <int P>
+template <int P, bool COLS2 = false>
 __device__ __forceinline__ void epilogue_role(const Params& p, float* lds, unsigned v0, unsigned n_tiles, int hl) {
     const float* const E = lds + E_OFF_DW;
     const int e_row = hl >> 4, e_c4 = hl & 15;
     const int nk = p.nk;
-    const auto rs_y = __builtin_amdgcn_make_buffer_rsrc(p.Y, 0, (int)((int64_t)p.M * p.N * 4), 0x00020000);
+    const int ny = COLS2 ? p.N0 : p.N;
+    const auto rs_y = __builtin_amdgcn_make_buffer_rsrc(p.Y, 0, (int)((int64_t)p.M * ny * 4), 0x00020000);
+    const auto rs_y1 = __builtin_amdgcn_make_buffer_rsrc(COLS2 ? p.Y1 : p.Y, 0, COLS2 ? (int)((int64_t)p.M * (p.N - p.N0) * 4) : 0, 0x00020000);
     const auto rs_r = __builtin_amdgcn_make_buffer_rsrc(const_cast<float*>(p.residual ? p.residual : p.Y), 0,
-                                                        p.residual ? (int)((int64_t)p.M * p.N * 4) : 0, 0x00020000);
+                                                        p.residual ? (int)((int64_t)p.M * ny * 4) : 0, 0x00020000);
     const auto rs_b = __builtin_amdgcn_make_buffer_rsrc(const_cast<float*>(p.bias ? p.bias : p.Y), 0, p.bias ? p.N * 4 : 0, 0x00020000);
     constexpr int STEPS = PASSES / P;
     f32x4 rv[PASSES], bias4;
-    uint32_t yo[PASSES];
-    const uint32_t row16 = 16u * (uint32_t)p.N * 4u;
+    uint32_t yo[PASSES], yo1[COLS2 ? PASSES : 1];
+    const uint32_t row16 = 16u * (uint32_t)ny * 4u;
     auto begin_tile = [&](unsigned t) {
         unsigned tm, tn;
         tile_coords(p, t, tm, tn);
         const int n = (int)tn * T + 4 * e_c4;
-        const uint32_t ybase = n < p.N ? (((uint32_t)tm * T + e_row) * (uint32_t)p.N + (uint32_t)n) * 4u : OOB;
+        const uint32_t ybase = n < ny ? (((uint32_t)tm * T + e_row) * (uint32_t)ny + (uint32_t)n) * 4u : OOB;
+        if (COLS2) {
+            const uint32_t n1 = (uint32_t)(p.N - p.N0);
+            const uint32_t ybase1 = (n >= p.N0 && n < p.N) ? (((uint32_t)tm * T + e_row) * n1 + (uint32_t)(n - p.N0)) * 4u : OOB;
+#pragma unroll
+            for (int e = 0; e < PASSES; ++e) yo1[e] = ybase1 + (uint32_t)e * (16u * n1 * 4u);
+        }
 #pragma unroll
         for (int e = 0; e < PASSES; ++e) {
             yo[e] = ybase + (uint32_t)e * row16;
@@ -179,6 +187,7 @@
         }
         v += rv[e];
         __builtin_amdgcn_raw_buffer_store_b128(__builtin_bit_cast(u32x4, v), rs_y, yo[e], 0, 0);
+        if (COLS2) __builtin_amdgcn_raw_buffer_store_b128(__builtin_bit_cast(u32x4, v), rs_y1, yo1[e], 0, 0);
     };
     ws_barrier();
     for (int c = 0; c < nk; ++c) ws_barrier();
@@ -199,7 +208,7 @@
     for (int e = 0; e < PASSES; ++e) pass(e);
 }
 
-template <int P>
+template <int P, bool COLS2 = false>
 __global__ __launch_bounds__(768, 6) void gemm_ws64_kernel(Params p) {
     extern __shared__ __attribute__((aligned(1024))) float lds[];
     const int tid = threadIdx.x, lane = tid & 63;
@@ -213,20 +222,25 @@
     else {
         __builtin_amdgcn_s_setprio(3);
         if (wave < 8) loader_role(p, lds, v0, n_chunks, tid - 256);
-        else epilogue_role<P>(p, lds, v0, cnt, tid - 512);
+        else epilogue_role<P, COLS2>(p, lds, v0, cnt, tid - 512);
     }
 }
 
 inline bool eligible(int64_t M, int N, int K) { return gemm_ws::eligible(M, N, K); }
 
 inline int launch(const float* x, const float* W, const float* bias, const float* residual, float* y, int64_t M, int N, int K,
-                  int act, int num_cu, hipStream_t s, int per_cu = 2) {
+                  int act, int num_cu, hipStream_t s, int per_cu = 2, float* y1 = nullptr, int n0 = 0) {
     Params p;
     const unsigned grid = gemm_ws::base_params(p, x, W, bias, residual, y, M, N, K, act, T, BK, (unsigned)per_cu * (unsigned)num_cu);
     const int P = gemm_ws::passes_per_chunk(PASSES, p.nk);
     const int lds_bytes = per_cu == 1 ? 2 * LDS_BYTES + 1024 : LDS_BYTES;
     g_route = Route{};
     g_route.family = Route::WS64; g_route.passes = (uint8_t)(P > 4 ? 4 : P);
+    p.Y1 = y1; p.N0 = n0;
+    if (y1) { g_route.n0 = n0; g_route.n1 = N - n0; }
+    if (y1) return gemm_ws::with_passes<4>(P, [&](auto pc) {
+        return gemm_ws::launch_ws<gemm_ws64_kernel<decltype(pc)::value, true>>(grid, lds_bytes, 2 * LDS_BYTES + 1024, s, p, "gemm_ws64");
+    });
     return gemm_ws::with_passes<4>(P, [&](auto pc) {
         return gemm_ws::launch_ws<gemm_ws64_kernel<decltype(pc)::value>>(grid, lds_bytes, 2 * LDS_BYTES + 1024, s, p, "gemm_ws64");
     });
diff --git a/multilateral-temporal-view-pyramid-transformer-for-video-inpainting-detection_amd/models/encoder/multiTemporalViewEncoder.py b/multilateral-temporal-view-pyramid-transformer-for-video-inpainting-detection_amd/models/encoder/multiTemporalViewEncoder.py
--- a/multilateral-temporal-view-pyramid-transformer-for-video-inpainting-detection_amd/models/encoder/multiTemporalViewEncoder.py
+++ b/multilateral-temporal-view-pyramid-transformer-for-video-inpainting-detection_amd/models/encoder/multiTemporalViewEncoder.py
@@ -66,6 +66,12 @@
         out = ops.linear(a, self.attn.proj.weight, self.attn.proj.bias)
         return ops.add(x1, out), out
 
+    def msa_handover(self, x1, wcat, bcat):
+        h, w = self.input_resolution
+        b, l1, c1 = x1.shape
+        a = self.attn.attend(ops.layernorm(x1, self.norm1.weight, self.norm1.bias, self.norm1.eps), b, l1 // w, w, 0, None)
+        return ops.linear_split(a, wcat, bcat, c1, residual=x1)
+
     def prep(self, x1):
         if self.last_view:
             return None
@@ -73,13 +79,13 @@
         b, l1, _ = x1.shape
         return self.cva.crossattn._prep(x1, (b, l1 // w, w))
 
-    def tail(self, x1, x2, prep=None):
+    def tail(self, x1, x2, prep=None, projected=False):
         h, w = self.input_resolution
         b, l1, c1 = x1.shape
         hs1 = l1 // w
         if not self.last_view:
             hs2 = x2.shape[1] // w
-            x2p = ops.linear(x2, self.pre.weight, self.pre.bias)
+            x2p = x2 if projected else ops.linear(x2, self.pre.weight, self.pre.bias)
             x1 = self.cva.crossattn.attend_combine(x1, x2p, b, hs1, w, hs2, prep)
         if ops.storage() == "bf16":
             return self.mlp.forward_bf16(ops.layernorm_bf16(x1, self.norm2.weight, self.norm2.bias, self.norm2.eps), x1)
@@ -107,10 +113,31 @@
                                      temporal_dims=view_configs[0]["temporal_ratio"], **kw)
         self.block3 = CrossSwinBlock(hid[2], hid[2], input_resolution[2], heads[2], window_size=ws[2], last_view=True,
                                      temporal_dims=3, **kw)
+        self._handover = [Derived(), Derived()]
+
+    @staticmethod
+    def handover_active():
+        return not torch.is_grad_enabled() and ops.matrix_math() == "fp32" and ops.storage() == "fp32"
+
+    def handover_weights(self):
+        def cat(proj, pre):
+            w, b = ops.compose_linear(pre.weight, pre.bias, proj.weight, proj.bias)
+            return torch.cat([proj.weight.detach(), w]).contiguous(), torch.cat([proj.bias.detach(), b]).contiguous()
+        pairs = ((self.block3.attn.proj, self.block2.pre), (self.block2.attn.proj, self.block1.pre))
+        return [d.get((proj.weight, proj.bias, pre.weight, pre.bias), lambda proj=proj, pre=pre: cat(proj, pre))
+                for d, (proj, pre) in zip(self._handover, pairs)]
 
     def forward(self, x):
         from mumpy_hip import streams
+        ho = self.handover_weights() if self.handover_active() else None
         if streams.SERIAL:
+            if ho:
+                x3a, p3 = self.block3.msa_handover(x[2], *ho[0])
+                x3 = self.block3.tail(x3a, None)
+                x2a, p2 = self.block2.msa_handover(x[1], *ho[1])
+                x2 = self.block2.tail(x2a, p3, projected=True)
+                x1a, _ = self.block1.msa(x[0])
+                return [self.block1.tail(x1a, p2, projected=True), x2, x3]
             x3, out3 = self.block3(x[2], x[2])
             x2, out2 = self.block2(x[1], out3)
             x1, _ = self.block1(x[0], out2)
@@ -121,17 +148,17 @@
         fork.record(main)
         streams._DEPTH[0] += 1
         try:
-            x3a, out3 = self.block3.msa(x[2])
+            x3a, out3 = self.block3.msa_handover(x[2], *ho[0]) if ho else self.block3.msa(x[2])
             e3.record(main)
             sa.wait_event(fork)
             x[1].record_stream(sa)
             with torch.cuda.stream(sa):
-                x2a, out2 = self.block2.msa(x[1])
+                x2a, out2 = self.block2.msa_handover(x[1], *ho[1]) if ho else self.block2.msa(x[1])
                 e2.record(sa)
                 prep2 = self.block2.prep(x2a)
                 sa.wait_event(e3)
                 out3.record_stream(sa)
-                x2 = self.block2.tail(x2a, out3, prep2)
+                x2 = self.block2.tail(x2a, out3, prep2, projected=ho is not None)
             sb.wait_event(fork)
             x[0].record_stream(sb)
             with torch.cuda.stream(sb):
@@ -139,7 +166,7 @@
                 prep1 = self.block1.prep(x1a)
                 sb.wait_event(e2)
                 out2.record_stream(sb)
-                x1 = self.block1.tail(x1a, out2, prep1)
+                x1 = self.block1.tail(x1a, out2, prep1, projected=ho is not None)
             x3 = self.block3.tail(x3a, None)
         finally:
             streams._DEPTH[0] -= 1
diff --git a/multilateral-temporal-view-pyramid-transformer-for-video-inpainting-detection_amd/mumpy_hip/lib.py b/multilateral-temporal-view-pyramid-transformer-for-video-inpainting-detection_amd/mumpy_hip/lib.py
--- a/multilateral-temporal-view-pyramid-transformer-for-video-inpainting-detection_amd/mumpy_hip/lib.py
+++ b/multilateral-temporal-view-pyramid-transformer-for-video-inpainting-detection_amd/mumpy_hip/lib.py
@@ -187,6 +187,10 @@
     "mumpy_resize_nearest_u8_fwd": [c_f, c_f, c_f, c_f, c_l, c_i, c_i, c_i, c_i, c_i, c_f],
 })
 
+LINEAR_SPLIT = Surface("mumpy_linear_split.h", "mumpy_linear_split_version", 1, {
+    "mumpy_linear_split_fwd": [c_f, c_f, c_f, c_f, c_f, c_f, c_l, c_i, c_i, c_i, c_i, c_f, c_l, c_f],
+})
+
 
 def library_path() -> str:
     if "MUMPY_HIP_LIB" in os.environ:
@@ -221,7 +225,7 @@
     lib.mumpy_last_error.restype = ctypes.c_char_p
     lib.mumpy_last_route.restype = ctypes.c_char_p
     lib.mumpy_last_route.argtypes = []
-    for s in SURFACES + [PERTURB]:
+    for s in SURFACES + [PERTURB, LINEAR_SPLIT]:
         version = getattr(lib, s.version_fn)
         version.restype, version.argtypes = c_i, []
         if version() != s.version:
diff --git a/multilateral-temporal-view-pyramid-transformer-for-video-inpainting-detection_amd/mumpy_hip/ops.py b/multilateral-temporal-view-pyramid-transformer-for-video-inpainting-detection_amd/mumpy_hip/ops.py
--- a/multilateral-temporal-view-pyramid-transformer-for-video-inpainting-detection_amd/mumpy_hip/ops.py
+++ b/multilateral-temporal-view-pyramid-transformer-for-video-inpainting-detection_amd/mumpy_hip/ops.py
@@ -325,6 +325,38 @@
     _call("mumpy_linear_wsz_fwd", _p(x), _p(weight), _p(bias), _p(residual),
           _p(out), m, n, k, act | _MATH, _p(ws), 0 if ws is None else ws.numel() * 4, _stream(), work=2.0 * m * n * k)
     return out
+
+
+def linear_split(x, weight, bias, n0, residual=None):
+    if _MATH != MATH_FP32 or _STORAGE != "fp32":
+        raise RuntimeError(f"linear_split: fp32 matrix math and storage only (matrix math {matrix_math()}, storage {_STORAGE})")
+    x, weight = _chk(x, "x"), _chk(weight, "weight")
+    if weight.dim() != 2 or x.shape[-1] != weight.shape[1]:
+        raise RuntimeError(f"linear_split: x has {x.shape[-1]} features, weight is {tuple(weight.shape)}")
+    n, k = weight.shape
+    n1 = n - n0
+    if n0 <= 0 or n1 <= 0:
+        raise RuntimeError(f"linear_split: n0={n0} must split the {n} rows of weight in two")
+    m = x.numel() // k
+    residual, bias = _rd_opt(residual, "residual", m * n0, "linear_split"), _rd_opt(bias, "bias", n, "linear_split")
+    y0 = torch.empty(*x.shape[:-1], n0, device=x.device, dtype=torch.float32)
+    y1 = torch.empty(*x.shape[:-1], n1, device=x.device, dtype=torch.float32)
+    wsb = _ws_bytes((m, n, k), "mumpy_linear_workspace_bytes", m, n, k)
+    ws = _kept_workspace(wsb, x.device) if wsb else None
+    _call("mumpy_linear_split_fwd", _p(x), _p(weight), _p(bias), _p(residual), _p(y0), _p(y1), m, n0, n1, k, ACT_NONE, _p(ws),
+          0 if ws is None else ws.numel() * 4, _stream(), work=2.0 * m * n * k)
+    return y0, y1
+
+
+def compose_linear(w2, b2, w1, b1):
+    w2d = w2.detach().double()
+    w = w2d @ w1.detach().double()
+    b = torch.zeros(w2.shape[0], dtype=torch.float64, device=w2.device)
+    if b1 is not None:
+        b = b + w2d @ b1.detach().double()
+    if b2 is not None:
+        b = b + b2.detach().double()
+    return w.float().contiguous(), b.float().contiguous()
 
 
 _BACKGROUND = [0]
```

Result: no change. 381.0 clips/s (-0.9%).
